# dragonlong/articulated-pose

Measured on AMD Instinct MI355X. Metric: point-clouds/sec (N=1024, eyeglasses ANCSH infer+pose-fit), higher is better.
Workload: dtype f32 (network) / f64 (joint LM)

## Files before the change

### articulated-pose_amd/_lib.py

```python
import ctypes
import os
import subprocess

import torch

_HERE = os.path.dirname(os.path.abspath(__file__))
LIB_PATH = os.environ.get("ANCSH_HIP_LIB") or os.path.join(_HERE, "libancsh_hip.so")

_c_int, _c_long, _c_float, _vp = ctypes.c_int, ctypes.c_long, ctypes.c_float, ctypes.c_void_p

SIGNATURES = {
    "ancsh_farthest_point_sample": [_c_int, _c_int, _c_int, _vp, _vp, _vp, _vp],
    "ancsh_farthest_point_sample_gather": [_c_int, _c_int, _c_int, _vp, _vp, _vp, _vp, _vp],
    "ancsh_prob_sample": [_c_int, _c_int, _c_int, _vp, _vp, _vp, _vp, _vp],
    "ancsh_gather_point": [_c_int, _c_int, _c_int, _vp, _vp, _vp, _vp],
    "ancsh_query_ball_point": [_c_int, _c_int, _c_int, _c_float, _c_int, _vp, _vp, _vp, _vp, _vp],
    "ancsh_query_ball_point_multi": [_c_int] + [_vp] * 10,
    "ancsh_group_point": [_c_int, _c_int, _c_int, _c_int, _c_int, _vp, _vp, _vp, _vp],
    "ancsh_group_point_multi": [_c_int] + [_vp] * 9,
    "ancsh_selection_sort": [_c_int, _c_int, _c_int, _c_int, _vp, _vp, _vp, _vp],
    "ancsh_knn_point": [_c_int, _c_int, _c_int, _c_int, _c_int, _vp, _vp, _vp, _vp, _vp],
    "ancsh_group_point_ex": [_c_int, _c_int, _c_int, _c_int, _c_int, _vp, _vp, _vp, _vp, _c_int, _c_int, _vp],
    "ancsh_three_nn": [_c_int, _c_int, _c_int, _vp, _vp, _vp, _vp, _vp],
    "ancsh_three_weights": [_c_int, _vp, _vp, _vp],
    "ancsh_three_nn_weights": [_c_int, _c_int, _c_int, _vp, _vp, _vp, _vp, _vp, _vp],
    "ancsh_three_interpolate": [_c_int, _c_int, _c_int, _c_int, _vp, _vp, _vp, _vp, _vp],
    "ancsh_three_interpolate_ex": [_c_int, _c_int, _c_int, _c_int, _vp, _vp, _vp, _vp, _c_int, _c_int, _vp],
    "ancsh_conv1x1": [_c_long, _c_int, _c_int, _vp, _c_int, _vp, _vp, _vp, _vp, _c_int, _vp, _c_int, _c_int, _vp],
    "ancsh_conv1x1_ex": [_c_long, _c_int, _c_int, _vp, _c_int, _vp, _vp, _vp, _vp, _c_int, _vp, _c_int, _c_int, _vp, _c_int, _vp],
    "ancsh_conv1x1_packed": [_c_long, _c_int, _c_int, _vp, _c_int, _vp, _vp, _vp, _vp, _c_int, _vp, _c_int, _c_int, _vp, _c_int, _vp],
    "ancsh_conv1x1_packed_grouped": [_c_int, _c_long, _c_int, _c_int, _vp, _c_int, _vp, _vp, _vp, _vp, _c_int, _vp, _c_int, _c_int, _vp, _c_int, _vp],
    "ancsh_conv1x1_grouped": [_c_int, _c_long, _c_int, _c_int, _vp, _c_int, _vp, _vp, _vp, _vp, _c_int, _vp, _c_int, _c_int, _vp],
    "ancsh_sa_module_fused_grouped": [_c_int] * 9 + [_vp] * 4 + [_vp, _vp, _vp],
    "ancsh_sa_module_fused_partial_grouped": [_c_int] * 8 + [_vp] * 7,
    "ancsh_fp_interpolate_concat_ex": [_c_int, _c_int, _c_int, _c_int, _vp, _vp, _vp, _vp, _c_int, _vp, _c_int, _c_int, _c_int, _vp],
    "ancsh_sa_pack_weights_bf16x3": [_c_int, _c_int, _vp, _vp, _vp],
    "ancsh_sa_module_fused_bf16x3": [_c_int] * 8 + [_vp] * 4 + [_vp, _vp, _vp],
    "ancsh_sa_module_fused_partial_bf16x3": [_c_int] * 7 + [_vp] * 7,
    "ancsh_sa_module_fused_bf16x3_grouped": [_c_int] * 9 + [_vp] * 4 + [_vp, _vp, _vp],
    "ancsh_sa_module_fused_partial_bf16x3_grouped": [_c_int] * 8 + [_vp] * 7,
    "ancsh_sa_pack_weights_f16x2": [_c_int, _c_int, _vp, _vp, _vp],
    "ancsh_sa_module_fused_f16x2_grouped": [_c_int] * 9 + [_vp] * 4 + [_vp, _vp, _vp],
    "ancsh_sa_module_fused_partial_f16x2_grouped": [_c_int] * 8 + [_vp] * 7,
    "ancsh_mlp_chain_grouped_fp_f16x2": [_c_int] * 5 + [_vp] * 7 + [_vp],
    "ancsh_sa3_chain_grouped_bf16x3": [_c_int] * 7 + [_vp] * 4 + [_vp],
    "ancsh_sa3_chain_grouped_f16x2": [_c_int] * 7 + [_vp] * 4 + [_vp],
    "ancsh_fp1_chain_grouped_bf16x3": [_c_int] * 6 + [_vp] * 4 + [_vp],
    "ancsh_fp1_chain_grouped_f16x2": [_c_int] * 6 + [_vp] * 4 + [_vp],
    "ancsh_fp2_chain_grouped_bf16x3": [_c_int] * 8 + [_vp] * 6 + [_vp],
    "ancsh_fp2_chain_grouped_f16x2": [_c_int] * 8 + [_vp] * 6 + [_vp],
    "ancsh_sa_module_fused_f16x2_grouped_guarded": [_c_int] * 9 + [_vp] * 4 + [_vp, _vp, _vp, _c_int, _vp],
    "ancsh_sa_module_fused_partial_f16x2_grouped_guarded": [_c_int] * 8 + [_vp] * 6 + [_vp, _c_int, _vp],
    "ancsh_mlp_chain_grouped_fp_f16x2_guarded": [_c_int] * 5 + [_vp] * 7 + [_vp, _c_int, _vp],
    "ancsh_sa3_chain_grouped_f16x2_guarded": [_c_int] * 7 + [_vp] * 4 + [_vp, _c_int, _vp],
    "ancsh_fp1_chain_grouped_f16x2_guarded": [_c_int] * 6 + [_vp] * 4 + [_vp, _c_int, _vp],
    "ancsh_fp2_chain_grouped_f16x2_guarded": [_c_int] * 8 + [_vp] * 6 + [_vp, _c_int, _vp],
    "ancsh_iou_3d": [_c_int, _c_int, _vp, _vp, _vp, _vp, _vp],
    "ancsh_joint_params": [_c_int] * 5 + [_vp] * 9 + [_vp],
    "ancsh_part_extents": [_c_int] * 4 + [_vp] * 3 + [_c_int] + [_vp] * 4 + [_vp],
    "ancsh_articulation_rec": [_c_int] * 5 + [_vp] * 10 + [_vp] * 4 + [_vp],
    "ancsh_fp_interpolate_concat": [_c_int, _c_int, _c_int, _c_int, _vp, _vp, _vp, _vp, _c_int, _vp, _c_int, _vp],
    "ancsh_query_ball_group_xyz": [_c_int, _c_int, _c_int, _c_float, _c_int, _vp, _vp, _c_int, _vp, _vp, _vp, _c_int, _vp],
    "ancsh_query_ball_group_xyz_multi": [_c_int] + [_vp] * 13,
    "ancsh_group_max": [_c_long, _c_int, _c_int, _vp, _vp, _vp],
    "ancsh_sa_module_fused": [_c_int] * 8 + [_vp] * 4 + [_vp, _vp, _vp],
    "ancsh_sa_module_fused_partial": [_c_int] * 7 + [_vp] * 7,
    "ancsh_sa_pack_weights": [_c_int, _c_int, _vp, _vp, _vp],
    "ancsh_mlp_chain": [_c_long, _c_int, _vp, _c_int, _c_int, _vp, _vp, _vp],
    "ancsh_mlp_chain_grouped": [_c_int, _c_long, _c_int, _vp, _c_int, _vp, _vp, _vp, _vp, _vp],
    "ancsh_sa3_chain_grouped": [_c_int] * 7 + [_vp] * 4 + [_vp],
    "ancsh_fp_single_source_init": [_c_int] * 5 + [_vp] * 3 + [_vp],
    "ancsh_fp1_chain_grouped": [_c_int] * 6 + [_vp] * 4 + [_vp],
    "ancsh_fp2_chain_grouped": [_c_int] * 8 + [_vp] * 6 + [_vp],
    "ancsh_mlp_chain_grouped_fp": [_c_int] * 5 + [_vp] * 8 + [_vp],
    "ancsh_mlp_chain_grouped_fp_bf16x3": [_c_int] * 5 + [_vp] * 7 + [_vp],
    "ancsh_head_activations": [_c_long, _c_int, _c_int, _vp, _c_int] + [_vp] * 10 + [_vp],
    "ancsh_pose_partition": [_c_int, _c_int, _c_int] + [_vp] * 11 + [_vp],
    "ancsh_pose_poison_records": [_c_int, _c_int, _c_int] + [_vp] * 5 + [_vp],
    "ancsh_pose_joint_direction": [_c_int, _c_int, _c_int, _vp, _vp, _vp, _vp],
    "ancsh_ransac_single": [_c_int, _vp, _vp, _vp, _c_float, _c_int, _vp, ctypes.c_ulonglong, _c_int, _vp, _vp, _vp, _vp, _vp],
    "ancsh_ransac_single_ex": [_c_int, _vp, _vp, _vp, _c_float, _c_int, _vp, ctypes.c_ulonglong, _c_int, _vp, _vp, _vp, _vp, _vp, _c_long, _vp],
    "ancsh_ransac_single_rec": [_c_int, _vp, _vp, _vp, _c_float, _c_int, _vp, ctypes.c_ulonglong, _c_int, _vp, _vp, _vp, _vp, _vp, _c_long,
                                _vp, _c_int, _vp, _c_float, _vp],
    "ancsh_ransac_joint_rec": [_c_int, _vp, _vp, _vp, _vp, _vp, ctypes.c_double, _c_int, _vp, ctypes.c_ulonglong, _c_int]
                              + [_vp] * 7 + [_c_int, _vp, _c_int, _vp, ctypes.c_double, _vp],
    "ancsh_ransac_joint": [_c_int, _vp, _vp, _vp, _vp, _vp, ctypes.c_double, _c_int, _vp, ctypes.c_ulonglong, _c_int]
                          + [_vp] * 7 + [_vp],
    "ancsh_ransac_single_rec_dseed": [_c_int, _vp, _vp, _vp, _c_float, _c_int, _vp, _vp, _c_int, _vp, _vp, _vp, _vp, _vp, _c_long,
                                      _vp, _c_int, _vp, _c_float, _vp],
    "ancsh_ransac_joint_rec_dseed": [_c_int, _vp, _vp, _vp, _vp, _vp, ctypes.c_double, _c_int, _vp, _vp, _c_int]
                                    + [_vp] * 7 + [_c_int, _vp, _c_int, _vp, ctypes.c_double, _vp],
    "ancsh_input_sample_stream": [_c_int, _c_int, _c_int, _vp, _c_long, _vp, _vp, _c_int, _vp, _vp, _vp, _vp, _vp],
    "ancsh_input_sample_stream_keyed": [_c_int, _c_int, _c_int, _vp, _c_long, _vp, _vp, _c_int, _vp, _vp, _vp, _vp, _vp],
    "ancsh_ransac_single_rec_dkey": [_c_int, _vp, _vp, _vp, _c_float, _c_int, _vp, _vp, _c_int, _vp, _vp, _vp, _vp, _vp, _c_long,
                                     _vp, _c_int, _vp, _c_float, _vp],
    "ancsh_ransac_joint_rec_dkey": [_c_int, _vp, _vp, _vp, _vp, _vp, ctypes.c_double, _c_int, _vp, _vp, _c_int]
                                   + [_vp] * 7 + [_c_int, _vp, _c_int, _vp, ctypes.c_double, _vp],
    "ancsh_raw_point_labels": [_c_int] * 5 + [_vp, _c_long] + [_vp] * 8 + [_vp],
    "ancsh_pose_joint_direction_pred": [_c_int, _c_int, _c_int, _c_int, _vp, _vp, _vp, _vp],
    "ancsh_pose_poison_records_pred": [_c_int, _c_int, _c_int] + [_vp] * 4 + [_c_int, _vp, _vp, _vp],
    "ancsh_input_sample_stream_xyz": [_c_int, _c_int, _c_int, _vp, _c_long, _vp, _vp, _vp, _vp, _vp, _vp],
    "ancsh_input_sample_stream_xyz_keyed": [_c_int, _c_int, _c_int, _vp, _c_long, _vp, _vp, _vp, _vp, _vp, _vp],
    "ancsh_ransac_joint_rec_kind": [_c_int, _vp, _vp, _vp, _vp, _vp, ctypes.c_double, _c_int, _vp, ctypes.c_ulonglong, _c_int]
                                   + [_vp] * 7 + [_c_int, _vp, _c_int, _vp, ctypes.c_double, _vp, _vp],
    "ancsh_ransac_joint_rec_dseed_kind": [_c_int, _vp, _vp, _vp, _vp, _vp, ctypes.c_double, _c_int, _vp, _vp, _c_int]
                                         + [_vp] * 7 + [_c_int, _vp, _c_int, _vp, ctypes.c_double, _vp, _vp],
    "ancsh_ransac_joint_rec_dkey_kind": [_c_int, _vp, _vp, _vp, _vp, _vp, ctypes.c_double, _c_int, _vp, _vp, _c_int]
                                        + [_vp] * 7 + [_c_int, _vp, _c_int, _vp, ctypes.c_double, _vp, _vp],
    "ancsh_depth_unproject_stream": [_c_int, _c_int, _vp, _vp, _c_long, _vp, _vp, _vp, _c_long, _vp, _vp, _vp, _vp],
    "ancsh_depth_label_images": [_c_int, _c_int, _vp, _vp, _c_long] + [_vp] * 5 + [_c_long, _vp, _vp, _vp, _c_long, _vp],
    "ancsh_joint_state_rec": [_c_int] * 3 + [_vp, _c_int] + [_vp] * 5 + [_vp],
    "ancsh_input_sample": [_c_int, _c_int, _c_int, _vp, _vp, _vp, _vp, _c_int, _c_int, _c_int, _vp, _vp, _vp, _vp, _vp],
    "ancsh_test_losses": [_c_int, _c_int, _c_int, _c_int, _vp, _vp, _vp],
    "ancsh_ransac_joint_ex": [_c_int, _vp, _vp, _vp, _vp, _vp, ctypes.c_double, _c_int, _vp, ctypes.c_ulonglong, _c_int]
                             + [_vp] * 7 + [_c_int, _vp],
    "ancsh_umeyama": [_c_int, _vp, _vp, _vp, _vp, _vp],
    "ancsh_estimate_similarity_transform": [_c_int, _vp, _vp, _vp, _c_int, _vp, ctypes.c_ulonglong, _vp, _vp, _vp],
}

_lib = None


def build(force=False):
    args = ["make", "-s", "-j8", "-C", os.path.join(_HERE, "csrc")]
    if force:
        subprocess.check_call(args + ["clean"])
    subprocess.check_call(args)
    return LIB_PATH


def lib():
    global _lib
    if _lib is None:
        if not os.path.exists(LIB_PATH):
            raise RuntimeError(
                f"{LIB_PATH} is missing: the HIP extension is not built (run __graft_entry__.build()); "
                "there is no CPU fallback for the product path")
        L = ctypes.CDLL(LIB_PATH)
        for name, argtypes in SIGNATURES.items():
            fn = getattr(L, name)
            fn.argtypes = argtypes
            fn.restype = _c_int
        L.ancsh_last_error.restype = ctypes.c_char_p
        L.ancsh_abi_version.restype = _c_int
        L.ancsh_last_ball_query_schedule.restype = _c_int
        L.ancsh_sa_packed_weight_floats.argtypes = [_c_int, _c_int]
        L.ancsh_sa_packed_weight_floats.restype = _c_long
        L.ancsh_sa_packed_weight_bytes_bf16x3.argtypes = [_c_int, _c_int]
        L.ancsh_sa_packed_weight_bytes_bf16x3.restype = _c_long
        L.ancsh_sa_packed_weight_bytes_f16x2.argtypes = [_c_int, _c_int]
        L.ancsh_sa_packed_weight_bytes_f16x2.restype = _c_long
        L.ancsh_ransac_single_quads_floats.argtypes = [_c_long, _c_int]
        L.ancsh_ransac_single_quads_floats.restype = _c_long
        _lib = L
    return _lib


def stream_ptr():
    return torch.cuda.current_stream().cuda_stream


def ptr(t):
    return 0 if t is None else t.data_ptr()


_prof = None
_prof_lead = (0, {})


def profile_start(lead=0, lead_for=None):
    global _prof, _prof_lead
    _prof, _prof_lead = [], (int(lead), dict(lead_for or {}))


def profile_stop():
    global _prof
    rec, _prof = _prof, None
    torch.cuda.synchronize()
    return [(n, a, e0.elapsed_time(e1)) for n, a, e0, e1 in rec]


def call(name, *args):
    L = lib()
    if _prof is not None:
        e0, e1 = torch.cuda.Event(enable_timing=True), torch.cuda.Event(enable_timing=True)
        for _ in range(_prof_lead[1].get(name, _prof_lead[0])):
            getattr(L, name)(*args, stream_ptr())
        e0.record()
        rc = getattr(L, name)(*args, stream_ptr())
        e1.record()
        _prof.append((name, args, e0, e1))
    else:
        rc = getattr(L, name)(*args, stream_ptr())
    if rc != 0:
        msg = L.ancsh_last_error().decode()
        if rc == -1:
            raise ValueError(msg)
        raise RuntimeError(f"{name}: {msg}")


def require_cuda(*tensors):
    for t in tensors:
        if t is not None and not t.is_cuda:
            raise RuntimeError("articulated-pose_amd ops run on the MI355X only: got a CPU tensor "
                               "(no CPU fallback in the product path)")
```

### articulated-pose_amd/csrc/pose.hip

```cpp
#include "common.h"
#include "pose_math.h"

namespace ancsh {
namespace pose {

constexpr int MODEL_A = 13;
constexpr int MODEL_B = 26;

__device__ __forceinline__ unsigned long long splitmix64(unsigned long long x) {
    x += 0x9E3779B97F4A7C15ull;
    x = (x ^ (x >> 30)) * 0xBF58476D1CE4E5B9ull;
    x = (x ^ (x >> 27)) * 0x94D049BB133111EBull;
    return x ^ (x >> 31);
}
__device__ __forceinline__ int device_draw(unsigned long long seed, int prob, int iter, int k, int n) {
    const unsigned long long h = splitmix64(seed ^ splitmix64(((unsigned long long)prob << 40) ^ ((unsigned long long)iter << 8) ^ (unsigned)k));
    return (int)(h % (unsigned long long)n);
}
enum { KEY_VALUE = 0, KEY_DSEED = 1, KEY_DKEY = 2 };
struct DKey {
    const ancsh_stream_key *key;
    int parts;
};
template <int KM> struct KeyArgT { typedef unsigned long long type; };
// ... 262 lines not shown
                s3[i][c] = src[(size_t)(r0 + id[i]) * 3 + c];
                t3[i][c] = tgt[(size_t)(r0 + id[i]) * 3 + c];
            }
        estimate_single3(s3, t3, R, sc, tr);
    }
    typedef float f32x8 __attribute__((ext_vector_type(8)));
    const int q0 = quad_start(r0, prob);
    const f32x8 *Q = reinterpret_cast<const f32x8 *>(quads + (size_t)q0 * 24);
    int nq = ((n + 7) >> 3) * 2;
    nq = min(nq, (cap_quads - q0) & ~1);
    f32x2 cnt2 = {0.f, 0.f};
    auto score4 = [&](const f32x8 &v0, const f32x8 &v1, const f32x8 &v2) {
        inlier2_count_f32(R, sc, tr, f32x2{v0[0], v0[1]}, f32x2{v0[4], v0[5]}, f32x2{v1[0], v1[1]}, f32x2{v1[4], v1[5]},
                          f32x2{v2[0], v2[1]}, f32x2{v2[4], v2[5]}, th, cnt2);
        inlier2_count_f32(R, sc, tr, f32x2{v0[2], v0[3]}, f32x2{v0[6], v0[7]}, f32x2{v1[2], v1[3]}, f32x2{v1[6], v1[7]},
                          f32x2{v2[2], v2[3]}, f32x2{v2[6], v2[7]}, th, cnt2);
    };
    constexpr int LGKM0 = 0xC07F;
    if (nq > 0) {
        f32x8 a0 = Q[0], a1 = Q[1], a2 = Q[2];
        __builtin_amdgcn_s_waitcnt(LGKM0);
        for (int q = 0; q < nq; q += 2) {
            const int q2 = q + 2 < nq ? q + 2 : q;
            const f32x8 b0 = Q[q * 3 + 3], b1 = Q[q * 3 + 4], b2 = Q[q * 3 + 5];
            __builtin_amdgcn_sched_barrier(0);
            score4(a0, a1, a2);
            __builtin_amdgcn_sched_barrier(0);
            __builtin_amdgcn_s_waitcnt(LGKM0);
            a0 = Q[q2 * 3]; a1 = Q[q2 * 3 + 1]; a2 = Q[q2 * 3 + 2];
            __builtin_amdgcn_sched_barrier(0);
            score4(b0, b1, b2);
            __builtin_amdgcn_sched_barrier(0);
            __builtin_amdgcn_s_waitcnt(LGKM0);
        }
    }
    if (h < niter) scores[(size_t)prob * niter + h] = n > 0 ? (int)(cnt2.x + cnt2.y) : 0;
}

template <class T>
__device__ __forceinline__ int block_argmax_first(const T *sc, int niter, T *best_out, void *lds) {
    T bv = (T)-1;
    int bi = 0x7fffffff;
    for (int h = threadIdx.x; h < niter; h += blockDim.x) {
        const T v = sc[h];
        if (v > bv) { bv = v; bi = h; }
    }
#pragma unroll
    for (int o = 32; o > 0; o >>= 1) {
        const T ov = __shfl_xor(bv, o, 64);
        const int oi = __shfl_xor(bi, o, 64);
        if (ov > bv || (ov == bv && oi < bi)) { bv = ov; bi = oi; }
    }
    T *rv = (T *)lds;
    int *ri = (int *)(rv + 8);
    const int lane = threadIdx.x & 63, wave = threadIdx.x >> 6, nw = blockDim.x >> 6;
    __syncthreads();
    if (lane == 0) { rv[wave] = bv; ri[wave] = bi; }
    __syncthreads();
    bv = rv[0]; bi = ri[0];
    for (int w = 1; w < nw; ++w)
        if (rv[w] > bv || (rv[w] == bv && ri[w] < bi)) { bv = rv[w]; bi = ri[w]; }
    __syncthreads();
    *best_out = bv;
    return bi;
}

__device__ __forceinline__ void pair_sums(const float (*cs)[3], const float (*ct)[3], int n, double (&pr)[3]) {
#pragma clang fp contract(off)
    const int lane = threadIdx.x & 63;
    const int wave = __builtin_amdgcn_readfirstlane(threadIdx.x >> 6), nw = blockDim.x >> 6;
    const int seg = (n + nw - 1) / nw;
    const int j0 = wave * seg, j1 = min(n, j0 + seg);
    constexpr int RB = 6;
    for (int ib = lane; ib < n; ib += 64 * RB) {
        float sx[RB], sy[RB], sz[RB], tx[RB], ty[RB], tz[RB], ab[RB], aa[RB], bb[RB];
#pragma unroll
        for (int r = 0; r < RB; ++r) {
            const int i = min(ib + 64 * r, n - 1);
            sx[r] = cs[i][0]; sy[r] = cs[i][1]; sz[r] = cs[i][2];
            tx[r] = ct[i][0]; ty[r] = ct[i][1]; tz[r] = ct[i][2];
            ab[r] = aa[r] = bb[r] = 0.f;
        }
        for (int j = j0; j < j1; ++j) {
            const float cx = cs[j][0], cy = cs[j][1], cz = cs[j][2], dx = ct[j][0], dy = ct[j][1], dz = ct[j][2];
#pragma unroll
            for (int r = 0; r < RB; ++r) {
                const float ux = sx[r] - cx, uy = sy[r] - cy, uz = sz[r] - cz;
                const float vx = tx[r] - dx, vy = ty[r] - dy, vz = tz[r] - dz;
                const float A = __builtin_amdgcn_sqrtf((ux * ux + uy * uy) + uz * uz);
                const float b = __builtin_amdgcn_sqrtf((vx * vx + vy * vy) + vz * vz);
                ab[r] += A * b;
                aa[r] += A * A;
                bb[r] += b * b;
            }
        }
#pragma unroll
        for (int r = 0; r < RB; ++r)
            if (ib + 64 * r < n) { pr[0] += (double)ab[r]; pr[1] += (double)aa[r]; pr[2] += (double)bb[r]; }
    }
}

__device__ __forceinline__ void refit_similarity(const float (*cs)[3], const float (*ct)[3], int n_in, double *red,
                                                 double R[9], double &scale, double tr[3]) {
    double sums[6] = {0, 0, 0, 0, 0, 0};
    for (int i = threadIdx.x; i < n_in; i += 256) {
#pragma unroll
        for (int c = 0; c < 3; ++c) { sums[c] += cs[i][c]; sums[3 + c] += ct[i][c]; }
    }
    block_sum<6>(sums, red, 4);
    double sm[3], tm[3];
#pragma unroll
    for (int c = 0; c < 3; ++c) { sm[c] = sums[c] / n_in; tm[c] = sums[3 + c] / n_in; }
    double M[9] = {0, 0, 0, 0, 0, 0, 0, 0, 0};
    for (int i = threadIdx.x; i < n_in; i += 256)
#pragma unroll
        for (int a = 0; a < 3; ++a)
#pragma unroll
            for (int b = 0; b < 3; ++b) M[a * 3 + b] += (ct[i][a] - tm[a]) * (cs[i][b] - sm[b]);
    block_sum<9>(M, red, 4);
    double q[4];
    horn_quat(M, q);
    quat_to_mat(q, R);
    double pr[3] = {0, 0, 0};
    pair_sums(cs, ct, n_in, pr);
    block_sum<3>(pr, red, 4);
    scale = pr[0] / (pr[1] + 1e-6);
    const double sf = (double)(float)scale;
#pragma unroll
    for (int a = 0; a < 3; ++a) tr[a] = tm[a] - sf * (R[a * 3 + 0] * sm[0] + R[a * 3 + 1] * sm[1] + R[a * 3 + 2] * sm[2]);
}

__device__ __forceinline__ int compact_flagged(bool flag, int i, int n, const float *src, const float *tgt, size_t row0,
                                               float (*cs)[3], float (*ct)[3], int base, int *wcnt) {
    const int lane = threadIdx.x & 63, wave = threadIdx.x >> 6;
    const unsigned long long m = __ballot(flag);
    __syncthreads();
    if (lane == 0) wcnt[wave] = __popcll(m);
    __syncthreads();
    int start = base;
    for (int w = 0; w < wave; ++w) start += wcnt[w];
    const int total = wcnt[0] + wcnt[1] + wcnt[2] + wcnt[3];
    if (flag) {
        const int pos = start + __builtin_amdgcn_mbcnt_hi((unsigned)(m >> 32), __builtin_amdgcn_mbcnt_lo((unsigned)m, 0));
#pragma unroll
        for (int c = 0; c < 3; ++c) {
            cs[pos][c] = src[(row0 + i) * 3 + c];
            ct[pos][c] = tgt[(row0 + i) * 3 + c];
        }
    }
    return base + total;
}

template <int KM>
__global__ __launch_bounds__(256) void ransac_single_finish_kernel(const int *__restrict__ off, const float *__restrict__ src,
                                                                   const float *__restrict__ tgt, float th, int niter,
                                                                   const int *__restrict__ draws, KeyArg<KM> seed_arg,
                                                                   const int *__restrict__ scores, int max_n,
                                                                   double *__restrict__ out_model,
                                                                   unsigned char *__restrict__ out_inliers,
                                                                   int *__restrict__ out_best, FitExtras E) {
    const unsigned long long seed = kernel_seed<KM>(seed_arg, 0);
    const int kbase = key_problem_base<KM>(seed_arg);
    extern __shared__ __attribute__((aligned(16))) unsigned char smem[];
    double *red = (double *)smem;
    int *wcnt = (int *)(red + 64);
    float(*cs)[3] = (float(*)[3])(wcnt + 8);
    float(*ct)[3] = cs + max_n;
    const int prob = blockIdx.x;
    const int r0 = off[prob], n = off[prob + 1] - r0;
    double *om = out_model + (size_t)prob * MODEL_A;
    if (n <= 0 || n > max_n) {
        if (threadIdx.x < MODEL_A) om[threadIdx.x] = NAN;
        if (E.record && threadIdx.x < (E.K == 1 ? 2 * MODEL_A : MODEL_A)) E.record[(size_t)prob * 26 + threadIdx.x] = NAN;
        if (E.tie && threadIdx.x < 2) E.tie[prob * 2 + threadIdx.x] = 0;
        if (threadIdx.x == 0) { out_best[prob * 2] = -1; out_best[prob * 2 + 1] = n <= 0 ? 0 : -2; }
        for (int i = threadIdx.x; i < n; i += 256) out_inliers[r0 + i] = 0;
        return;
    }
    int best_score;
    const int best = block_argmax_first<int>(scores + (size_t)prob * niter, niter, &best_score, red);
    int id[3];
    load_draw3(draws, seed, prob, kbase, niter, best, 0, 3, n, id);
    float s3[3][3], t3[3][3], R[9], sc, tr[3];
#pragma unroll
    for (int i = 0; i < 3; ++i)
#pragma unroll
        for (int c = 0; c < 3; ++c) {
            s3[i][c] = src[(size_t)(r0 + id[i]) * 3 + c];
            t3[i][c] = tgt[(size_t)(r0 + id[i]) * 3 + c];
        }
    estimate_single3(s3, t3, R, sc, tr);
    int n_in = 0, n_border = 0, n_near = 0;
    for (int base = 0; base < n; base += 256) {
        const int i = base + threadIdx.x;
        bool f = false, border = false;
        if (i < n) {
            const float *ps = src + (size_t)(r0 + i) * 3, *pt = tgt + (size_t)(r0 + i) * 3;
            const float rs = residual_sq_f32(R, sc, tr, ps[0], ps[1], ps[2], pt[0], pt[1], pt[2]);
            f = rs < th;
            border = rs >= E.lo_f && rs < E.hi_f;
            out_inliers[r0 + i] = f ? 1 : 0;
        }
        n_border += __popcll(__ballot(border));
        n_in = compact_flagged(f, i, n, src, tgt, (size_t)r0, cs, ct, n_in, wcnt);
    }
    if (E.tie) {
        const bool winner_degenerate = id[0] == id[1] || id[0] == id[2] || id[1] == id[2];
        __shared__ int s_cand[TIE_MAX_CAND];
        const int *sp = scores + (size_t)prob * niter;
        const int lane = threadIdx.x & 63, wave = threadIdx.x >> 6;
        int found = 0;
        for (int h0 = 0; h0 < niter; h0 += 256) {
            const int h = h0 + threadIdx.x;
            bool cand = false;
            if (h < niter && h != best && sp[h] >= best_score - 1) {
                int d3[3];
                load_draw3(draws, seed, prob, kbase, niter, h, 0, 3, n, d3);
                cand = d3[0] == d3[1] || d3[0] == d3[2] || d3[1] == d3[2];
            }
            const unsigned long long m = __ballot(cand);
            __syncthreads();
            if (lane == 0) wcnt[wave] = __popcll(m);
            __syncthreads();
            int start = found;
            for (int w = 0; w < wave; ++w) start += wcnt[w];
            if (cand) {
                const int slot = start + __builtin_amdgcn_mbcnt_hi((unsigned)(m >> 32), __builtin_amdgcn_mbcnt_lo((unsigned)m, 0));
                if (slot < TIE_MAX_CAND) s_cand[slot] = h;
            }
            found += wcnt[0] + wcnt[1] + wcnt[2] + wcnt[3];
        }
        __syncthreads();
        const int ncand = found < TIE_MAX_CAND ? found : TIE_MAX_CAND;
        n_near = found - ncand + (winner_degenerate ? 1 : 0);
        for (int c = 0; c < ncand; ++c) {
            const int h = s_cand[c];
            int d3[3];
            load_draw3(draws, seed, prob, kbase, niter, h, 0, 3, n, d3);
            float hs[3][3], ht[3][3], hR[9], hsc, htr[3];
#pragma unroll
            for (int i = 0; i < 3; ++i)
#pragma unroll
                for (int cc = 0; cc < 3; ++cc) {
                    hs[i][cc] = src[(size_t)(r0 + d3[i]) * 3 + cc];
                    ht[i][cc] = tgt[(size_t)(r0 + d3[i]) * 3 + cc];
                }
            estimate_single3(hs, ht, hR, hsc, htr);
            int differs = 0;
            for (int i = threadIdx.x; i < n; i += 256) {
                const float *ps = src + (size_t)(r0 + i) * 3, *pt = tgt + (size_t)(r0 + i) * 3;
                const bool f = residual_sq_f32(hR, hsc, htr, ps[0], ps[1], ps[2], pt[0], pt[1], pt[2]) < th;
                differs |= (int)(f != (out_inliers[r0 + i] != 0));
            }
            n_near += __syncthreads_or(differs) ? 1 : 0;
        }
        if ((threadIdx.x & 63) == 0) wcnt[4 + (threadIdx.x >> 6)] = n_border;
        __syncthreads();
        if (threadIdx.x == 0) {
            E.tie[prob * 2] = wcnt[4] + wcnt[5] + wcnt[6] + wcnt[7];
            E.tie[prob * 2 + 1] = winner_degenerate ? -n_near : n_near;
        }
    }
    __syncthreads();
    double Rd[9], scale, trd[3];
    if (n_in > 0) {
        refit_similarity(cs, ct, n_in, red, Rd, scale, trd);
    } else {
#pragma unroll
        for (int a = 0; a < 9; ++a) Rd[a] = NAN;
        scale = NAN; trd[0] = trd[1] = trd[2] = NAN;
    }
    if (threadIdx.x == 0) {
#pragma unroll
        for (int a = 0; a < 9; ++a) om[a] = Rd[a];
        om[9] = (double)(float)scale;
#pragma unroll
        for (int a = 0; a < 3; ++a) om[10 + a] = trd[a];
        out_best[prob * 2] = best;
        out_best[prob * 2 + 1] = best_score;
        if (E.record) {
            double *rec = E.record + (size_t)prob * 26;
#pragma unroll
            for (int a = 0; a < MODEL_A; ++a) rec[a] = om[a];
            if (E.K == 1) {
#pragma unroll
                for (int a = 0; a < MODEL_A; ++a) rec[MODEL_A + a] = om[a];
            }
        }
    }
}

struct PartFd {
    Rod b, p[3];
    double rh[3];
    double blk[6];
    double gv[3];
    double ju[3];
    double jd[3][3];

    __device__ __forceinline__ void begin_points(const double r[3]) {
        b = rod_prepare(r[0], r[1], r[2]);
#pragma unroll
        for (int q = 0; q < 3; ++q) {
            const double h = fd_step(r[q]);
            rh[q] = fast_rcp(h);
            p[q] = rod_prepare(r[0] + (q == 0 ? h : 0.0), r[1] + (q == 1 ? h : 0.0), r[2] + (q == 2 ? h : 0.0));
        }
#pragma unroll
        for (int i = 0; i < 6; ++i) blk[i] = 0.0;
        gv[0] = gv[1] = gv[2] = 0.0;
    }
    __device__ __forceinline__ void begin(const double r[3], const double J[3]) {
        begin_points(r);
        rod_apply(b, J[0], J[1], J[2], ju[0], ju[1], ju[2]);
#pragma unroll
        for (int q = 0; q < 3; ++q) {
            double qx, qy, qz;
            rod_apply(p[q], J[0], J[1], J[2], qx, qy, qz);
            jd[0][q] = qx; jd[1][q] = qy; jd[2][q] = qz;
        }
    }
    __device__ __forceinline__ void point(double px, double py, double pz, double yx, double yy, double yz) {
        double ox, oy, oz;
        rod_apply(b, px, py, pz, ox, oy, oz);
        const double f0 = yx - ox, f1 = yy - oy, f2 = yz - oz;
        double a[3][3];
#pragma unroll
        for (int q = 0; q < 3; ++q) {
            double qx, qy, qz;
            rod_apply(p[q], px, py, pz, qx, qy, qz);
            a[0][q] = ((yx - qx) - f0) * rh[q];
            a[1][q] = ((yy - qy) - f1) * rh[q];
            a[2][q] = ((yz - qz) - f2) * rh[q];
        }
#pragma unroll
        for (int q = 0; q < 3; ++q) {
#pragma unroll
            for (int r = 0; r <= q; ++r) blk[q * (q + 1) / 2 + r] += a[0][q] * a[0][r] + a[1][q] * a[1][r] + a[2][q] * a[2][r];
            gv[q] += a[0][q] * f0 + a[1][q] * f1 + a[2][q] * f2;
        }
    }
};

__device__ __forceinline__ void assemble_normal(const PartFd &p0, const double blk0[6], const double g0[3], const PartFd &p1,
                                                const double blk1[6], const double g1[3], double wj, double A[21], double g[6]) {
    double f[3], a[3][6];
#pragma unroll
    for (int c = 0; c < 3; ++c) f[c] = p0.ju[c] - p1.ju[c];
#pragma unroll
    for (int c = 0; c < 3; ++c)
#pragma unroll
        for (int q = 0; q < 3; ++q) {
            a[c][q] = (((p0.jd[c][q] - p1.ju[c]) - f[c])) * p0.rh[q];
            a[c][3 + q] = (((p0.ju[c] - p1.jd[c][q]) - f[c])) * p1.rh[q];
        }
#pragma unroll
    for (int i = 0; i < 6; ++i) {
#pragma unroll
        for (int j = 0; j <= i; ++j) {
            double v = wj * (a[0][i] * a[0][j] + a[1][i] * a[1][j] + a[2][i] * a[2][j]);
            if (i < 3) v += blk0[i * (i + 1) / 2 + j];
            else if (j >= 3) v += blk1[(i - 3) * (i - 2) / 2 + (j - 3)];
            A[i * (i + 1) / 2 + j] = v;
        }
        g[i] = wj * (a[0][i] * f[0] + a[1][i] * f[1] + a[2][i] * f[2]) + (i < 3 ? g0[i] : g1[i - 3]);
    }
}

__device__ __forceinline__ double prismatic_cost(const double x[6]) {
    const double a = x[0] - x[3], b = x[1] - x[4], c = x[2] - x[5];
    return a * a + b * b + c * c;
}
__device__ __forceinline__ void assemble_normal_prismatic(const double x[6], const double blk0[6], const double g0[3],
                                                          const double blk1[6], const double g1[3], double A[21], double g[6]) {
    double f[3], d0[3], d1[3];
#pragma unroll
    for (int c = 0; c < 3; ++c) {
        const double h0 = fd_step(x[c]), h1 = fd_step(x[3 + c]);
        f[c] = x[c] - x[3 + c];
        d0[c] = (((x[c] + h0) - x[3 + c]) - f[c]) * fast_rcp(h0);
        d1[c] = ((x[c] - (x[3 + c] + h1)) - f[c]) * fast_rcp(h1);
    }
#pragma unroll
    for (int i = 0; i < 6; ++i) {
#pragma unroll
        for (int j = 0; j <= i; ++j) {
            double v = 0.0;
            if (i < 3) v = (i == j ? d0[i] * d0[i] : 0.0) + blk0[i * (i + 1) / 2 + j];
            else if (j >= 3) v = (i == j ? d1[i - 3] * d1[i - 3] : 0.0) + blk1[(i - 3) * (i - 2) / 2 + (j - 3)];
            else if (i - 3 == j) v = d1[j] * d0[j];
            A[i * (i + 1) / 2 + j] = v;
        }
        g[i] = i < 3 ? d0[i] * f[i] + g0[i] : d1[i - 3] * f[i - 3] + g1[i - 3];
    }
}

template <bool PRISM>
struct HypProblemT {
    double x0[3][3], y0[3][3], x1[3][3], y1[3][3], J[3], wj;

    __device__ __forceinline__ double cost(const double x[6]) const {
        const Rod r0 = rod_prepare(x[0], x[1], x[2]), r1 = rod_prepare(x[3], x[4], x[5]);
        double s = 0.0, ox, oy, oz;
#pragma unroll
        for (int i = 0; i < 3; ++i) {
            rod_apply(r0, x0[i][0], x0[i][1], x0[i][2], ox, oy, oz);
            const double a = y0[i][0] - ox, b = y0[i][1] - oy, c = y0[i][2] - oz;
            s += a * a + b * b + c * c;
            rod_apply(r1, x1[i][0], x1[i][1], x1[i][2], ox, oy, oz);
            const double d = y1[i][0] - ox, e = y1[i][1] - oy, f = y1[i][2] - oz;
            s += d * d + e * e + f * f;
        }
        if constexpr (PRISM) {
            return s + prismatic_cost(x);
        } else {
            double ux, uy, uz, wx, wy, wz;
            rod_apply(r0, J[0], J[1], J[2], ux, uy, uz);
            rod_apply(r1, J[0], J[1], J[2], wx, wy, wz);
            s += wj * ((ux - wx) * (ux - wx) + (uy - wy) * (uy - wy) + (uz - wz) * (uz - wz));
            return s;
        }
    }
    __device__ __forceinline__ void normal(const double x[6], double A[21], double g[6]) const {
        PartFd p0, p1;
        if constexpr (PRISM) p0.begin_points(x); else p0.begin(x, J);
#pragma unroll
        for (int i = 0; i < 3; ++i) p0.point(x0[i][0], x0[i][1], x0[i][2], y0[i][0], y0[i][1], y0[i][2]);
        if constexpr (PRISM) p1.begin_points(x + 3); else p1.begin(x + 3, J);
#pragma unroll
        for (int i = 0; i < 3; ++i) p1.point(x1[i][0], x1[i][1], x1[i][2], y1[i][0], y1[i][1], y1[i][2]);
        if constexpr (PRISM) assemble_normal_prismatic(x, p0.blk, p0.gv, p1.blk, p1.gv, A, g);
        else assemble_normal(p0, p0.blk, p0.gv, p1, p1.blk, p1.gv, wj, A, g);
    }
};
typedef HypProblemT<false> HypProblem;

__device__ __forceinline__ void scales3(const float s[3][3], const float t[3][3], float &sc, float &sc_inv) {
    double ab = 0.0, aa = 0.0, bb = 0.0;
#pragma unroll
    for (int i = 0; i < 3; ++i)
#pragma unroll
        for (int j = i + 1; j < 3; ++j) {
            double ds = 0.0, dt = 0.0;
#pragma unroll
            for (int c = 0; c < 3; ++c) {
                const double u = (double)s[i][c] - s[j][c], v = (double)t[i][c] - t[j][c];
                ds += u * u;
                dt += v * v;
            }
            ab += 2.0 * sqrt(ds) * sqrt(dt);
            aa += 2.0 * ds;
            bb += 2.0 * dt;
        }
    sc = (float)(ab / (aa + 1e-6));
    sc_inv = (float)(ab / (bb + 1e-6));
}

__device__ __forceinline__ void center_part3(const float s[3][3], const float t[3][3], float sc_inv, double xc[3][3],
                                             double yc[3][3]) {
    float sm[3], tm[3];
#pragma unroll
    for (int c = 0; c < 3; ++c) {
        sm[c] = ((s[0][c] + s[1][c]) + s[2][c]) / 3.0f;
        tm[c] = ((sc_inv * t[0][c] + sc_inv * t[1][c]) + sc_inv * t[2][c]) / 3.0f;
    }
#pragma unroll
    for (int i = 0; i < 3; ++i) {
#pragma unroll
        for (int c = 0; c < 3; ++c) {
            xc[i][c] = (double)(s[i][c] - sm[c]);
            yc[i][c] = (double)(sc_inv * t[i][c] - tm[c]);
        }
    }
}

__device__ __forceinline__ void prep_part3(const float s[3][3], const float t[3][3], float sc_inv, double xc[3][3],
                                           double yc[3][3], double rv[3]) {
    center_part3(s, t, sc_inv, xc, yc);
    double M[9] = {0, 0, 0, 0, 0, 0, 0, 0, 0};
#pragma unroll
    for (int i = 0; i < 3; ++i)
#pragma unroll
        for (int a = 0; a < 3; ++a)
#pragma unroll
            for (int b = 0; b < 3; ++b) M[a * 3 + b] += yc[i][a] * xc[i][b];
    double q[4];
    horn_quat_fast(M, q);
    quat_to_rotvec(q, rv);
}

__device__ __forceinline__ double residual_sq_f64(const double R[9], double sc, const double tr[3], float sx, float sy, float sz,
                                                  float tx, float ty, float tz) {
    const double rx = R[0] * sx + R[1] * sy + R[2] * sz, ry = R[3] * sx + R[4] * sy + R[5] * sz,
                 rz = R[6] * sx + R[7] * sy + R[8] * sz;
    const double ex = ((double)tx - sc * rx) - tr[0], ey = ((double)ty - sc * ry) - tr[1], ez = ((double)tz - sc * rz) - tr[2];
    return ex * ex + ey * ey + ez * ez;
}
__device__ __forceinline__ bool inlier_f64(const double R[9], double sc, const double tr[3], float sx, float sy, float sz,
                                           float tx, float ty, float tz, double th) {
    return residual_sq_f64(R, sc, tr, sx, sy, sz, tx, ty, tz) < th;
}

struct HypSamples {
    float s0[3][3], t0[3][3], s1[3][3], t1[3][3];
};
__device__ __forceinline__ void load_hyp_samples(const float *__restrict__ src, const float *__restrict__ tgt, const int *draws,
                                                 unsigned long long seed, int prob, int kbase, int niter, int h, int a0, int n0, int a1,
                                                 int n1, HypSamples &q) {
    int i0[3], i1[3];
    load_draw3(draws, seed, prob, kbase, niter, h, 0, 6, n0, i0);
    load_draw3(draws, seed, prob, kbase, niter, h, 3, 6, n1, i1);
#pragma unroll
    for (int i = 0; i < 3; ++i)
#pragma unroll
        for (int c = 0; c < 3; ++c) {
            q.s0[i][c] = src[(size_t)(a0 + i0[i]) * 3 + c];
            q.t0[i][c] = tgt[(size_t)(a0 + i0[i]) * 3 + c];
            q.s1[i][c] = src[(size_t)(a1 + i1[i]) * 3 + c];
            q.t1[i][c] = tgt[(size_t)(a1 + i1[i]) * 3 + c];
        }
}

template <int KM>
__global__ __launch_bounds__(64) void ransac_joint_init_kernel(const int *__restrict__ rng0, const int *__restrict__ rng1,
                                                               const float *__restrict__ src, const float *__restrict__ tgt,
                                                               int niter, const int *__restrict__ draws, KeyArg<KM> seed_arg,
                                                               double *__restrict__ scores, double *__restrict__ models) {
    const unsigned long long seed = kernel_seed<KM>(seed_arg, 1);
    const int kbase = key_problem_base<KM>(seed_arg);
    const int prob = blockIdx.y, h = blockIdx.x * 64 + threadIdx.x;
    const int a0 = rng0[prob * 2], n0 = rng0[prob * 2 + 1] - a0;
    const int a1 = rng1[prob * 2], n1 = rng1[prob * 2 + 1] - a1;
    if (h >= niter) return;
    double *mo = models + ((size_t)prob * niter + h) * MODEL_B;
    if (n0 <= 0 || n1 <= 0) {
        scores[(size_t)prob * niter + h] = -1.0;
        for (int i = 0; i < MODEL_B; ++i) mo[i] = NAN;
        return;
    }
    HypSamples q;
    load_hyp_samples(src, tgt, draws, seed, prob, kbase, niter, h, a0, n0, a1, n1, q);
    float sc0, sc0i, sc1, sc1i;
    scales3(q.s0, q.t0, sc0, sc0i);
    scales3(q.s1, q.t1, sc1, sc1i);
    double xc[3][3], yc[3][3], x[6];
    prep_part3(q.s0, q.t0, sc0i, xc, yc, x);
    prep_part3(q.s1, q.t1, sc1i, xc, yc, x + 3);
#pragma unroll
    for (int i = 0; i < 6; ++i) mo[i] = x[i];
    mo[6] = sc0i; mo[7] = sc1i; mo[8] = sc0; mo[9] = sc1;
}

constexpr int HYP_CHUNK = 256;
constexpr int HYP_CHUNK_SMALL = 64;
constexpr long HYP_SMALL_LAUNCH = 8192;
constexpr int HYP_REFILL = 16;

template <int KM, bool PRISM>
__device__ __forceinline__ void ransac_joint_lm_run(const int *__restrict__ rng0, const int *__restrict__ rng1,
                                                    const float *__restrict__ src, const float *__restrict__ tgt,
                                                    const float *__restrict__ joint_dir, int niter,
                                                    const int *__restrict__ draws, KeyArg<KM> seed_arg,
                                                    double *__restrict__ models, int *__restrict__ lm_stat, int chunk) {
    const unsigned long long seed = kernel_seed<KM>(seed_arg, 1);
    const int kbase = key_problem_base<KM>(seed_arg);
    const int prob = blockIdx.y;
    const int a0 = rng0[prob * 2], n0 = rng0[prob * 2 + 1] - a0;
    const int a1 = rng1[prob * 2], n1 = rng1[prob * 2 + 1] - a1;
    if (n0 <= 0 || n1 <= 0) return;
    const int c1 = min(niter, (int)(blockIdx.x + 1) * chunk);
    int next = blockIdx.x * chunk;
    HypProblemT<PRISM> P;
    if constexpr (!PRISM) {
        P.J[0] = joint_dir[prob * 3]; P.J[1] = joint_dir[prob * 3 + 1]; P.J[2] = joint_dir[prob * 3 + 2];
        P.wj = 3.0;
    }
    Lm6 S;
    bool active = false;
    int h = 0;
    for (;;) {
        const unsigned long long idle = __ballot(!active);
        const int n_idle = __popcll(idle);
        if (next < c1 && (n_idle >= HYP_REFILL || n_idle >= c1 - next || n_idle == 64)) {
            if (!active) {
                const int mine = next + __builtin_amdgcn_mbcnt_hi((unsigned)(idle >> 32), __builtin_amdgcn_mbcnt_lo((unsigned)idle, 0));
                if (mine < c1) {
                    h = mine;
                    const double *mo = models + ((size_t)prob * niter + h) * MODEL_B;
                    HypSamples q;
                    load_hyp_samples(src, tgt, draws, seed, prob, kbase, niter, h, a0, n0, a1, n1, q);
                    center_part3(q.s0, q.t0, (float)mo[6], P.x0, P.y0);
                    center_part3(q.s1, q.t1, (float)mo[7], P.x1, P.y1);
#pragma unroll
                    for (int i = 0; i < 6; ++i) S.x[i] = mo[i];
                    lm6_begin(P, S);
                    active = true;
                }
            }
            next += n_idle;
        } else if (n_idle == 64) {
            break;
        }
        if (active && lm6_trip(P, S, 1e-4, 1e-8, 1e-8, 4200)) {
            double *mo = models + ((size_t)prob * niter + h) * MODEL_B;
#pragma unroll
            for (int i = 0; i < 6; ++i) mo[i] = S.x[i];
#ifdef LM_COUNT
            if (lm_stat) { lm_stat[((size_t)prob * niter + h) * 2] = S.info | (S.trips << 4) | (S.nchol << 17); lm_stat[((size_t)prob * niter + h) * 2 + 1] = S.nfev; }
#else
            if (lm_stat) { lm_stat[((size_t)prob * niter + h) * 2] = S.info; lm_stat[((size_t)prob * niter + h) * 2 + 1] = S.nfev; }
#endif
            active = false;
        }
    }
}

template <int KM>
__global__ __launch_bounds__(64) void ransac_joint_lm_kernel(const int *__restrict__ rng0, const int *__restrict__ rng1,
                                                             const float *__restrict__ src, const float *__restrict__ tgt,
                                                             const float *__restrict__ joint_dir, int niter,
                                                             const int *__restrict__ draws, KeyArg<KM> seed_arg,
                                                             double *__restrict__ models, int *__restrict__ lm_stat, int chunk) {
    ransac_joint_lm_run<KM, false>(rng0, rng1, src, tgt, joint_dir, niter, draws, seed_arg, models, lm_stat, chunk);
}

template <int KM>
__global__ __launch_bounds__(64) void ransac_joint_lm_kind_kernel(const int *__restrict__ rng0, const int *__restrict__ rng1,
                                                                  const float *__restrict__ src, const float *__restrict__ tgt,
                                                                  const float *__restrict__ joint_dir, int niter,
                                                                  const int *__restrict__ draws, KeyArg<KM> seed_arg,
                                                                  double *__restrict__ models, int *__restrict__ lm_stat, int chunk,
                                                                  const int *__restrict__ joint_kind) {
    if (joint_kind[blockIdx.y] != 0) ransac_joint_lm_run<KM, true>(rng0, rng1, src, tgt, joint_dir, niter, draws, seed_arg, models, lm_stat, chunk);
    else ransac_joint_lm_run<KM, false>(rng0, rng1, src, tgt, joint_dir, niter, draws, seed_arg, models, lm_stat, chunk);
}

constexpr int COOP_G = 8;
constexpr int COOP_XCH = 112;
constexpr int COOP_HYP_PER_WAVE = 32;

__device__ __forceinline__ void group_lds_fence() {
    __builtin_amdgcn_fence(__ATOMIC_RELEASE, "wavefront");
    __builtin_amdgcn_wave_barrier();
    __builtin_amdgcn_fence(__ATOMIC_ACQUIRE, "wavefront");
}

template <bool PRISM>
struct HypProblemCoopT {
    double x0[3][3], y0[3][3], x1[3][3], y1[3][3], J[3], wj;
    double *xch;
    int role;

    __device__ __forceinline__ double cost(const double x[6]) const {
        const bool joint = role >= 6;
        const bool p1 = role >= 3 && role < 6;
        const int i = joint ? 0 : (p1 ? role - 3 : role);
        double partial;
        if (!joint) {
            const Rod r = p1 ? rod_prepare(x[3], x[4], x[5]) : rod_prepare(x[0], x[1], x[2]);
            const double px = p1 ? (i == 0 ? x1[0][0] : i == 1 ? x1[1][0] : x1[2][0]) : (i == 0 ? x0[0][0] : i == 1 ? x0[1][0] : x0[2][0]);
            const double py = p1 ? (i == 0 ? x1[0][1] : i == 1 ? x1[1][1] : x1[2][1]) : (i == 0 ? x0[0][1] : i == 1 ? x0[1][1] : x0[2][1]);
            const double pz = p1 ? (i == 0 ? x1[0][2] : i == 1 ? x1[1][2] : x1[2][2]) : (i == 0 ? x0[0][2] : i == 1 ? x0[1][2] : x0[2][2]);
            const double tx = p1 ? (i == 0 ? y1[0][0] : i == 1 ? y1[1][0] : y1[2][0]) : (i == 0 ? y0[0][0] : i == 1 ? y0[1][0] : y0[2][0]);
            const double ty = p1 ? (i == 0 ? y1[0][1] : i == 1 ? y1[1][1] : y1[2][1]) : (i == 0 ? y0[0][1] : i == 1 ? y0[1][1] : y0[2][1]);
            const double tz = p1 ? (i == 0 ? y1[0][2] : i == 1 ? y1[1][2] : y1[2][2]) : (i == 0 ? y0[0][2] : i == 1 ? y0[1][2] : y0[2][2]);
            double ox, oy, oz;
            rod_apply(r, px, py, pz, ox, oy, oz);
            const double a = tx - ox, b = ty - oy, c = tz - oz;
            partial = a * a + b * b + c * c;
        } else if constexpr (PRISM) {
            partial = prismatic_cost(x);
        } else {
            const Rod r0 = rod_prepare(x[0], x[1], x[2]), r1 = rod_prepare(x[3], x[4], x[5]);
            double ux, uy, uz, wx, wy, wz;
            rod_apply(r0, J[0], J[1], J[2], ux, uy, uz);
            rod_apply(r1, J[0], J[1], J[2], wx, wy, wz);
            partial = (ux - wx) * (ux - wx) + (uy - wy) * (uy - wy) + (uz - wz) * (uz - wz);
        }
        double *cs = xch + 102;
        if (role < 7) cs[role] = partial;
        group_lds_fence();
        double s = 0.0;
#pragma unroll
        for (int k = 0; k < 3; ++k) { s += cs[k]; s += cs[3 + k]; }
        if constexpr (PRISM) s += cs[6]; else s += wj * cs[6];
        group_lds_fence();
        return s;
    }

    __device__ __forceinline__ void normal(const double x[6], double A[21], double g[6]) const {
        double *col = xch, *jdx = xch + 54, *rhx = xch + 72, *fx = xch + 78, *jux = xch + 96;
        {
            const int cr = role < 6 ? role : role - 6;
            const bool p1 = cr >= 3;
            const int q = p1 ? cr - 3 : cr;
            const double r0 = p1 ? x[3] : x[0], r1 = p1 ? x[4] : x[1], r2 = p1 ? x[5] : x[2];
            const Rod b = rod_prepare(r0, r1, r2);
            const double h = fd_step(q == 0 ? r0 : q == 1 ? r1 : r2);
            const double rh = fast_rcp(h);
            const Rod pr = rod_prepare(r0 + (q == 0 ? h : 0.0), r1 + (q == 1 ? h : 0.0), r2 + (q == 2 ? h : 0.0));
            const bool wr = role < 6;
#pragma unroll
            for (int i = 0; i < 3; ++i) {
                const double px = p1 ? x1[i][0] : x0[i][0], py = p1 ? x1[i][1] : x0[i][1], pz = p1 ? x1[i][2] : x0[i][2];
                const double yx = p1 ? y1[i][0] : y0[i][0], yy = p1 ? y1[i][1] : y0[i][1], yz = p1 ? y1[i][2] : y0[i][2];
                double ox, oy, oz, qx, qy, qz;
                rod_apply(b, px, py, pz, ox, oy, oz);
                const double f0 = yx - ox, f1 = yy - oy, f2 = yz - oz;
// ... 172 lines not shown
    for (int i = 0; i < 6; ++i) x[i] = mo[i];
    const float sc0 = (float)mo[8], sc1 = (float)mo[9];
    double R0[9], R1[9], tr0[3], tr1[3];
    rotvec_to_mat(x, R0);
    rotvec_to_mat(x + 3, R1);
#pragma unroll
    for (int a = 0; a < 3; ++a) {
        double u = 0.0, v = 0.0;
#pragma unroll
        for (int i = 0; i < 3; ++i) {
            u += (double)q.t0[i][a] - (double)sc0 * (R0[a * 3] * q.s0[i][0] + R0[a * 3 + 1] * q.s0[i][1] + R0[a * 3 + 2] * q.s0[i][2]);
            v += (double)q.t1[i][a] - (double)sc1 * (R1[a * 3] * q.s1[i][0] + R1[a * 3 + 1] * q.s1[i][1] + R1[a * 3 + 2] * q.s1[i][2]);
        }
        tr0[a] = u / 3.0;
        tr1[a] = v / 3.0;
    }
#pragma unroll
    for (int a = 0; a < 9; ++a) { mo[a] = R0[a]; mo[13 + a] = R1[a]; }
    mo[9] = sc0; mo[22] = sc1;
#pragma unroll
    for (int a = 0; a < 3; ++a) { mo[10 + a] = tr0[a]; mo[23 + a] = tr1[a]; }
}

__global__ __launch_bounds__(256) void ransac_joint_verify_kernel(const int *__restrict__ rng0, const int *__restrict__ rng1,
                                                                 const float *__restrict__ src, const float *__restrict__ tgt,
                                                                 double th, int niter, const double *__restrict__ models,
                                                                 double *__restrict__ scores) {
    const int prob = blockIdx.y, lane = threadIdx.x & 63;
    const int h = blockIdx.x * 4 + (threadIdx.x >> 6);
    if (h >= niter) return;
    const int a0 = rng0[prob * 2], n0 = rng0[prob * 2 + 1] - a0;
    const int a1 = rng1[prob * 2], n1 = rng1[prob * 2 + 1] - a1;
    if (n0 <= 0 || n1 <= 0) return;
    const double *mo = models + ((size_t)prob * niter + h) * MODEL_B;
    double R0[9], R1[9], tr0[3], tr1[3];
#pragma unroll
    for (int a = 0; a < 9; ++a) { R0[a] = mo[a]; R1[a] = mo[13 + a]; }
    const double sc0 = mo[9], sc1 = mo[22];
#pragma unroll
    for (int a = 0; a < 3; ++a) { tr0[a] = mo[10 + a]; tr1[a] = mo[23 + a]; }
    int c0 = 0, c1 = 0;
    for (int i = lane; i < n0; i += 64) {
        const float *ps = src + (size_t)(a0 + i) * 3, *pt = tgt + (size_t)(a0 + i) * 3;
        c0 += inlier_f64(R0, sc0, tr0, ps[0], ps[1], ps[2], pt[0], pt[1], pt[2], th) ? 1 : 0;
    }
    for (int i = lane; i < n1; i += 64) {
        const float *ps = src + (size_t)(a1 + i) * 3, *pt = tgt + (size_t)(a1 + i) * 3;
        c1 += inlier_f64(R1, sc1, tr1, ps[0], ps[1], ps[2], pt[0], pt[1], pt[2], th) ? 1 : 0;
    }
#pragma unroll
    for (int o = 32; o > 0; o >>= 1) { c0 += __shfl_xor(c0, o, 64); c1 += __shfl_xor(c1, o, 64); }
    if (lane == 0) scores[(size_t)prob * niter + h] = ((double)c0 / 3.0 + (double)c1 / 3.0) / 2.0;
}

template <bool PRISM>
struct BlockProblemT {
    const float (*x0)[3];
    const float (*y0)[3];
    const float (*x1)[3];
    const float (*y1)[3];
    int n0, n1;
    double J[3], wj;
    double *red;

    __device__ __forceinline__ double cost(const double x[6]) const {
        const Rod r0 = rod_prepare(x[0], x[1], x[2]), r1 = rod_prepare(x[3], x[4], x[5]);
        double s[1] = {0.0}, ox, oy, oz;
        for (int i = threadIdx.x; i < n0; i += 256) {
            rod_apply(r0, x0[i][0], x0[i][1], x0[i][2], ox, oy, oz);
            const double a = y0[i][0] - ox, b = y0[i][1] - oy, c = y0[i][2] - oz;
            s[0] += a * a + b * b + c * c;
        }
        for (int i = threadIdx.x; i < n1; i += 256) {
            rod_apply(r1, x1[i][0], x1[i][1], x1[i][2], ox, oy, oz);
            const double a = y1[i][0] - ox, b = y1[i][1] - oy, c = y1[i][2] - oz;
            s[0] += a * a + b * b + c * c;
        }
        block_sum<1>(s, red, 4);
        if constexpr (PRISM) {
            return s[0] + prismatic_cost(x);
        } else {
            double ux, uy, uz, wx, wy, wz;
            rod_apply(r0, J[0], J[1], J[2], ux, uy, uz);
            rod_apply(r1, J[0], J[1], J[2], wx, wy, wz);
            return s[0] + wj * ((ux - wx) * (ux - wx) + (uy - wy) * (uy - wy) + (uz - wz) * (uz - wz));
        }
    }
    __device__ __forceinline__ void normal(const double x[6], double A[21], double g[6]) const {
        PartFd p0, p1;
        if constexpr (PRISM) p0.begin_points(x); else p0.begin(x, J);
        for (int i = threadIdx.x; i < n0; i += 256) p0.point(x0[i][0], x0[i][1], x0[i][2], y0[i][0], y0[i][1], y0[i][2]);
        if constexpr (PRISM) p1.begin_points(x + 3); else p1.begin(x + 3, J);
        for (int i = threadIdx.x; i < n1; i += 256) p1.point(x1[i][0], x1[i][1], x1[i][2], y1[i][0], y1[i][1], y1[i][2]);
        double v[18];
#pragma unroll
        for (int i = 0; i < 6; ++i) { v[i] = p0.blk[i]; v[9 + i] = p1.blk[i]; }
#pragma unroll
        for (int i = 0; i < 3; ++i) { v[6 + i] = p0.gv[i]; v[15 + i] = p1.gv[i]; }
        block_sum<18>(v, red, 4);
        if constexpr (PRISM) assemble_normal_prismatic(x, v, v + 6, v + 9, v + 15, A, g);
        else assemble_normal(p0, v, v + 6, p1, v + 9, v + 15, wj, A, g);
    }
};
typedef BlockProblemT<false> BlockProblem;

__device__ __forceinline__ void block_scales(const float (*cs)[3], const float (*ct)[3], int n, double *red, float &sc,
                                             float &sc_inv) {
    double pr[3] = {0, 0, 0};
    pair_sums(cs, ct, n, pr);
    block_sum<3>(pr, red, 4);
    sc = (float)(pr[0] / (pr[1] + 1e-6));
    sc_inv = (float)(pr[0] / (pr[2] + 1e-6));
}

__device__ __forceinline__ void block_prep_part(float (*cs)[3], float (*ct)[3], int n, float sc_inv, double *red,
                                                double smean[3], double tmean[3], double rv[3]) {
    double sums[6] = {0, 0, 0, 0, 0, 0};
    for (int i = threadIdx.x; i < n; i += 256)
#pragma unroll
        for (int c = 0; c < 3; ++c) { sums[c] += cs[i][c]; sums[3 + c] += ct[i][c]; }
    block_sum<6>(sums, red, 4);
#pragma unroll
    for (int c = 0; c < 3; ++c) { smean[c] = sums[c] / n; tmean[c] = sums[3 + c] / n; }
    double M[9] = {0, 0, 0, 0, 0, 0, 0, 0, 0};
    for (int i = threadIdx.x; i < n; i += 256) {
        float xc[3], yc[3];
#pragma unroll
        for (int c = 0; c < 3; ++c) {
            xc[c] = cs[i][c] - (float)smean[c];
            yc[c] = sc_inv * ct[i][c] - (float)((double)sc_inv * tmean[c]);
            cs[i][c] = xc[c];
            ct[i][c] = yc[c];
        }
#pragma unroll
        for (int a = 0; a < 3; ++a)
#pragma unroll
            for (int b = 0; b < 3; ++b) M[a * 3 + b] += (double)yc[a] * xc[b];
    }
    block_sum<9>(M, red, 4);
    double q[4];
    horn_quat(M, q);
    quat_to_rotvec(q, rv);
}

template <int KM, bool PRISM>
__device__ __forceinline__ void ransac_joint_finish_run(const int *__restrict__ rng0, const int *__restrict__ rng1,
                                                        const float *__restrict__ src, const float *__restrict__ tgt,
                                                        const float *__restrict__ joint_dir, double th, int niter,
                                                        const double *__restrict__ scores,
                                                        const double *__restrict__ models, int max_n,
                                                        double *__restrict__ out_model,
                                                        unsigned char *__restrict__ out_inliers,
                                                        int *__restrict__ out_best, double *__restrict__ out_score, const FitExtras &E,
                                                        unsigned char *smem) {
    double *red = (double *)smem;
    int *wcnt = (int *)(red + 128);
    float(*c0s)[3] = (float(*)[3])(wcnt + 8);
    float(*c0t)[3] = c0s + max_n;
    float(*c1s)[3] = c0t + max_n;
    float(*c1t)[3] = c1s + max_n;
    const int prob = blockIdx.x;
    const int a0 = rng0[prob * 2], n0 = rng0[prob * 2 + 1] - a0;
    const int a1 = rng1[prob * 2], n1 = rng1[prob * 2 + 1] - a1;
    double *om = out_model + (size_t)prob * MODEL_B;
    unsigned char *oi0 = out_inliers + (size_t)prob * 2 * max_n, *oi1 = oi0 + max_n;
    double *rec1 = nullptr, *rec0 = nullptr;
    if (E.record) {
        const int cloud = prob / (E.K - 1), q = prob - cloud * (E.K - 1);
        rec1 = E.record + ((size_t)cloud * E.K + q + 1) * 26 + MODEL_A;
        if (q == 0) rec0 = E.record + (size_t)cloud * E.K * 26 + MODEL_A;
    }
    if (n0 <= 0 || n1 <= 0 || n0 > max_n || n1 > max_n) {
        if (threadIdx.x < MODEL_B) om[threadIdx.x] = NAN;
        if (threadIdx.x < MODEL_A) { if (rec1) rec1[threadIdx.x] = NAN; if (rec0) rec0[threadIdx.x] = NAN; }
        if (E.tie && threadIdx.x < 2) E.tie[prob * 2 + threadIdx.x] = 0;
        if (threadIdx.x == 0) { out_best[prob] = -1; out_score[prob] = -1.0; }
        for (int i = threadIdx.x; i < 2 * max_n; i += 256) oi0[i] = 0;
        return;
    }
    for (int i = n0 + threadIdx.x; i < max_n; i += 256) oi0[i] = 0;
    for (int i = n1 + threadIdx.x; i < max_n; i += 256) oi1[i] = 0;
    double best_score;
    const int best = block_argmax_first<double>(scores + (size_t)prob * niter, niter, &best_score, red);
    const double *bm = models + ((size_t)prob * niter + best) * MODEL_B;
    double R0[9], R1[9], tr0[3], tr1[3];
#pragma unroll
    for (int a = 0; a < 9; ++a) { R0[a] = bm[a]; R1[a] = bm[13 + a]; }
    const double hs0 = bm[9], hs1 = bm[22];
#pragma unroll
    for (int a = 0; a < 3; ++a) { tr0[a] = bm[10 + a]; tr1[a] = bm[23 + a]; }
    int m0 = 0, m1 = 0, n_border = 0, n_near = 0;
    for (int base = 0; base < n0; base += 256) {
        const int i = base + threadIdx.x;
        bool f = false, border = false;
        if (i < n0) {
            const float *ps = src + (size_t)(a0 + i) * 3, *pt = tgt + (size_t)(a0 + i) * 3;
            const double rs = residual_sq_f64(R0, hs0, tr0, ps[0], ps[1], ps[2], pt[0], pt[1], pt[2]);
            f = rs < th;
            border = rs >= E.lo_d && rs < E.hi_d;
            oi0[i] = f ? 1 : 0;
        }
        n_border += __popcll(__ballot(border));
        m0 = compact_flagged(f, i, n0, src, tgt, (size_t)a0, c0s, c0t, m0, wcnt);
    }
    for (int base = 0; base < n1; base += 256) {
        const int i = base + threadIdx.x;
        bool f = false, border = false;
        if (i < n1) {
            const float *ps = src + (size_t)(a1 + i) * 3, *pt = tgt + (size_t)(a1 + i) * 3;
            const double rs = residual_sq_f64(R1, hs1, tr1, ps[0], ps[1], ps[2], pt[0], pt[1], pt[2]);
            f = rs < th;
            border = rs >= E.lo_d && rs < E.hi_d;
            oi1[i] = f ? 1 : 0;
        }
        n_border += __popcll(__ballot(border));
        m1 = compact_flagged(f, i, n1, src, tgt, (size_t)a1, c1s, c1t, m1, wcnt);
    }
    if (E.tie) {
        const unsigned long long tseed = kernel_seed<KM>(E.seed, 1);
        const int tbase = KM == KEY_DKEY ? ((const ancsh_stream_key *)E.seed)->cloud_base * (E.K - 1) : 0;
        const double *sp = scores + (size_t)prob * niter;
        const double near = best_score - (1.0 / 6.0 + 1e-9);
        for (int h = threadIdx.x; h < niter + 255 - (niter + 255) % 256; h += 256) {
            bool degenerate = false;
            if (h < niter && sp[h] >= near) {
                int i0[3], i1[3];
                load_draw3(E.draws, tseed, prob, tbase, niter, h, 0, 6, n0, i0);
                load_draw3(E.draws, tseed, prob, tbase, niter, h, 3, 6, n1, i1);
                degenerate = i0[0] == i0[1] || i0[0] == i0[2] || i0[1] == i0[2] || i1[0] == i1[1] || i1[0] == i1[2] || i1[1] == i1[2];
            }
            n_near += __popcll(__ballot(degenerate));
        }
        if ((threadIdx.x & 63) == 0) { wcnt[4 + (threadIdx.x >> 6)] = n_border; red[8 + (threadIdx.x >> 6)] = (double)n_near; }
        __syncthreads();
        if (threadIdx.x == 0) {
            E.tie[prob * 2] = wcnt[4] + wcnt[5] + wcnt[6] + wcnt[7];
            E.tie[prob * 2 + 1] = (int)(red[8] + red[9] + red[10] + red[11]);
        }
    }
    __syncthreads();
    if (m0 == 0 || m1 == 0) {
        if (threadIdx.x < MODEL_B) om[threadIdx.x] = NAN;
        if (threadIdx.x < MODEL_A) { if (rec1) rec1[threadIdx.x] = NAN; if (rec0) rec0[threadIdx.x] = NAN; }
        if (threadIdx.x == 0) { out_best[prob] = best; out_score[prob] = best_score; }
        return;
    }
    float sc0, sc0i, sc1, sc1i;
    block_scales(c0s, c0t, m0, red, sc0, sc0i);
    block_scales(c1s, c1t, m1, red, sc1, sc1i);
    double sm0[3], tm0[3], sm1[3], tm1[3], x[6];
    block_prep_part(c0s, c0t, m0, sc0i, red, sm0, tm0, x);
    block_prep_part(c1s, c1t, m1, sc1i, red, sm1, tm1, x + 3);
    __syncthreads();
    if constexpr (PRISM) {
        BlockProblemT<true> P;
        P.x0 = c0s; P.y0 = c0t; P.x1 = c1s; P.y1 = c1t;
        P.n0 = m0; P.n1 = m1;
        P.red = red;
        lmdif6(P, x, 1e-4, 1e-8, 1e-8, 4200, nullptr);
    } else {
        BlockProblem P;
        P.x0 = c0s; P.y0 = c0t; P.x1 = c1s; P.y1 = c1t;
        P.n0 = m0; P.n1 = m1;
        P.J[0] = joint_dir[prob * 3]; P.J[1] = joint_dir[prob * 3 + 1]; P.J[2] = joint_dir[prob * 3 + 2];
        P.wj = (double)(m0 < m1 ? m0 : m1);
        P.red = red;
        lmdif6(P, x, 1e-4, 1e-8, 1e-8, 4200, nullptr);
    }
    rotvec_to_mat(x, R0);
    rotvec_to_mat(x + 3, R1);
    if (threadIdx.x == 0) {
#pragma unroll
        for (int a = 0; a < 9; ++a) { om[a] = R0[a]; om[13 + a] = R1[a]; }
        om[9] = sc0; om[22] = sc1;
#pragma unroll
        for (int a = 0; a < 3; ++a) {
            om[10 + a] = tm0[a] - (double)sc0 * (R0[a * 3] * sm0[0] + R0[a * 3 + 1] * sm0[1] + R0[a * 3 + 2] * sm0[2]);
            om[23 + a] = tm1[a] - (double)sc1 * (R1[a * 3] * sm1[0] + R1[a * 3 + 1] * sm1[1] + R1[a * 3 + 2] * sm1[2]);
        }
        out_best[prob] = best;
        out_score[prob] = best_score;
#pragma unroll
        for (int a = 0; a < MODEL_A; ++a) {
            if (rec1) rec1[a] = om[MODEL_A + a];
            if (rec0) rec0[a] = om[a];
        }
    }
}

template <int KM>
__global__ __launch_bounds__(256) void ransac_joint_finish_kernel(const int *__restrict__ rng0, const int *__restrict__ rng1,
                                                                  const float *__restrict__ src, const float *__restrict__ tgt,
                                                                  const float *__restrict__ joint_dir, double th, int niter,
                                                                  const double *__restrict__ scores,
                                                                  const double *__restrict__ models, int max_n,
                                                                  double *__restrict__ out_model,
                                                                  unsigned char *__restrict__ out_inliers,
                                                                  int *__restrict__ out_best, double *__restrict__ out_score, FitExtras E) {
    extern __shared__ __attribute__((aligned(16))) unsigned char smem[];
    ransac_joint_finish_run<KM, false>(rng0, rng1, src, tgt, joint_dir, th, niter, scores, models, max_n, out_model, out_inliers, out_best,
                                       out_score, E, smem);
}

template <int KM>
__global__ __launch_bounds__(256) void ransac_joint_finish_kind_kernel(const int *__restrict__ rng0, const int *__restrict__ rng1,
                                                                       const float *__restrict__ src, const float *__restrict__ tgt,
                                                                       const float *__restrict__ joint_dir, double th, int niter,
                                                                       const double *__restrict__ scores,
                                                                       const double *__restrict__ models, int max_n,
                                                                       double *__restrict__ out_model,
                                                                       unsigned char *__restrict__ out_inliers,
                                                                       int *__restrict__ out_best, double *__restrict__ out_score, FitExtras E,
                                                                       const int *__restrict__ joint_kind) {
    extern __shared__ __attribute__((aligned(16))) unsigned char smem[];
    if (joint_kind[blockIdx.x] != 0)
        ransac_joint_finish_run<KM, true>(rng0, rng1, src, tgt, joint_dir, th, niter, scores, models, max_n, out_model, out_inliers, out_best,
                                          out_score, E, smem);
    else
        ransac_joint_finish_run<KM, false>(rng0, rng1, src, tgt, joint_dir, th, niter, scores, models, max_n, out_model, out_inliers, out_best,
                                           out_score, E, smem);
}

__global__ __launch_bounds__(256) void partition_kernel(int n, int K, const float *__restrict__ W, const float *__restrict__ P,
                                                        const float *__restrict__ nocs, int *__restrict__ labels,
                                                        int *__restrict__ part_index, int *__restrict__ off,
                                                        float *__restrict__ src, float *__restrict__ tgt,
                                                        int *__restrict__ counts, int *__restrict__ rng0, int *__restrict__ rng1) {
    __shared__ int wcnt[4];
    __shared__ int part_start[17];
    const int b = blockIdx.x, lane = threadIdx.x & 63, wave = threadIdx.x >> 6;
    const float *Wb = W + (size_t)b * n * K;
    int base = 0;
    for (int j = 0; j < K; ++j) {
        if (threadIdx.x == 0) { off[b * K + j] = b * n + base; part_start[j] = b * n + base; }
        for (int c0 = 0; c0 < n; c0 += 256) {
            const int i = c0 + threadIdx.x;
            bool f = false;
            if (i < n) {
                int lab = 0;
                float bv = Wb[(size_t)i * K];
                for (int k = 1; k < K; ++k) {
                    const float v = Wb[(size_t)i * K + k];
                    if (v > bv) { bv = v; lab = k; }
                }
                f = lab == j;
                if (f && labels) labels[(size_t)b * n + i] = lab;
            }
            const unsigned long long m = __ballot(f);
            __syncthreads();
            if (lane == 0) wcnt[wave] = __popcll(m);
            __syncthreads();
            int start = base;
            for (int w = 0; w < wave; ++w) start += wcnt[w];
            if (f) {
                const int pos = start + __builtin_amdgcn_mbcnt_hi((unsigned)(m >> 32), __builtin_amdgcn_mbcnt_lo((unsigned)m, 0));
                const size_t row = (size_t)b * n + pos;
                part_index[row] = i;
#pragma unroll
                for (int c = 0; c < 3; ++c) {
                    src[row * 3 + c] = nocs[((size_t)b * n + i) * 3 * K + 3 * j + c];
                    tgt[row * 3 + c] = P[((size_t)b * n + i) * 3 + c];
                }
            }
            base += wcnt[0] + wcnt[1] + wcnt[2] + wcnt[3];
        }
    }
    if (threadIdx.x == 0 && b == gridDim.x - 1) off[gridDim.x * K] = gridDim.x * n;
    if (threadIdx.x == 0) part_start[K] = (b + 1) * n;
    __syncthreads();
    if ((int)threadIdx.x < K && counts) counts[b * K + threadIdx.x] = part_start[threadIdx.x + 1] - part_start[threadIdx.x];
    if ((int)threadIdx.x >= 1 && (int)threadIdx.x < K && rng0 && rng1) {
        const int q = b * (K - 1) + (int)threadIdx.x - 1;
        rng0[q * 2] = part_start[0]; rng0[q * 2 + 1] = part_start[1];
        rng1[q * 2] = part_start[threadIdx.x]; rng1[q * 2 + 1] = part_start[threadIdx.x + 1];
    }
}

template <bool IDX>
__global__ __launch_bounds__(1024) void poison_records_kernel(int n, int K, const float *__restrict__ P, const float *__restrict__ nocs,
                                                              const float *__restrict__ W, const float *__restrict__ axis,
                                                              double *__restrict__ record, int jc, const float *__restrict__ index) {
    const int b = blockIdx.x;
    bool bad = false;
    const auto scan = [&](const float *p, long cnt) {
        for (long i0 = threadIdx.x; i0 < cnt; i0 += 8 * 1024) {
            float v[8];
#pragma unroll
            for (int u = 0; u < 8; ++u) v[u] = p[i0 + u * 1024 < cnt ? i0 + u * 1024 : i0];
#pragma unroll
            for (int u = 0; u < 8; ++u) bad = bad | !(fabsf(v[u]) <= 3.4028234664e38f);
        }
    };
    scan(P + (size_t)b * n * 3, (long)n * 3);
    scan(nocs + (size_t)b * n * 3 * K, (long)n * 3 * K);
    scan(W + (size_t)b * n * K, (long)n * K);
    if (axis) scan(axis + (size_t)b * n * 3, (long)n * 3);
    if (IDX) scan(index + (size_t)b * n * jc, (long)n * jc);
    if (__syncthreads_or(bad))
        for (int i = threadIdx.x; i < K * 26; i += 1024) record[(size_t)b * K * 26 + i] = __builtin_nan("");
}

#define ANCSH_JD_COMPACT(IS_J)                                                                                                        \
    for (int c0 = 0; c0 < n; c0 += 256) {                                                                                             \
        const int i = c0 + threadIdx.x;                                                                                               \
        const bool f = i < n && (IS_J);                                                                                               \
        const unsigned long long m = __ballot(f);                                                                                     \
        __syncthreads();                                                                                                              \
        if (lane == 0) wcnt[wave] = __popcll(m);                                                                                      \
        __syncthreads();                                                                                                              \
        int start = cnt;                                                                                                              \
        for (int w = 0; w < wave; ++w) start += wcnt[w];                                                                              \
        if (f) {                                                                                                                      \
            const int pos = start + __builtin_amdgcn_mbcnt_hi((unsigned)(m >> 32), __builtin_amdgcn_mbcnt_lo((unsigned)m, 0));       \
            _Pragma("unroll") for (int c = 0; c < 3; ++c) vals[c * npow2 + pos] = axis[((size_t)b * n + i) * 3 + c];                 \
        }                                                                                                                             \
        cnt += wcnt[0] + wcnt[1] + wcnt[2] + wcnt[3];                                                                                 \
    }
#define ANCSH_JD_MEDIAN                                                                                                               \
    int p2 = 1;                                                                                                                       \
    while (p2 < cnt) p2 <<= 1;                                                                                                        \
    for (int e = cnt + threadIdx.x; e < p2; e += 256)                                                                                 \
        _Pragma("unroll") for (int c = 0; c < 3; ++c) vals[c * npow2 + e] = INFINITY;                                                 \
    __syncthreads();                                                                                                                  \
    for (int k = 2; k <= p2; k <<= 1)                                                                                                 \
        for (int s = k >> 1; s > 0; s >>= 1) {                                                                                        \
            for (int e = threadIdx.x; e < p2; e += 256) {                                                                             \
                const int partner = e ^ s;                                                                                            \
                if (partner > e) {                                                                                                    \
                    const bool up = (e & k) == 0;                                                                                     \
                    _Pragma("unroll") for (int c = 0; c < 3; ++c) {                                                                   \
                        float *v = vals + c * npow2;                                                                                  \
                        const float a = v[e], bb = v[partner];                                                                       \
                        if ((a > bb) == up) { v[e] = bb; v[partner] = a; }                                                            \
                    }                                                                                                                 \
                }                                                                                                                     \
            }                                                                                                                         \
            __syncthreads();                                                                                                          \
        }                                                                                                                             \
    if (threadIdx.x < 3) {                                                                                                            \
        const float *v = vals + threadIdx.x * npow2;                                                                                  \
        float med = NAN;                                                                                                              \
        if (cnt > 0) med = (cnt & 1) ? v[cnt / 2] : (v[cnt / 2 - 1] + v[cnt / 2]) * 0.5f;                                             \
        out[((size_t)b * (K - 1) + (j - 1)) * 3 + threadIdx.x] = med;                                                                 \
    }

__global__ __launch_bounds__(256) void joint_direction_kernel(int n, int K, const float *__restrict__ axis,
                                                              const int *__restrict__ joint_cls, float *__restrict__ out) {
    extern __shared__ float vals[];
    __shared__ int wcnt[4];
    const int b = blockIdx.x, j = blockIdx.y + 1, lane = threadIdx.x & 63, wave = threadIdx.x >> 6;
    int npow2 = 1;
    while (npow2 < n) npow2 <<= 1;
    int cnt = 0;
    ANCSH_JD_COMPACT(joint_cls[(size_t)b * n + i] == j)
    ANCSH_JD_MEDIAN
}

__device__ __forceinline__ int np_argmax_row(const float *r, int jc) {
    int c = 0;
    float best = r[0];
    for (int k = 1; k < jc && best == best; ++k) {
        const float v = r[k];
        if (!(v <= best)) { best = v; c = k; }
    }
    return c;
}

__global__ __launch_bounds__(256) void joint_direction_pred_kernel(int n, int K, int jc, const float *__restrict__ axis,
                                                                   const float *__restrict__ index, float *__restrict__ out) {
    extern __shared__ float vals[];
    __shared__ int wcnt[4];
    const int b = blockIdx.x, j = blockIdx.y + 1, lane = threadIdx.x & 63, wave = threadIdx.x >> 6;
    int npow2 = 1;
// ... 208 lines not shown
        if (is_in(i)) {
            double sc[3], tc[3];
#pragma unroll
            for (int c = 0; c < 3; ++c) { sc[c] = src[(size_t)(r0 + i) * 3 + c] - sm[c]; tc[c] = tgt[(size_t)(r0 + i) * 3 + c] - tm[c]; }
#pragma unroll
            for (int a = 0; a < 3; ++a)
#pragma unroll
                for (int b = 0; b < 3; ++b) acc[a * 3 + b] += tc[a] * sc[b];
            acc[9] += sc[0] * sc[0] + sc[1] * sc[1] + sc[2] * sc[2];
        }
    block_sum<10>(acc, red, 2);
    if (h != 0) return;
    double M[9], q[4], R[9];
#pragma unroll
    for (int a = 0; a < 9; ++a) M[a] = acc[a] / m;
    horn_quat(M, q);
    quat_to_mat(q, R);
    double trace = 0.0;
#pragma unroll
    for (int a = 0; a < 9; ++a) trace += R[a] * M[a];
    const double s = trace / (acc[9] / m);
    o[0] = o[1] = o[2] = s;
#pragma unroll
    for (int a = 0; a < 3; ++a)
#pragma unroll
        for (int b = 0; b < 3; ++b) o[3 + a * 3 + b] = R[b * 3 + a];
#pragma unroll
    for (int a = 0; a < 3; ++a) {
        const double Tv = tm[a] - s * (R[a * 3] * sm[0] + R[a * 3 + 1] * sm[1] + R[a * 3 + 2] * sm[2]);
        o[12 + a] = Tv;
#pragma unroll
        for (int b = 0; b < 3; ++b) o[15 + a * 4 + b] = s * R[a * 3 + b];
        o[15 + a * 4 + 3] = Tv;
    }
    o[27] = 0; o[28] = 0; o[29] = 0; o[30] = 1; o[31] = bestRatio;
    status[prob] = 0;
}

}
}

using namespace ancsh;
using namespace ancsh::pose;

static float sq_threshold_f32(float th) {
    float t = th * th;
    while (sqrtf(t) >= th && t > 0.f) t = nextafterf(t, 0.f);
    while (sqrtf(t) < th) t = nextafterf(t, INFINITY);
    return t;
}
static double sq_threshold_f64(double th) {
    double t = th * th;
    while (sqrt(t) >= th && t > 0.0) t = nextafter(t, 0.0);
    while (sqrt(t) < th) t = nextafter(t, INFINITY);
    return t;
}

extern "C" int ancsh_pose_partition(int b, int n, int K, const float *W, const float *P, const float *nocs, int *labels,
                                    int *part_index, int *off, float *src, float *tgt, int *counts, int *rng0, int *rng1,
                                    void *stream) {
    ANCSH_REQUIRE(b >= 0 && n > 0 && K >= 1 && K <= 16, "pose_partition: bad shape b=%d n=%d K=%d", b, n, K);
    if (b == 0) return ANCSH_OK;
    ANCSH_REQUIRE(W && P && nocs && part_index && off && src && tgt, "pose_partition: null pointer");
    ANCSH_REQUIRE((rng0 == nullptr) == (rng1 == nullptr), "pose_partition: rng0 and rng1 go together");
    hipLaunchKernelGGL(partition_kernel, dim3(b), dim3(256), 0, (hipStream_t)stream, n, K, W, P, nocs, labels, part_index, off,
                       src, tgt, counts, rng0, rng1);
    return check_launch("pose_partition");
}

extern "C" int ancsh_pose_poison_records(int b, int n, int K, const float *P, const float *nocs, const float *W, const float *joint_axis,
                                         double *record, void *stream) {
    ANCSH_REQUIRE(b >= 0 && n > 0 && K >= 1 && K <= 16, "pose_poison_records: bad shape b=%d n=%d K=%d", b, n, K);
    if (b == 0) return ANCSH_OK;
    ANCSH_REQUIRE(P && nocs && W && record, "pose_poison_records: null pointer");
    hipLaunchKernelGGL(poison_records_kernel<false>, dim3(b), dim3(1024), 0, (hipStream_t)stream, n, K, P, nocs, W, joint_axis, record, 0,
                       nullptr);
    return check_launch("pose_poison_records");
}

extern "C" int ancsh_pose_poison_records_pred(int b, int n, int K, const float *P, const float *nocs, const float *W,
                                              const float *joint_axis, int joint_channels, const float *joint_index, double *record,
                                              void *stream) {
    ANCSH_REQUIRE(b >= 0 && n > 0 && K >= 1 && K <= 16, "pose_poison_records_pred: bad shape b=%d n=%d K=%d", b, n, K);
    ANCSH_REQUIRE(joint_channels >= 1 && joint_channels <= 64, "pose_poison_records_pred: joint_channels=%d must be in [1,64]",
                  joint_channels);
    ANCSH_REQUIRE(P && nocs && W && joint_index && record, "pose_poison_records_pred: null pointer");
    if (b == 0) return ANCSH_OK;
    hipLaunchKernelGGL(poison_records_kernel<true>, dim3(b), dim3(1024), 0, (hipStream_t)stream, n, K, P, nocs, W, joint_axis, record,
                       joint_channels, joint_index);
    return check_launch("pose_poison_records_pred");
}

extern "C" int ancsh_pose_joint_direction(int b, int n, int K, const float *joint_axis, const int *joint_cls, float *out,
                                          void *stream) {
    ANCSH_REQUIRE(b >= 0 && n > 0 && K >= 1, "pose_joint_direction: bad shape");
    ANCSH_REQUIRE(n <= 8192, "pose_joint_direction: n %d > 8192", n);
    if (b == 0 || K == 1) return ANCSH_OK;
    ANCSH_REQUIRE(joint_axis && joint_cls && out, "pose_joint_direction: null pointer");
    int npow2 = 1;
    while (npow2 < n) npow2 <<= 1;
    const size_t lds = (size_t)3 * npow2 * sizeof(float);
    if (lds > 48 * 1024) (void)hipFuncSetAttribute((const void *)joint_direction_kernel, hipFuncAttributeMaxDynamicSharedMemorySize, (int)lds);
    hipLaunchKernelGGL(joint_direction_kernel, dim3(b, K - 1), dim3(256), lds, (hipStream_t)stream, n, K, joint_axis, joint_cls, out);
    return check_launch("pose_joint_direction");
}

extern "C" int ancsh_pose_joint_direction_pred(int b, int n, int K, int joint_channels, const float *joint_axis, const float *joint_index,
                                               float *out, void *stream) {
    ANCSH_REQUIRE(b >= 0 && n > 0 && K >= 2 && K <= 16, "pose_joint_direction_pred: bad shape b=%d n=%d K=%d (K >= 2: a joint)", b, n, K);
    ANCSH_REQUIRE(n <= 8192, "pose_joint_direction_pred: n %d > 8192", n);
    ANCSH_REQUIRE(joint_channels >= 1 && joint_channels <= 64, "pose_joint_direction_pred: joint_channels=%d must be in [1,64]",
                  joint_channels);
    ANCSH_REQUIRE(joint_axis && joint_index && out, "pose_joint_direction_pred: null pointer");
    if (b == 0) return ANCSH_OK;
    int npow2 = 1;
    while (npow2 < n) npow2 <<= 1;
    const size_t lds = (size_t)3 * npow2 * sizeof(float);
    if (lds > 48 * 1024)
        (void)hipFuncSetAttribute((const void *)joint_direction_pred_kernel, hipFuncAttributeMaxDynamicSharedMemorySize, (int)lds);
    hipLaunchKernelGGL(joint_direction_pred_kernel, dim3(b, K - 1), dim3(256), lds, (hipStream_t)stream, n, K, joint_channels, joint_axis,
                       joint_index, out);
    return check_launch("pose_joint_direction_pred");
}

static FitExtras no_extras() {
    FitExtras E;
    E.record = nullptr; E.K = 0; E.tie = nullptr;
    E.lo_f = E.hi_f = 0.f; E.lo_d = E.hi_d = 0.0;
    E.draws = nullptr; E.seed = 0;
    return E;
}

static int make_extras(const char *who, int nprob, double *record, int K, int min_K, int *tie, double th, double window, FitExtras &E) {
    E.record = record; E.K = K; E.tie = tie;
    if (record) {
        ANCSH_REQUIRE(K >= min_K && nprob % (K - (min_K - 1)) == 0, "%s: record needs K >= %d and nprob (%d) a multiple of %s (K = %d)", who, min_K, nprob,
                      min_K == 1 ? "K" : "K - 1", K);
    }
    if (tie) {
        ANCSH_REQUIRE(window >= 0.0 && window < th, "%s: tie_window %g must be in [0, inlier_th)", who, window);
        const double lo = (th - window) * (th - window), hi = (th + window) * (th + window);
        E.lo_f = (float)lo; E.hi_f = (float)hi; E.lo_d = lo; E.hi_d = hi;
    }
    return ANCSH_OK;
}

static long single_quads_needed(long rows, int nprob) { return 2 * ((rows + 7) / 8 + nprob) + 2; }

extern "C" long ancsh_ransac_single_quads_floats(long rows, int nprob) {
    if (rows < 0 || nprob < 0) return -1;
    return 24 * single_quads_needed(rows, nprob);
}

template <int KM>
static int ransac_single_impl(int nprob, const int *off, const float *src, const float *tgt, float inlier_th, int niter,
                              const int *draws, KeyArg<KM> seed, int max_n, double *out_model,
                              unsigned char *out_inliers, int *out_best, int *scratch_scores, float *scratch_quads, long rows,
                              FitExtras E, void *stream) {
    ANCSH_REQUIRE(nprob >= 0 && niter > 0 && max_n > 0, "ransac_single: bad sizes nprob=%d niter=%d max_n=%d", nprob, niter, max_n);
    ANCSH_REQUIRE(max_n <= 6144, "ransac_single: max_n %d > 6144 (refit keeps the inliers in LDS)", max_n);
    if (nprob == 0) return ANCSH_OK;
    ANCSH_REQUIRE(off && src && tgt && out_model && out_inliers && out_best && scratch_scores, "ransac_single: null pointer");
    hipStream_t st = (hipStream_t)stream;
    ANCSH_REQUIRE(inlier_th > 0.f, "ransac_single: inlier_th must be positive");
    inlier_th = sq_threshold_f32(inlier_th);
    if (scratch_quads && inlier_th >= 0x1p-100f && inlier_th < 4.0f) {
        ANCSH_REQUIRE(rows >= 0 && rows < (1L << 30), "ransac_single_ex: rows=%ld out of range", rows);
        ANCSH_REQUIRE((((uintptr_t)scratch_quads) & 31) == 0, "ransac_single_ex: scratch_quads must be 32-byte aligned");
        const int cap = (int)single_quads_needed(rows, nprob);
        hipLaunchKernelGGL(soa_quads_kernel, dim3((max_n + 7 + 255) / 256, nprob), dim3(256), 0, st, off, src, tgt, scratch_quads, cap);
        hipLaunchKernelGGL(ransac_single_score_sreg_kernel<KM>, dim3((niter + 255) / 256, nprob), dim3(256), 0, st, off, src, tgt,
                           (const float *)scratch_quads, cap, inlier_th, niter, draws, seed, scratch_scores);
    } else {
        hipLaunchKernelGGL(ransac_single_score_kernel<KM>, dim3((niter + 255) / 256, nprob), dim3(256), 0, st, off, src, tgt, inlier_th,
                           niter, draws, seed, scratch_scores);
    }
    const size_t lds = 64 * sizeof(double) + 8 * sizeof(int) + (size_t)2 * max_n * 3 * sizeof(float);
    if (lds > 48 * 1024) (void)hipFuncSetAttribute((const void *)ransac_single_finish_kernel<KM>, hipFuncAttributeMaxDynamicSharedMemorySize, (int)lds);
    hipLaunchKernelGGL(ransac_single_finish_kernel<KM>, dim3(nprob), dim3(256), lds, st, off, src, tgt, inlier_th, niter, draws, seed,
                       scratch_scores, max_n, out_model, out_inliers, out_best, E);
    return check_launch("ransac_single");
}

extern "C" int ancsh_ransac_single(int nprob, const int *off, const float *src, const float *tgt, float inlier_th, int niter,
                                   const int *draws, unsigned long long seed, int max_n, double *out_model,
                                   unsigned char *out_inliers, int *out_best, int *scratch_scores, void *stream) {
    return ransac_single_impl<KEY_VALUE>(nprob, off, src, tgt, inlier_th, niter, draws, seed, max_n, out_model, out_inliers, out_best,
                                     scratch_scores, nullptr, 0, no_extras(), stream);
}

extern "C" int ancsh_ransac_single_ex(int nprob, const int *off, const float *src, const float *tgt, float inlier_th, int niter,
                                      const int *draws, unsigned long long seed, int max_n, double *out_model,
                                      unsigned char *out_inliers, int *out_best, int *scratch_scores, float *scratch_quads,
                                      long rows, void *stream) {
    ANCSH_REQUIRE(scratch_quads, "ransac_single_ex: scratch_quads is NULL (ancsh_ransac_single is the call without it)");
    return ransac_single_impl<KEY_VALUE>(nprob, off, src, tgt, inlier_th, niter, draws, seed, max_n, out_model, out_inliers, out_best,
                                     scratch_scores, scratch_quads, rows, no_extras(), stream);
}

extern "C" int ancsh_ransac_single_rec(int nprob, const int *off, const float *src, const float *tgt, float inlier_th, int niter,
                                       const int *draws, unsigned long long seed, int max_n, double *out_model,
                                       unsigned char *out_inliers, int *out_best, int *scratch_scores, float *scratch_quads,
                                       long rows, double *record, int K, int *tie_stats, float tie_window, void *stream) {
    FitExtras E = no_extras();
    if (int rc = make_extras("ransac_single_rec", nprob, record, K, 1, tie_stats, (double)inlier_th, (double)tie_window, E)) return rc;
    return ransac_single_impl<KEY_VALUE>(nprob, off, src, tgt, inlier_th, niter, draws, seed, max_n, out_model, out_inliers, out_best,
                                     scratch_scores, scratch_quads, rows, E, stream);
}

template <int KM>
static int ransac_joint_impl(int nprob, const int *rng0, const int *rng1, const float *src, const float *tgt,
                             const float *joint_dir, double inlier_th, int niter, const int *draws,
                             KeyArg<KM> seed, int max_n, double *out_model, unsigned char *out_inliers,
                             int *out_best, double *out_score, double *scratch_scores, double *scratch_models,
                             int *lm_stat, int lm_schedule, FitExtras E, void *stream, const int *joint_kind = nullptr) {
    ANCSH_REQUIRE(lm_schedule >= ANCSH_LM_AUTO && lm_schedule <= ANCSH_LM_LATENCY, "ransac_joint: unknown lm_schedule %d", lm_schedule);
    ANCSH_REQUIRE(nprob >= 0 && niter > 0 && max_n > 0, "ransac_joint: bad sizes");
    ANCSH_REQUIRE(max_n <= 3072, "ransac_joint: max_n %d > 3072 (refit keeps both parts' inliers in LDS)", max_n);
    if (nprob == 0) return ANCSH_OK;
    ANCSH_REQUIRE(rng0 && rng1 && src && tgt && joint_dir && out_model && out_inliers && out_best && out_score &&
                      scratch_scores && scratch_models, "ransac_joint: null pointer");
    hipStream_t st = (hipStream_t)stream;
    ANCSH_REQUIRE(inlier_th > 0.0, "ransac_joint: inlier_th must be positive");
    inlier_th = sq_threshold_f64(inlier_th);
    const dim3 per_hyp((niter + 63) / 64, nprob);
    hipLaunchKernelGGL(ransac_joint_init_kernel<KM>, per_hyp, dim3(64), 0, st, rng0, rng1, src, tgt, niter, draws, seed, scratch_scores,
                       scratch_models);
    if (lm_schedule == ANCSH_LM_LATENCY) {
        const dim3 grid((niter + COOP_HYP_PER_WAVE - 1) / COOP_HYP_PER_WAVE, nprob);
        if (joint_kind)
            hipLaunchKernelGGL(ransac_joint_lm_coop_kind_kernel<KM>, grid, dim3(64), 0, st, rng0, rng1, src, tgt, joint_dir, niter, draws, seed,
                               scratch_models, lm_stat, joint_kind);
        else
            hipLaunchKernelGGL(ransac_joint_lm_coop_kernel<KM>, grid, dim3(64), 0, st,
                               rng0, rng1, src, tgt, joint_dir, niter, draws, seed, scratch_models, lm_stat);
    } else {
        const int chunk = (long)nprob * niter <= HYP_SMALL_LAUNCH ? HYP_CHUNK_SMALL : HYP_CHUNK;
        if (joint_kind)
            hipLaunchKernelGGL(ransac_joint_lm_kind_kernel<KM>, dim3((niter + chunk - 1) / chunk, nprob), dim3(64), 0, st, rng0, rng1, src, tgt,
                               joint_dir, niter, draws, seed, scratch_models, lm_stat, chunk, joint_kind);
        else
            hipLaunchKernelGGL(ransac_joint_lm_kernel<KM>, dim3((niter + chunk - 1) / chunk, nprob), dim3(64), 0, st, rng0, rng1, src, tgt,
                               joint_dir, niter, draws, seed, scratch_models, lm_stat, chunk);
    }
    hipLaunchKernelGGL(ransac_joint_model_kernel<KM>, per_hyp, dim3(64), 0, st, rng0, rng1, src, tgt, niter, draws, seed, scratch_models);
    hipLaunchKernelGGL(ransac_joint_verify_kernel, dim3((niter + 3) / 4, nprob), dim3(256), 0, st, rng0, rng1, src, tgt, inlier_th,
                       niter, scratch_models, scratch_scores);
    const size_t lds = 128 * sizeof(double) + 8 * sizeof(int) + (size_t)4 * max_n * 3 * sizeof(float);
    if (joint_kind) {
        if (lds > 48 * 1024) (void)hipFuncSetAttribute((const void *)ransac_joint_finish_kind_kernel<KM>, hipFuncAttributeMaxDynamicSharedMemorySize, (int)lds);
        hipLaunchKernelGGL(ransac_joint_finish_kind_kernel<KM>, dim3(nprob), dim3(256), lds, st, rng0, rng1, src, tgt, joint_dir, inlier_th,
                           niter, scratch_scores, scratch_models, max_n, out_model, out_inliers, out_best, out_score, E, joint_kind);
        return check_launch("ransac_joint");
    }
    if (lds > 48 * 1024) (void)hipFuncSetAttribute((const void *)ransac_joint_finish_kernel<KM>, hipFuncAttributeMaxDynamicSharedMemorySize, (int)lds);
    hipLaunchKernelGGL(ransac_joint_finish_kernel<KM>, dim3(nprob), dim3(256), lds, st, rng0, rng1, src, tgt, joint_dir, inlier_th,
                       niter, scratch_scores, scratch_models, max_n, out_model, out_inliers, out_best, out_score, E);
    return check_launch("ransac_joint");
}

static int check_joint_kind(const char *who, int nprob, const int *joint_kind) {
    if (!joint_kind || nprob <= 0) return ANCSH_OK;
    hipPointerAttribute_t at;
    if (hipPointerGetAttributes(&at, joint_kind) != hipSuccess) { (void)hipGetLastError(); return ANCSH_OK; }
    if (at.type != hipMemoryTypeHost) return ANCSH_OK;
    for (int p = 0; p < nprob; ++p)
        ANCSH_REQUIRE(joint_kind[p] == 0 || joint_kind[p] == 1, "%s: joint_kind[%d] = %d (0 revolute, 1 prismatic)", who, p, joint_kind[p]);
    return ANCSH_OK;
}

extern "C" int ancsh_ransac_joint(int nprob, const int *rng0, const int *rng1, const float *src, const float *tgt,
                                  const float *joint_dir, double inlier_th, int niter, const int *draws,
                                  unsigned long long seed, int max_n, double *out_model, unsigned char *out_inliers,
                                  int *out_best, double *out_score, double *scratch_scores, double *scratch_models,
                                  int *lm_stat, void *stream) {
    return ransac_joint_impl<KEY_VALUE>(nprob, rng0, rng1, src, tgt, joint_dir, inlier_th, niter, draws, seed, max_n, out_model, out_inliers,
                                    out_best, out_score, scratch_scores, scratch_models, lm_stat, ANCSH_LM_AUTO, no_extras(), stream);
}

extern "C" int ancsh_ransac_joint_ex(int nprob, const int *rng0, const int *rng1, const float *src, const float *tgt,
                                     const float *joint_dir, double inlier_th, int niter, const int *draws,
                                     unsigned long long seed, int max_n, double *out_model, unsigned char *out_inliers,
                                     int *out_best, double *out_score, double *scratch_scores, double *scratch_models,
                                     int *lm_stat, int lm_schedule, void *stream) {
    return ransac_joint_impl<KEY_VALUE>(nprob, rng0, rng1, src, tgt, joint_dir, inlier_th, niter, draws, seed, max_n, out_model, out_inliers,
                                    out_best, out_score, scratch_scores, scratch_models, lm_stat, lm_schedule, no_extras(), stream);
}

extern "C" int ancsh_ransac_joint_rec(int nprob, const int *rng0, const int *rng1, const float *src, const float *tgt,
                                      const float *joint_dir, double inlier_th, int niter, const int *draws,
                                      unsigned long long seed, int max_n, double *out_model, unsigned char *out_inliers,
                                      int *out_best, double *out_score, double *scratch_scores, double *scratch_models,
                                      int *lm_stat, int lm_schedule, double *record, int K, int *tie_stats, double tie_window,
                                      void *stream) {
    FitExtras E = no_extras();
    if (int rc = make_extras("ransac_joint_rec", nprob, record, K, 2, tie_stats, inlier_th, tie_window, E)) return rc;
    E.draws = draws; E.seed = seed;
    return ransac_joint_impl<KEY_VALUE>(nprob, rng0, rng1, src, tgt, joint_dir, inlier_th, niter, draws, seed, max_n, out_model, out_inliers,
                                    out_best, out_score, scratch_scores, scratch_models, lm_stat, lm_schedule, E, stream);
}

extern "C" int ancsh_ransac_single_rec_dseed(int nprob, const int *off, const float *src, const float *tgt, float inlier_th, int niter,
                                             const int *draws, const unsigned long long *seed, int max_n, double *out_model,
                                             unsigned char *out_inliers, int *out_best, int *scratch_scores, float *scratch_quads,
                                             long rows, double *record, int K, int *tie_stats, float tie_window, void *stream) {
    ANCSH_REQUIRE(seed, "ransac_single_rec_dseed: null seed pointer");
    FitExtras E = no_extras();
    if (int rc = make_extras("ransac_single_rec_dseed", nprob, record, K, 1, tie_stats, (double)inlier_th, (double)tie_window, E)) return rc;
    return ransac_single_impl<KEY_DSEED>(nprob, off, src, tgt, inlier_th, niter, draws, (unsigned long long)(uintptr_t)seed, max_n, out_model,
                                    out_inliers, out_best, scratch_scores, scratch_quads, rows, E, stream);
}

extern "C" int ancsh_ransac_joint_rec_dseed(int nprob, const int *rng0, const int *rng1, const float *src, const float *tgt,
                                            const float *joint_dir, double inlier_th, int niter, const int *draws,
                                            const unsigned long long *seed, int max_n, double *out_model, unsigned char *out_inliers,
                                            int *out_best, double *out_score, double *scratch_scores, double *scratch_models,
                                            int *lm_stat, int lm_schedule, double *record, int K, int *tie_stats, double tie_window,
                                            void *stream) {
    ANCSH_REQUIRE(seed, "ransac_joint_rec_dseed: null seed pointer");
    FitExtras E = no_extras();
    if (int rc = make_extras("ransac_joint_rec_dseed", nprob, record, K, 2, tie_stats, inlier_th, tie_window, E)) return rc;
    E.draws = draws; E.seed = (unsigned long long)(uintptr_t)seed;
    return ransac_joint_impl<KEY_DSEED>(nprob, rng0, rng1, src, tgt, joint_dir, inlier_th, niter, draws, E.seed, max_n, out_model,
                                   out_inliers, out_best, out_score, scratch_scores, scratch_models, lm_stat, lm_schedule, E, stream);
}

extern "C" int ancsh_ransac_single_rec_dkey(int nprob, const int *off, const float *src, const float *tgt, float inlier_th, int niter,
                                            const int *draws, const ancsh_stream_key *key, int max_n, double *out_model,
                                            unsigned char *out_inliers, int *out_best, int *scratch_scores, float *scratch_quads,
                                            long rows, double *record, int K, int *tie_stats, float tie_window, void *stream) {
    ANCSH_REQUIRE(key, "ransac_single_rec_dkey: null key pointer");
    ANCSH_REQUIRE(K >= 1 && nprob >= 0 && nprob % K == 0 && nprob < (1 << 20),
                  "ransac_single_rec_dkey: nprob (%d) must be a multiple of K (%d) below 2^20", nprob, K);
    FitExtras E = no_extras();
    if (int rc = make_extras("ransac_single_rec_dkey", nprob, record, K, 1, tie_stats, (double)inlier_th, (double)tie_window, E)) return rc;
    return ransac_single_impl<KEY_DKEY>(nprob, off, src, tgt, inlier_th, niter, draws, DKey{key, K}, max_n, out_model, out_inliers,
                                        out_best, scratch_scores, scratch_quads, rows, E, stream);
}

extern "C" int ancsh_ransac_joint_rec_dkey(int nprob, const int *rng0, const int *rng1, const float *src, const float *tgt,
                                           const float *joint_dir, double inlier_th, int niter, const int *draws,
                                           const ancsh_stream_key *key, int max_n, double *out_model, unsigned char *out_inliers,
                                           int *out_best, double *out_score, double *scratch_scores, double *scratch_models,
                                           int *lm_stat, int lm_schedule, double *record, int K, int *tie_stats, double tie_window,
                                           void *stream) {
    ANCSH_REQUIRE(key, "ransac_joint_rec_dkey: null key pointer");
    ANCSH_REQUIRE(K >= 2 && nprob >= 0 && nprob % (K - 1) == 0 && nprob < (1 << 20),
                  "ransac_joint_rec_dkey: nprob (%d) must be a multiple of K - 1 (K = %d >= 2) below 2^20", nprob, K);
    FitExtras E = no_extras();
    if (int rc = make_extras("ransac_joint_rec_dkey", nprob, record, K, 2, tie_stats, inlier_th, tie_window, E)) return rc;
    E.draws = draws; E.seed = (unsigned long long)(uintptr_t)key;
    return ransac_joint_impl<KEY_DKEY>(nprob, rng0, rng1, src, tgt, joint_dir, inlier_th, niter, draws, DKey{key, K - 1}, max_n,
                                       out_model, out_inliers, out_best, out_score, scratch_scores, scratch_models, lm_stat, lm_schedule,
                                       E, stream);
}

extern "C" int ancsh_ransac_joint_rec_kind(int nprob, const int *rng0, const int *rng1, const float *src, const float *tgt,
                                           const float *joint_dir, double inlier_th, int niter, const int *draws,
                                           unsigned long long seed, int max_n, double *out_model, unsigned char *out_inliers,
                                           int *out_best, double *out_score, double *scratch_scores, double *scratch_models,
                                           int *lm_stat, int lm_schedule, double *record, int K, int *tie_stats, double tie_window,
                                           const int *joint_kind, void *stream) {
    if (int rc = check_joint_kind("ransac_joint_rec_kind", nprob, joint_kind)) return rc;
    FitExtras E = no_extras();
    if (int rc = make_extras("ransac_joint_rec_kind", nprob, record, K, 2, tie_stats, inlier_th, tie_window, E)) return rc;
    E.draws = draws; E.seed = seed;
    return ransac_joint_impl<KEY_VALUE>(nprob, rng0, rng1, src, tgt, joint_dir, inlier_th, niter, draws, seed, max_n, out_model, out_inliers,
                                        out_best, out_score, scratch_scores, scratch_models, lm_stat, lm_schedule, E, stream, joint_kind);
}

extern "C" int ancsh_ransac_joint_rec_dseed_kind(int nprob, const int *rng0, const int *rng1, const float *src, const float *tgt,
                                                 const float *joint_dir, double inlier_th, int niter, const int *draws,
                                                 const unsigned long long *seed, int max_n, double *out_model,
                                                 unsigned char *out_inliers, int *out_best, double *out_score, double *scratch_scores,
                                                 double *scratch_models, int *lm_stat, int lm_schedule, double *record, int K,
                                                 int *tie_stats, double tie_window, const int *joint_kind, void *stream) {
    ANCSH_REQUIRE(seed, "ransac_joint_rec_dseed_kind: null seed pointer");
    if (int rc = check_joint_kind("ransac_joint_rec_dseed_kind", nprob, joint_kind)) return rc;
    FitExtras E = no_extras();
    if (int rc = make_extras("ransac_joint_rec_dseed_kind", nprob, record, K, 2, tie_stats, inlier_th, tie_window, E)) return rc;
    E.draws = draws; E.seed = (unsigned long long)(uintptr_t)seed;
    return ransac_joint_impl<KEY_DSEED>(nprob, rng0, rng1, src, tgt, joint_dir, inlier_th, niter, draws, E.seed, max_n, out_model,
                                        out_inliers, out_best, out_score, scratch_scores, scratch_models, lm_stat, lm_schedule, E, stream,
                                        joint_kind);
}

extern "C" int ancsh_ransac_joint_rec_dkey_kind(int nprob, const int *rng0, const int *rng1, const float *src, const float *tgt,
                                                const float *joint_dir, double inlier_th, int niter, const int *draws,
                                                const ancsh_stream_key *key, int max_n, double *out_model, unsigned char *out_inliers,
                                                int *out_best, double *out_score, double *scratch_scores, double *scratch_models,
                                                int *lm_stat, int lm_schedule, double *record, int K, int *tie_stats,
                                                double tie_window, const int *joint_kind, void *stream) {
    ANCSH_REQUIRE(key, "ransac_joint_rec_dkey_kind: null key pointer");
    ANCSH_REQUIRE(K >= 2 && nprob >= 0 && nprob % (K - 1) == 0 && nprob < (1 << 20),
                  "ransac_joint_rec_dkey_kind: nprob (%d) must be a multiple of K - 1 (K = %d >= 2) below 2^20", nprob, K);
    if (int rc = check_joint_kind("ransac_joint_rec_dkey_kind", nprob, joint_kind)) return rc;
    FitExtras E = no_extras();
    if (int rc = make_extras("ransac_joint_rec_dkey_kind", nprob, record, K, 2, tie_stats, inlier_th, tie_window, E)) return rc;
    E.draws = draws; E.seed = (unsigned long long)(uintptr_t)key;
    return ransac_joint_impl<KEY_DKEY>(nprob, rng0, rng1, src, tgt, joint_dir, inlier_th, niter, draws, DKey{key, K - 1}, max_n,
                                       out_model, out_inliers, out_best, out_score, scratch_scores, scratch_models, lm_stat, lm_schedule,
                                       E, stream, joint_kind);
}

extern "C" int ancsh_umeyama(int nprob, const int *off, const float *src, const float *tgt, double *out, void *stream) {
    ANCSH_REQUIRE(nprob >= 0, "umeyama: negative nprob");
    if (nprob == 0) return ANCSH_OK;
    ANCSH_REQUIRE(off && src && tgt && out, "umeyama: null pointer");
    hipLaunchKernelGGL(umeyama_kernel, dim3(nprob), dim3(256), 0, (hipStream_t)stream, off, src, tgt, out);
    return check_launch("umeyama");
}

extern "C" int ancsh_estimate_similarity_transform(int nprob, const int *off, const float *src, const float *tgt, int niter,
                                                   const int *draws, unsigned long long seed, double *out, int *status,
                                                   void *stream) {
    ANCSH_REQUIRE(nprob >= 0 && niter > 0 && niter <= 128, "estimate_similarity_transform: niter %d outside 1..128", niter);
    if (nprob == 0) return ANCSH_OK;
    ANCSH_REQUIRE(off && src && tgt && out && status, "estimate_similarity_transform: null pointer");
    hipLaunchKernelGGL(ransac_umeyama5_kernel, dim3(nprob), dim3(128), 0, (hipStream_t)stream, off, src, tgt, niter, draws, seed,
                       out, status);
    return check_launch("estimate_similarity_transform");
}
```

### articulated-pose_amd/pose/parallel_ancsh_pose.py

```python
import os
import pickle

import numpy as np
import torch

from .. import _lib
from .d3_utils import rot_diff_degree


def _i32(t, dev):
    if torch.is_tensor(t):
        return t.to(dev, torch.int32).contiguous()
    return torch.from_numpy(np.ascontiguousarray(t, np.int32)).to(dev)


def _f32(t, dev):
    if torch.is_tensor(t):
        return t.to(dev, torch.float32).contiguous()
    return torch.from_numpy(np.ascontiguousarray(t, np.float32)).to(dev)


TIE_WINDOW = 32 * 2.0 ** -27


def ransac_single_batch(off, src, tgt, inlier_th, niter, draws=None, seed=0, max_n=None, scalar_points=True, record=None, K=0,
                        tie_window=None, seed_dev=None, key_dev=None):
    dev = src.device
    nprob = off.numel() - 1
    rows = src.shape[0]
    max_n = int(max_n or rows)
    model = torch.empty((nprob, 13), dtype=torch.float64, device=dev)
    inl = torch.empty((rows,), dtype=torch.uint8, device=dev)
    best = torch.empty((nprob, 2), dtype=torch.int32, device=dev)
    scores = torch.empty((nprob * niter,), dtype=torch.int32, device=dev)
    d = None if draws is None else _i32(draws, dev)
    if d is not None and d.numel() != nprob * niter * 3:
        raise ValueError("draws must have shape (nprob, niter, 3)")
    quads, tie = None, None
    if scalar_points:
        quads = torch.empty((_lib.lib().ancsh_ransac_single_quads_floats(rows, nprob),), dtype=torch.float32, device=dev)
    if key_dev is not None or seed_dev is not None:
        tie = torch.empty((nprob, 2), dtype=torch.int32, device=dev) if tie_window is not None else None
        _lib.call("ancsh_ransac_single_rec_dkey" if key_dev is not None else "ancsh_ransac_single_rec_dseed", nprob, _lib.ptr(off),
                  _lib.ptr(src), _lib.ptr(tgt), float(inlier_th), int(niter), _lib.ptr(d), _lib.ptr(key_dev if key_dev is not None else seed_dev),
                  max_n, _lib.ptr(model), _lib.ptr(inl), _lib.ptr(best), _lib.ptr(scores), _lib.ptr(quads),
                  rows, _lib.ptr(record), int(K), _lib.ptr(tie), float(tie_window or 0.0))
    elif record is not None or tie_window is not None:
        tie = torch.empty((nprob, 2), dtype=torch.int32, device=dev) if tie_window is not None else None
        _lib.call("ancsh_ransac_single_rec", nprob, _lib.ptr(off), _lib.ptr(src), _lib.ptr(tgt), float(inlier_th), int(niter),
                  _lib.ptr(d), int(seed), max_n, _lib.ptr(model), _lib.ptr(inl), _lib.ptr(best), _lib.ptr(scores), _lib.ptr(quads), rows,
                  _lib.ptr(record), int(K), _lib.ptr(tie), float(tie_window or 0.0))
    elif scalar_points:
        _lib.call("ancsh_ransac_single_ex", nprob, _lib.ptr(off), _lib.ptr(src), _lib.ptr(tgt), float(inlier_th), int(niter),
                  _lib.ptr(d), int(seed), max_n, _lib.ptr(model), _lib.ptr(inl), _lib.ptr(best), _lib.ptr(scores), _lib.ptr(quads), rows)
    else:
        _lib.call("ancsh_ransac_single", nprob, _lib.ptr(off), _lib.ptr(src), _lib.ptr(tgt), float(inlier_th), int(niter),
                  _lib.ptr(d), int(seed), max_n, _lib.ptr(model), _lib.ptr(inl), _lib.ptr(best), _lib.ptr(scores))
    return dict(model=model, inliers=inl, best=best, scores=scores.view(nprob, niter), tie=tie, _keep=(d, scores, quads))


LM_SCHEDULES = {"auto": 0, "throughput": 1, "latency": 2}
JOINT_KINDS = {"revolute": 0, "prismatic": 1}


def check_joint_types(joint_types, num_parts):
    if joint_types is None:
        return None
    nj = max(int(num_parts) - 1, 0)
    if isinstance(joint_types, str):
        if joint_types not in JOINT_KINDS:
            raise ValueError("joint_types must be one of %s, got %r" % (tuple(JOINT_KINDS), joint_types))
        return (JOINT_KINDS[joint_types],) * nj
    if not isinstance(joint_types, (list, tuple)):
        raise ValueError("joint_types must be None, one of %s, or a sequence of %d of them (one per joint), got %r"
                         % (tuple(JOINT_KINDS), nj, joint_types))
    if len(joint_types) != nj:
        raise ValueError("joint_types must name the %d joints of a %d-part object, got %d entries: %r"
                         % (nj, num_parts, len(joint_types), list(joint_types)))
    for j, t in enumerate(joint_types):
        if not isinstance(t, str) or t not in JOINT_KINDS:
            raise ValueError("joint_types[%d] (joint %d) must be one of %s, got %r" % (j, j + 1, tuple(JOINT_KINDS), t))
    return tuple(JOINT_KINDS[t] for t in joint_types)


def joint_kind_tensor(kinds, B, device):
    if kinds is None:
        return None
    return torch.tensor(list(kinds) * int(B), dtype=torch.int32).to(device)


def ransac_joint_batch(rng0, rng1, src, tgt, joint_dir, inlier_th, niter, draws=None, seed=0, max_n=None, want_lm_stat=False,
                       lm_schedule="auto", record=None, K=0, tie_window=None, seed_dev=None, key_dev=None, joint_kind=None):
    dev = src.device
    nprob = rng0.shape[0]
    max_n = int(max_n or src.shape[0])
    model = torch.empty((nprob, 26), dtype=torch.float64, device=dev)
    inl = torch.empty((nprob, 2, max_n), dtype=torch.uint8, device=dev)
    best = torch.empty((nprob,), dtype=torch.int32, device=dev)
    score = torch.empty((nprob,), dtype=torch.float64, device=dev)
    sc = torch.empty((nprob * niter,), dtype=torch.float64, device=dev)
    mo = torch.empty((nprob * niter, 26), dtype=torch.float64, device=dev)
    stat = torch.empty((nprob, niter, 2), dtype=torch.int32, device=dev) if want_lm_stat else None
    d = None if draws is None else _i32(draws, dev)
    if d is not None and d.numel() != nprob * niter * 6:
        raise ValueError("draws must have shape (nprob, niter, 6)")
    tie = None
    if joint_kind is not None:
        if joint_kind.dtype != torch.int32 or joint_kind.numel() != nprob or not joint_kind.is_contiguous():
            raise ValueError("joint_kind must be a contiguous int32 tensor of %d entries (one per problem)" % nprob)
        tie = torch.empty((nprob, 2), dtype=torch.int32, device=dev) if tie_window is not None else None
        name, key = (("ancsh_ransac_joint_rec_dkey_kind", _lib.ptr(key_dev)) if key_dev is not None else
                     ("ancsh_ransac_joint_rec_dseed_kind", _lib.ptr(seed_dev)) if seed_dev is not None else
                     ("ancsh_ransac_joint_rec_kind", int(seed)))
        _lib.call(name, nprob, _lib.ptr(rng0), _lib.ptr(rng1), _lib.ptr(src), _lib.ptr(tgt), _lib.ptr(joint_dir), float(inlier_th),
                  int(niter), _lib.ptr(d), key, max_n, _lib.ptr(model), _lib.ptr(inl), _lib.ptr(best), _lib.ptr(score), _lib.ptr(sc),
                  _lib.ptr(mo), _lib.ptr(stat), LM_SCHEDULES[lm_schedule], _lib.ptr(record), int(K), _lib.ptr(tie),
                  float(tie_window or 0.0), _lib.ptr(joint_kind))
    elif key_dev is not None or seed_dev is not None:
        tie = torch.empty((nprob, 2), dtype=torch.int32, device=dev) if tie_window is not None else None
        _lib.call("ancsh_ransac_joint_rec_dkey" if key_dev is not None else "ancsh_ransac_joint_rec_dseed", nprob, _lib.ptr(rng0),
                  _lib.ptr(rng1), _lib.ptr(src), _lib.ptr(tgt), _lib.ptr(joint_dir), float(inlier_th), int(niter), _lib.ptr(d),
                  _lib.ptr(key_dev if key_dev is not None else seed_dev), max_n, _lib.ptr(model), _lib.ptr(inl), _lib.ptr(best),
                  _lib.ptr(score), _lib.ptr(sc), _lib.ptr(mo), _lib.ptr(stat), LM_SCHEDULES[lm_schedule], _lib.ptr(record), int(K),
                  _lib.ptr(tie), float(tie_window or 0.0))
    elif record is not None or tie_window is not None:
        tie = torch.empty((nprob, 2), dtype=torch.int32, device=dev) if tie_window is not None else None
        _lib.call("ancsh_ransac_joint_rec", nprob, _lib.ptr(rng0), _lib.ptr(rng1), _lib.ptr(src), _lib.ptr(tgt), _lib.ptr(joint_dir),
                  float(inlier_th), int(niter), _lib.ptr(d), int(seed), max_n, _lib.ptr(model), _lib.ptr(inl), _lib.ptr(best),
                  _lib.ptr(score), _lib.ptr(sc), _lib.ptr(mo), _lib.ptr(stat), LM_SCHEDULES[lm_schedule], _lib.ptr(record), int(K),
                  _lib.ptr(tie), float(tie_window or 0.0))
    else:
        _lib.call("ancsh_ransac_joint_ex", nprob, _lib.ptr(rng0), _lib.ptr(rng1), _lib.ptr(src), _lib.ptr(tgt), _lib.ptr(joint_dir),
                  float(inlier_th), int(niter), _lib.ptr(d), int(seed), max_n, _lib.ptr(model), _lib.ptr(inl), _lib.ptr(best),
                  _lib.ptr(score), _lib.ptr(sc), _lib.ptr(mo), _lib.ptr(stat), LM_SCHEDULES[lm_schedule])
    return dict(model=model, inliers=inl, best=best, score=score, lm_stat=stat, hyp_models=mo, hyp_scores=sc, tie=tie, _keep=(d, joint_kind))


def draws_from_seed(seed, counts, niter_a, niter_b):
    rs = np.random.RandomState(seed)
    K = len(counts)
    da = np.zeros((K, niter_a, 3), np.int32)
    for j in range(K):
        for i in range(niter_a):
            da[j, i] = rs.randint(counts[j], size=3)
    db = np.zeros((max(K - 1, 0), niter_b, 6), np.int32)
    for j in range(1, K):
        for i in range(niter_b):
            db[j - 1, i, :3] = rs.randint(counts[0], size=3)
            db[j - 1, i, 3:] = rs.randint(counts[j], size=3)
    return da, db


class PoseSolver(object):

    def __init__(self, num_parts, inlier_th=0.1, niter_a=10000, niter_b=200, device="cuda:0", want_lm_stat=False,
                 max_part_points=None, lm_schedule="auto", tie_window=TIE_WINDOW, joint_types=None):
        kinds = check_joint_types(joint_types, num_parts)
        self.joint_kinds = kinds if kinds is not None and any(kinds) else None
        self._kind_dev = {}
        self.K, self.th, self.niter_a, self.niter_b = num_parts, inlier_th, niter_a, niter_b
        self.tie_window = tie_window
        self.device = torch.device(device)
        self.max_part_points = max_part_points
        if lm_schedule not in LM_SCHEDULES:
            raise ValueError("lm_schedule must be one of %s" % sorted(LM_SCHEDULES))
        self.lm_schedule = lm_schedule
        self.want_lm_stat = want_lm_stat

    def prepare(self, B):
        if self.joint_kinds is None or self.K < 2:
            return None
        if B not in self._kind_dev:
            self._kind_dev[B] = joint_kind_tensor(self.joint_kinds, B, self.device)
        return self._kind_dev[B]

    def solve(self, P, nocs_pred, mask_pred, joint_axis_per_point, joint_cls=None, draws_a=None, draws_b=None, seed=0, seed_dev=None,
              key_dev=None, joint_index=None):
        _one_association(joint_cls, joint_index)
        out = self._partition(P, nocs_pred, mask_pred)
        self._stage_b_fits(out, joint_axis_per_point, joint_cls, draws_b, seed, seed_dev, key_dev, joint_index)
        return self._poison(self._stage_a_fits(out, draws_a, seed, seed_dev, key_dev))

    def solve_stage_a(self, P, nocs_pred, mask_pred, draws_a=None, seed=0):
        out = self._partition(P, nocs_pred, mask_pred)
        if self.K > 1:
            out["record"][:, :, 13:] = float("nan")
        return self._poison(self._stage_a_fits(out, draws_a, seed))

    def _poison(self, out):
        B, N = out["_shape"]
        P, nocs, W = out["_inputs"]
        axis = out.get("_axis")
        index = out.get("_index")
        if index is not None:
            _lib.call("ancsh_pose_poison_records_pred", B, N, self.K, _lib.ptr(P), _lib.ptr(nocs), _lib.ptr(W), _lib.ptr(axis),
                      int(index.shape[2]), _lib.ptr(index), _lib.ptr(out["record"]))
        else:
            _lib.call("ancsh_pose_poison_records", B, N, self.K, _lib.ptr(P), _lib.ptr(nocs), _lib.ptr(W), _lib.ptr(axis),
                      _lib.ptr(out["record"]))
        return out

    def _partition(self, P, nocs_pred, mask_pred):
        dev, K = self.device, self.K
        P, nocs, W = _f32(P, dev), _f32(nocs_pred, dev), _f32(mask_pred, dev)
        B, N, _ = P.shape
        if nocs.shape != (B, N, 3 * K) or W.shape != (B, N, K):
            raise ValueError("nocs_pred must be (B,N,3K) and mask_pred (B,N,K)")
        max_n = min(N, self.max_part_points or N)
        labels = torch.empty((B, N), dtype=torch.int32, device=dev)
        pidx = torch.empty((B, N), dtype=torch.int32, device=dev)
        off = torch.empty((B * K + 1,), dtype=torch.int32, device=dev)
        src = torch.empty((B * N, 3), dtype=torch.float32, device=dev)
        tgt = torch.empty((B * N, 3), dtype=torch.float32, device=dev)
        counts = torch.empty((B, K), dtype=torch.int32, device=dev)
        rng0 = torch.empty((B * max(K - 1, 1), 2), dtype=torch.int32, device=dev) if K > 1 else None
        rng1 = torch.empty((B * max(K - 1, 1), 2), dtype=torch.int32, device=dev) if K > 1 else None
        _lib.call("ancsh_pose_partition", B, N, K, _lib.ptr(W), _lib.ptr(P), _lib.ptr(nocs), _lib.ptr(labels), _lib.ptr(pidx),
                  _lib.ptr(off), _lib.ptr(src), _lib.ptr(tgt), _lib.ptr(counts), _lib.ptr(rng0), _lib.ptr(rng1))
        record = torch.empty((B, K, 26), dtype=torch.float64, device=dev)
        return dict(labels=labels, part_index=pidx, off=off, counts=counts, record=record, _src=src, _tgt=tgt, _max_n=max_n, _shape=(B, N),
                    _rng=(rng0, rng1), _inputs=(P, nocs, W))

    def _stage_a_fits(self, out, draws_a=None, seed=0, seed_dev=None, key_dev=None):
        dev, K = self.device, self.K
        B, N = out["_shape"]
        a = ransac_single_batch(out["off"], out["_src"], out["_tgt"], self.th, self.niter_a,
                                None if draws_a is None else _i32(draws_a, dev).reshape(B * K, self.niter_a, 3), seed, out["_max_n"],
                                record=out["record"], K=K, tie_window=self.tie_window, seed_dev=seed_dev, key_dev=key_dev)
        out.update(baseline=out["record"][:, :, :13], best_a=a["best"].view(B, K, 2), inliers_a=a["inliers"].view(B, N))
        if a["tie"] is not None:
            out["tie_a"] = a["tie"].view(B, K, 2)
        if K == 1:
            out["nonlinear"] = out["record"][:, :, 13:]
        return out

    def solve_stage_b(self, out, joint_axis_per_point, joint_cls=None, draws_b=None, seed=0, seed_dev=None, key_dev=None,
                      joint_index=None):
        _one_association(joint_cls, joint_index)
        return self._poison(self._stage_b_fits(out, joint_axis_per_point, joint_cls, draws_b, seed, seed_dev, key_dev, joint_index))

    def _stage_b_fits(self, out, joint_axis_per_point, joint_cls, draws_b=None, seed=0, seed_dev=None, key_dev=None, joint_index=None):
        dev, K = self.device, self.K
        B, N = out["_shape"]
        src, tgt, max_n = out["_src"], out["_tgt"], out["_max_n"]
        rng0, rng1 = out["_rng"]
        if K > 1:
            axis = _f32(joint_axis_per_point, dev)
            out["_axis"] = axis
            jdir = torch.empty((B, K - 1, 3), dtype=torch.float32, device=dev)
            if joint_index is not None:
                index = _f32(joint_index, dev)
                if index.dim() != 3 or tuple(index.shape[:2]) != (B, N):
                    raise ValueError("joint_index must be (B, N, C) for %d clouds of %d points, got %s" % (B, N, tuple(index.shape)))
                out["_index"] = index
                _lib.call("ancsh_pose_joint_direction_pred", B, N, K, int(index.shape[2]), _lib.ptr(axis), _lib.ptr(index), _lib.ptr(jdir))
            else:
                jcls = _i32(joint_cls, dev)
                _lib.call("ancsh_pose_joint_direction", B, N, K, _lib.ptr(axis), _lib.ptr(jcls), _lib.ptr(jdir))
            b = ransac_joint_batch(rng0, rng1, src, tgt, jdir.view(-1, 3), self.th, self.niter_b,
                                   None if draws_b is None else _i32(draws_b, dev).reshape(B * (K - 1), self.niter_b, 6),
                                   seed + 1, max_n, want_lm_stat=self.want_lm_stat, lm_schedule=self.lm_schedule,
                                   record=out["record"], K=K, tie_window=self.tie_window, seed_dev=seed_dev, key_dev=key_dev,
                                   joint_kind=self.prepare(B))
            if self.want_lm_stat:
                out["lm_stat"] = b["lm_stat"].view(B, K - 1, self.niter_b, 2)
            out["nonlinear"] = out["record"][:, :, 13:]
            if b["tie"] is not None:
                out["tie_b"] = b["tie"].view(B, K - 1, 2)
            out["best_b"] = b["best"].view(B, K - 1)
            out["score_b"] = b["score"].view(B, K - 1)
            out["joint_direction"] = jdir
            out["inliers_b"] = b["inliers"].view(B, K - 1, 2, max_n)
        else:
            out["nonlinear"] = out["record"][:, :, 13:]
        return out


def _one_association(joint_cls, joint_index):
    if (joint_cls is None) == (joint_index is None):
        raise ValueError("give exactly one of joint_cls (a label per point) and joint_index (the index_per_point head), got %s"
                         % ("both" if joint_cls is not None else "neither"))


def _model_to_rst(m):
    return m[:9].reshape(3, 3), m[9], m[10:13]


def records_from_solution(sol, rts_list=None):
    base = sol["baseline"].cpu().numpy()
    nonl = sol["nonlinear"].cpu().numpy()
    B, K, _ = base.shape
    recs = []
    for b in range(B):
        scale_dict = {'gt': [], 'baseline': [], 'nonlinear': []}
        r_dict = {'gt': [], 'baseline': [], 'nonlinear': []}
        t_dict = {'gt': [], 'baseline': [], 'nonlinear': []}
        xyz_err = {'baseline': [], 'nonlinear': []}
        rpy_err = {'baseline': [], 'nonlinear': []}
        scale_err = {'baseline': [], 'nonlinear': []}
        for j in range(K):
            for kind, arr in (('baseline', base), ('nonlinear', nonl)):
                R, s, t = _model_to_rst(arr[b, j])
                scale_dict[kind].append(s)
                r_dict[kind].append(R)
                t_dict[kind].append(t)
                if rts_list is not None:
                    rt_gt, s_gt = rts_list[b]['rt']['gt'][j], rts_list[b]['scale']['gt'][j]
                    rpy_err[kind].append(rot_diff_degree(R, rt_gt[:3, :3]))
                    xyz_err[kind].append(np.linalg.norm(t - rt_gt[:3, 3]))
                    scale_err[kind].append(np.linalg.norm(s - s_gt[0]))
            if rts_list is not None:
                scale_dict['gt'].append(rts_list[b]['scale']['gt'][j][0])
                r_dict['gt'].append(rts_list[b]['rt']['gt'][j][:3, :3])
                t_dict['gt'].append(rts_list[b]['rt']['gt'][j][:3, 3])
        recs.append({'scale': scale_dict, 'rotation': r_dict, 'translation': t_dict, 'xyz_err': xyz_err,
                     'rpy_err': rpy_err, 'scale_err': scale_err})
    return recs


JOINT_SOURCES = ("gt", "predicted")


def solver_ransac_nonlinear(s_ind, e_ind, test_exp, baseline_exp, choose_threshold, num_parts, test_group, problem_ins,
                            rts_all, file_name, base_path=None, batch_size=32, seed=0, device="cuda:0", joint_source="gt",
                            joint_types=None):
    if joint_source not in JOINT_SOURCES:
        raise ValueError("joint_source must be one of %s, got %r" % (JOINT_SOURCES, joint_source))
    check_joint_types(joint_types, num_parts)
    from .. import prediction_io
    base_path = base_path or os.environ.get("ANCSH_BASE_PATH", ".")
    solver = PoseSolver(num_parts, choose_threshold, device=device, joint_types=joint_types)
    names = [test_group[i].split('.')[0] for i in range(s_ind, e_ind) if test_group[i].split('_')[0] not in problem_ins]
    all_rts = {}
    for c0 in range(0, len(names), batch_size):
        chunk = names[c0:c0 + batch_size]
        f = [prediction_io.load_record(os.path.join(base_path, 'results/test_pred', str(test_exp)), n) for n in chunk]
        fb = [prediction_io.load_record(os.path.join(base_path, 'results/test_pred', str(baseline_exp)), n) for n in chunk]
        sol = solver.solve(np.stack([r['P'][:, :3] for r in f]), np.stack([r['nocs_per_point'] for r in fb]),
                           np.stack([r['instance_per_point'] for r in fb]), np.stack([r['joint_axis_per_point'] for r in f]),
                           **({"joint_index": np.stack([r['index_per_point'] for r in f])} if joint_source == "predicted" else
                              {"joint_cls": np.stack([r['joint_cls_gt'] for r in f])}), seed=seed + c0)
        gts = [rts_all[n] for n in chunk] if rts_all is not None else None
        for n, rec in zip(chunk, records_from_solution(sol, gts)):
            all_rts[n] = rec
    with open(file_name, 'wb') as fh:
        pickle.dump(all_rts, fh)
    return all_rts
```

### include/ancsh_hip.h

```cpp
#ifndef ANCSH_HIP_H
#define ANCSH_HIP_H

#ifdef __cplusplus
extern "C" {
#endif

#define ANCSH_OK 0
#define ANCSH_EINVAL (-1)
#define ANCSH_EHIP (-2)

#define ANCSH_ACT_NONE 0
#define ANCSH_ACT_RELU 1
#define ANCSH_MAX_GROUPS 4
#define ANCSH_ACT_RAW 2

int ancsh_abi_version(void);
const char *ancsh_last_error(void);


int ancsh_farthest_point_sample(int b, int n, int m, const float *inp, float *temp, int *out, void *stream);

int ancsh_farthest_point_sample_gather(int b, int n, int m, const float *inp, float *temp, int *out_idx, float *out_xyz,
                                       void *stream);

// ... 118 lines not shown
                    void *stream);

int ancsh_mlp_chain_grouped(int ngroups, long rows, int cin, const float *x, int ldx, const int *nops, const int *const *ops,
                            const void *const *const *ptrs, float *scratch, void *stream);

int ancsh_sa3_chain_grouped(int ngroups, int b, int npts, int cfeat, int c1, int c2, int c3, const float *xyz, const float *feats,
                            const float *const *params, float *out, void *stream);
int ancsh_fp_single_source_init(int ngroups, int b, int cin, int cout, int nparts, const float *x, const float *const *w, float *y,
                                void *stream);
int ancsh_fp1_chain_grouped(int ngroups, int b, int npts, int cskip, int c1, int c2, const float *skip, const float *init,
                            const float *const *params, float *out, void *stream);
int ancsh_fp2_chain_grouped(int ngroups, int b, int m, int n, int c2, int c1, int n1, int n2, const float *points2, const int *idx,
                            const float *weight, const float *points1, const float *const *params, float *out, void *stream);

int ancsh_last_ball_query_schedule(void);

int ancsh_mlp_chain_grouped_fp(int ngroups, int b, int n, int m, int c2, const float *points2, const int *idx, const float *weight,
                               const float *xyz, const int *nops, const int *const *ops, const void *const *const *ptrs, float *scratch,
                               void *stream);

int ancsh_mlp_chain_grouped_fp_bf16x3(int ngroups, int b, int n, int m, int c2, const float *points2, const int *idx, const float *weight,
                                      const float *xyz, const int *nops, const int *const *ops, const void *const *const *ptrs,
                                      void *stream);
int ancsh_mlp_chain_grouped_fp_f16x2(int ngroups, int b, int n, int m, int c2, const float *points2, const int *idx, const float *weight,
                                     const float *xyz, const int *nops, const int *const *ops, const void *const *const *ptrs,
                                     void *stream);
int ancsh_mlp_chain_grouped_fp_f16x2_guarded(int ngroups, int b, int n, int m, int c2, const float *points2, const int *idx, const float *weight,
                                             const float *xyz, const int *nops, const int *const *ops, const void *const *const *ptrs,
                                             unsigned *range_flags, int flag_bit0, void *stream);

int ancsh_sa3_chain_grouped_bf16x3(int ngroups, int b, int npts, int cfeat, int c1, int c2, int c3, const float *xyz, const float *feats,
                                   const float *const *params, float *out, void *stream);
int ancsh_sa3_chain_grouped_f16x2(int ngroups, int b, int npts, int cfeat, int c1, int c2, int c3, const float *xyz, const float *feats,
                                  const float *const *params, float *out, void *stream);
int ancsh_fp1_chain_grouped_bf16x3(int ngroups, int b, int npts, int cskip, int c1, int c2, const float *skip, const float *init,
                                   const float *const *params, float *out, void *stream);
int ancsh_fp1_chain_grouped_f16x2(int ngroups, int b, int npts, int cskip, int c1, int c2, const float *skip, const float *init,
                                  const float *const *params, float *out, void *stream);
int ancsh_fp2_chain_grouped_bf16x3(int ngroups, int b, int m, int n, int c2, int c1, int n1, int n2, const float *points2, const int *idx,
                                   const float *weight, const float *points1, const float *const *params, float *out, void *stream);
int ancsh_fp2_chain_grouped_f16x2(int ngroups, int b, int m, int n, int c2, int c1, int n1, int n2, const float *points2, const int *idx,
                                  const float *weight, const float *points1, const float *const *params, float *out, void *stream);
int ancsh_sa3_chain_grouped_f16x2_guarded(int ngroups, int b, int npts, int cfeat, int c1, int c2, int c3, const float *xyz, const float *feats,
                                          const float *const *params, float *out, unsigned *range_flags, int flag_bit0, void *stream);
int ancsh_fp1_chain_grouped_f16x2_guarded(int ngroups, int b, int npts, int cskip, int c1, int c2, const float *skip, const float *init,
                                          const float *const *params, float *out, unsigned *range_flags, int flag_bit0, void *stream);
int ancsh_fp2_chain_grouped_f16x2_guarded(int ngroups, int b, int m, int n, int c2, int c1, int n1, int n2, const float *points2, const int *idx,
                                          const float *weight, const float *points1, const float *const *params, float *out,
                                          unsigned *range_flags, int flag_bit0, void *stream);

int ancsh_group_max(long groups, int nsample, int c, const float *x, float *y, void *stream);

int ancsh_head_activations(long rows, int K, int mixed_pred, const float *logits, int ld, float *W, float *nocs,
                           float *confi, float *heatmap, float *unitvec, float *axis, float *joint_cls,
                           float *gocs, float *scale, float *trans, void *stream);


int ancsh_pose_partition(int b, int n, int K, const float *W, const float *P, const float *nocs, int *labels,
                         int *part_index, int *off, float *src, float *tgt, int *counts, int *rng0, int *rng1, void *stream);

int ancsh_pose_poison_records(int b, int n, int K, const float *P, const float *nocs, const float *W, const float *joint_axis,
                              double *record, void *stream);

int ancsh_pose_poison_records_pred(int b, int n, int K, const float *P, const float *nocs, const float *W, const float *joint_axis,
                                   int joint_channels, const float *joint_index, double *record, void *stream);

int ancsh_pose_joint_direction(int b, int n, int K, const float *joint_axis, const int *joint_cls, float *out,
                               void *stream);

int ancsh_pose_joint_direction_pred(int b, int n, int K, int joint_channels, const float *joint_axis, const float *joint_index,
                                    float *out, void *stream);

int ancsh_ransac_single(int nprob, const int *off, const float *src, const float *tgt, float inlier_th, int niter,
                        const int *draws, unsigned long long seed, int max_n, double *out_model,
                        unsigned char *out_inliers, int *out_best, int *scratch_scores, void *stream);

long ancsh_ransac_single_quads_floats(long rows, int nprob);
int ancsh_ransac_single_ex(int nprob, const int *off, const float *src, const float *tgt, float inlier_th, int niter,
                           const int *draws, unsigned long long seed, int max_n, double *out_model,
                           unsigned char *out_inliers, int *out_best, int *scratch_scores, float *scratch_quads, long rows,
                           void *stream);

int ancsh_ransac_single_rec(int nprob, const int *off, const float *src, const float *tgt, float inlier_th, int niter,
                            const int *draws, unsigned long long seed, int max_n, double *out_model, unsigned char *out_inliers,
                            int *out_best, int *scratch_scores, float *scratch_quads, long rows, double *record, int K,
                            int *tie_stats, float tie_window, void *stream);

int ancsh_ransac_joint(int nprob, const int *rng0, const int *rng1, const float *src, const float *tgt,
                       const float *joint_dir, double inlier_th, int niter, const int *draws,
                       unsigned long long seed, int max_n, double *out_model, unsigned char *out_inliers,
                       int *out_best, double *out_score, double *scratch_scores, double *scratch_models,
                       int *lm_stat, void *stream);

#define ANCSH_LM_AUTO 0
#define ANCSH_LM_THROUGHPUT 1
#define ANCSH_LM_LATENCY 2
int ancsh_ransac_joint_ex(int nprob, const int *rng0, const int *rng1, const float *src, const float *tgt,
                          const float *joint_dir, double inlier_th, int niter, const int *draws,
                          unsigned long long seed, int max_n, double *out_model, unsigned char *out_inliers,
                          int *out_best, double *out_score, double *scratch_scores, double *scratch_models,
                          int *lm_stat, int lm_schedule, void *stream);

int ancsh_ransac_joint_rec(int nprob, const int *rng0, const int *rng1, const float *src, const float *tgt,
                           const float *joint_dir, double inlier_th, int niter, const int *draws, unsigned long long seed,
                           int max_n, double *out_model, unsigned char *out_inliers, int *out_best, double *out_score,
                           double *scratch_scores, double *scratch_models, int *lm_stat, int lm_schedule, double *record, int K,
                           int *tie_stats, double tie_window, void *stream);

int ancsh_ransac_single_rec_dseed(int nprob, const int *off, const float *src, const float *tgt, float inlier_th, int niter,
                                  const int *draws, const unsigned long long *seed, int max_n, double *out_model,
                                  unsigned char *out_inliers, int *out_best, int *scratch_scores, float *scratch_quads, long rows,
                                  double *record, int K, int *tie_stats, float tie_window, void *stream);
int ancsh_ransac_joint_rec_dseed(int nprob, const int *rng0, const int *rng1, const float *src, const float *tgt,
                                 const float *joint_dir, double inlier_th, int niter, const int *draws, const unsigned long long *seed,
                                 int max_n, double *out_model, unsigned char *out_inliers, int *out_best, double *out_score,
                                 double *scratch_scores, double *scratch_models, int *lm_stat, int lm_schedule, double *record, int K,
                                 int *tie_stats, double tie_window, void *stream);

typedef struct {
    unsigned long long seed;
    int cloud_base;
    int reserved;
} ancsh_stream_key;

int ancsh_ransac_single_rec_dkey(int nprob, const int *off, const float *src, const float *tgt, float inlier_th, int niter,
                                 const int *draws, const ancsh_stream_key *key, int max_n, double *out_model,
                                 unsigned char *out_inliers, int *out_best, int *scratch_scores, float *scratch_quads, long rows,
                                 double *record, int K, int *tie_stats, float tie_window, void *stream);
int ancsh_ransac_joint_rec_dkey(int nprob, const int *rng0, const int *rng1, const float *src, const float *tgt,
                                const float *joint_dir, double inlier_th, int niter, const int *draws, const ancsh_stream_key *key,
                                int max_n, double *out_model, unsigned char *out_inliers, int *out_best, double *out_score,
                                double *scratch_scores, double *scratch_models, int *lm_stat, int lm_schedule, double *record, int K,
                                int *tie_stats, double tie_window, void *stream);

#define ANCSH_JOINT_REVOLUTE 0
#define ANCSH_JOINT_PRISMATIC 1
int ancsh_ransac_joint_rec_kind(int nprob, const int *rng0, const int *rng1, const float *src, const float *tgt,
                                const float *joint_dir, double inlier_th, int niter, const int *draws, unsigned long long seed,
                                int max_n, double *out_model, unsigned char *out_inliers, int *out_best, double *out_score,
                                double *scratch_scores, double *scratch_models, int *lm_stat, int lm_schedule, double *record, int K,
                                int *tie_stats, double tie_window, const int *joint_kind, void *stream);
int ancsh_ransac_joint_rec_dseed_kind(int nprob, const int *rng0, const int *rng1, const float *src, const float *tgt,
                                      const float *joint_dir, double inlier_th, int niter, const int *draws,
                                      const unsigned long long *seed, int max_n, double *out_model, unsigned char *out_inliers,
                                      int *out_best, double *out_score, double *scratch_scores, double *scratch_models, int *lm_stat,
                                      int lm_schedule, double *record, int K, int *tie_stats, double tie_window, const int *joint_kind,
                                      void *stream);
int ancsh_ransac_joint_rec_dkey_kind(int nprob, const int *rng0, const int *rng1, const float *src, const float *tgt,
                                     const float *joint_dir, double inlier_th, int niter, const int *draws, const ancsh_stream_key *key,
                                     int max_n, double *out_model, unsigned char *out_inliers, int *out_best, double *out_score,
                                     double *scratch_scores, double *scratch_models, int *lm_stat, int lm_schedule, double *record, int K,
                                     int *tie_stats, double tie_window, const int *joint_kind, void *stream);

int ancsh_umeyama(int nprob, const int *off, const float *src, const float *tgt, double *out, void *stream);

int ancsh_estimate_similarity_transform(int nprob, const int *off, const float *src, const float *tgt, int niter,
                                        const int *draws, unsigned long long seed, double *out, int *status, void *stream);

int ancsh_iou_3d(int npairs, int nres, const double *bbox1, const double *bbox2, double *iou, long *counts, void *stream);

int ancsh_joint_params(int b, int n, int K, int gocs_channels, int axis_mean, const float *gocs, const float *nocs,
                       const float *mask, const float *heatmap, const float *unitvec, const float *joint_axis,
                       const int *joint_cls, double *st, double *joint, void *stream);

int ancsh_part_extents(int b, int n, int K, int nocs_channels, const float *nocs, const float *mask, const float *P, int ldp,
                       const double *pose0, float *scale_pred, double *dynam, int *count, void *stream);

#define ANCSH_ARTICULATION_MAX_N 4096
int ancsh_articulation_rec(int b, int n, int K, int gocs_channels, int joint_channels, const float *gocs, const float *nocs,
                           const float *mask, const float *heatmap, const float *unitvec, const float *joint_axis,
                           const float *joint_index, const float *npcs_nocs, const float *npcs_mask, const double *record,
                           double *art, double *joint_nocs, double *st0, float *extent, void *stream);

int ancsh_joint_state_rec(int b, int n, int K, const float *P, int ldp, const float *npcs_nocs, const float *npcs_mask,
                          const double *record, const double *art, double *wide, void *stream);


int ancsh_input_sample(int nclouds, int num_points, int nchan, const float *rows, const int *offsets, const int *perm,
                       const float *norm_factor, int cls_col, int jcls_col, int n_parts, float *P, float *chan_out,
                       float *mask_array, float *joint_cls_mask, void *stream);

int ancsh_input_sample_stream(int nclouds, int num_points, int nchan, const float *rows, long capacity, const int *offsets,
                              const float *norm_factor, int jcls_col, const unsigned long long *seed, float *P, int *joint_cls,
                              int *perm_out, void *stream);

int ancsh_input_sample_stream_keyed(int nclouds, int num_points, int nchan, const float *rows, long capacity, const int *offsets,
                                    const float *norm_factor, int jcls_col, const ancsh_stream_key *key, float *P, int *joint_cls,
                                    int *perm_out, void *stream);

int ancsh_input_sample_stream_xyz(int nclouds, int num_points, int nchan, const float *rows, long capacity, const int *offsets,
                                  const float *norm_factor, const unsigned long long *seed, float *P, int *perm_out, void *stream);
int ancsh_input_sample_stream_xyz_keyed(int nclouds, int num_points, int nchan, const float *rows, long capacity, const int *offsets,
                                        const float *norm_factor, const ancsh_stream_key *key, float *P, int *perm_out, void *stream);

#define ANCSH_DEPTH_U16 0
#define ANCSH_DEPTH_F32 1
#define ANCSH_DEPTH_MAX_CHUNKS 64
int ancsh_depth_unproject_stream(int nclouds, int depth_type, const void *depth, const unsigned char *mask, long pixel_capacity,
                                 const int *geom, const float *cam, float *rows, long capacity, int *offsets, int *counts, int *scratch,
                                 void *stream);

#define ANCSH_LABEL_NAN_BITS 0x7fc00000u
int ancsh_depth_label_images(int nclouds, int depth_type, const void *depth, const unsigned char *mask, long pixel_capacity,
                             const int *geom, const int *offsets, const int *scratch, const int *labels, const float *values,
                             long capacity, const int *dest, int *img_labels, float *img_values, long image_capacity, void *stream);

int ancsh_raw_point_labels(int nclouds, int num_points, int K, int gocs_channels, int nchan, const float *rows, long capacity,
                           const int *offsets, const float *norm_factor, const float *P, const float *W, const float *nocs,
                           const float *gocs, int *labels, float *values, void *stream);


int ancsh_test_losses(int b, int n, int K, int type_l, const void *const *ptrs, float *out, void *stream);

#ifdef __cplusplus
}
#endif
#endif
```

Baseline: 17920.

## Fuse single-part and joint RANSAC finish stages into one paired launch

Adds a paired RANSAC entry point that runs the single-part and joint scoring and then launches one combined finish kernel. Blocks below nprob_a do the single-part refit and the rest do the joint refit. The goal is fewer kernel launches and host round trips, and letting the two independent fits share the GPU at the same time. In exchange, the combined kernel must reserve the larger joint LDS footprint for every block, which may lower occupancy for the single-part blocks. It also adds a new API surface and Python plumbing.

```diff
diff --git a/articulated-pose_amd/_lib.py b/articulated-pose_amd/_lib.py
--- a/articulated-pose_amd/_lib.py
+++ b/articulated-pose_amd/_lib.py
@@ -110,6 +110,18 @@
     "ancsh_depth_unproject_stream": [_c_int, _c_int, _vp, _vp, _c_long, _vp, _vp, _vp, _c_long, _vp, _vp, _vp, _vp],
     "ancsh_depth_label_images": [_c_int, _c_int, _vp, _vp, _c_long] + [_vp] * 5 + [_c_long, _vp, _vp, _vp, _c_long, _vp],
     "ancsh_joint_state_rec": [_c_int] * 3 + [_vp, _c_int] + [_vp] * 5 + [_vp],
+    "ancsh_ransac_pair_rec": [_vp, _vp, _c_int, _vp, _c_int]
+                             + [_c_int, _vp, _c_float, _c_int, _vp, ctypes.c_ulonglong, _vp, _vp, _vp, _vp, _vp, _c_long, _vp, _c_float]
+                             + [_c_int, _vp, _vp, _vp, ctypes.c_double, _c_int, _vp, ctypes.c_ulonglong] + [_vp] * 7
+                             + [_c_int, _vp, ctypes.c_double, _vp, _vp],
+    "ancsh_ransac_pair_rec_dseed": [_vp, _vp, _c_int, _vp, _c_int]
+                                   + [_c_int, _vp, _c_float, _c_int, _vp, _vp, _vp, _vp, _vp, _vp, _vp, _c_long, _vp, _c_float]
+                                   + [_c_int, _vp, _vp, _vp, ctypes.c_double, _c_int, _vp] + [_vp] * 7
+                                   + [_c_int, _vp, ctypes.c_double, _vp, _vp],
+    "ancsh_ransac_pair_rec_dkey": [_vp, _vp, _c_int, _vp, _c_int]
+                                  + [_c_int, _vp, _c_float, _c_int, _vp, _vp, _vp, _vp, _vp, _vp, _vp, _c_long, _vp, _c_float]
+                                  + [_c_int, _vp, _vp, _vp, ctypes.c_double, _c_int, _vp] + [_vp] * 7
+                                  + [_c_int, _vp, ctypes.c_double, _vp, _vp],
     "ancsh_input_sample": [_c_int, _c_int, _c_int, _vp, _vp, _vp, _vp, _c_int, _c_int, _c_int, _vp, _vp, _vp, _vp, _vp],
     "ancsh_test_losses": [_c_int, _c_int, _c_int, _c_int, _vp, _vp, _vp],
     "ancsh_ransac_joint_ex": [_c_int, _vp, _vp, _vp, _vp, _vp, ctypes.c_double, _c_int, _vp, ctypes.c_ulonglong, _c_int]
diff --git a/articulated-pose_amd/csrc/pose.hip b/articulated-pose_amd/csrc/pose.hip
--- a/articulated-pose_amd/csrc/pose.hip
+++ b/articulated-pose_amd/csrc/pose.hip
@@ -438,13 +438,13 @@
 }
 
 template <int KM>
-__global__ __launch_bounds__(256) void ransac_single_finish_kernel(const int *__restrict__ off, const float *__restrict__ src,
-                                                                   const float *__restrict__ tgt, float th, int niter,
-                                                                   const int *__restrict__ draws, KeyArg<KM> seed_arg,
-                                                                   const int *__restrict__ scores, int max_n,
-                                                                   double *__restrict__ out_model,
-                                                                   unsigned char *__restrict__ out_inliers,
-                                                                   int *__restrict__ out_best, FitExtras E) {
+__device__ __forceinline__ void ransac_single_finish_run(const int *off, const float *src,
+                                                         const float *tgt, float th, int niter,
+                                                         const int *draws, KeyArg<KM> seed_arg,
+                                                         const int *scores, int max_n,
+                                                         double *out_model,
+                                                         unsigned char *out_inliers,
+                                                         int *out_best, const FitExtras &E, int prob) {
     const unsigned long long seed = kernel_seed<KM>(seed_arg, 0);
     const int kbase = key_problem_base<KM>(seed_arg);
     extern __shared__ __attribute__((aligned(16))) unsigned char smem[];
@@ -452,7 +452,6 @@
     int *wcnt = (int *)(red + 64);
     float(*cs)[3] = (float(*)[3])(wcnt + 8);
     float(*ct)[3] = cs + max_n;
-    const int prob = blockIdx.x;
     const int r0 = off[prob], n = off[prob + 1] - r0;
     double *om = out_model + (size_t)prob * MODEL_A;
     if (n <= 0 || n > max_n) {
@@ -576,6 +575,17 @@
     }
 }
 
+template <int KM>
+__global__ __launch_bounds__(256) void ransac_single_finish_kernel(const int *__restrict__ off, const float *__restrict__ src,
+                                                                   const float *__restrict__ tgt, float th, int niter,
+                                                                   const int *__restrict__ draws, KeyArg<KM> seed_arg,
+                                                                   const int *__restrict__ scores, int max_n,
+                                                                   double *__restrict__ out_model,
+                                                                   unsigned char *__restrict__ out_inliers,
+                                                                   int *__restrict__ out_best, FitExtras E) {
+    ransac_single_finish_run<KM>(off, src, tgt, th, niter, draws, seed_arg, scores, max_n, out_model, out_inliers, out_best, E, blockIdx.x);
+}
+
 struct PartFd {
     Rod b, p[3];
     double rh[3];
@@ -840,6 +850,7 @@
 constexpr int HYP_CHUNK = 256;
 constexpr int HYP_CHUNK_SMALL = 64;
 constexpr long HYP_SMALL_LAUNCH = 8192;
+constexpr long HYP_WAVES_AT_ONCE = 1024;
 constexpr int HYP_REFILL = 16;
 
 template <int KM, bool PRISM>
@@ -1318,14 +1329,13 @@
                                                         double *__restrict__ out_model,
                                                         unsigned char *__restrict__ out_inliers,
                                                         int *__restrict__ out_best, double *__restrict__ out_score, const FitExtras &E,
-                                                        unsigned char *smem) {
+                                                        int prob, unsigned char *smem) {
     double *red = (double *)smem;
     int *wcnt = (int *)(red + 128);
     float(*c0s)[3] = (float(*)[3])(wcnt + 8);
     float(*c0t)[3] = c0s + max_n;
     float(*c1s)[3] = c0t + max_n;
     float(*c1t)[3] = c1s + max_n;
-    const int prob = blockIdx.x;
     const int a0 = rng0[prob * 2], n0 = rng0[prob * 2 + 1] - a0;
     const int a1 = rng1[prob * 2], n1 = rng1[prob * 2 + 1] - a1;
     double *om = out_model + (size_t)prob * MODEL_B;
@@ -1465,7 +1475,7 @@
                                                                   int *__restrict__ out_best, double *__restrict__ out_score, FitExtras E) {
     extern __shared__ __attribute__((aligned(16))) unsigned char smem[];
     ransac_joint_finish_run<KM, false>(rng0, rng1, src, tgt, joint_dir, th, niter, scores, models, max_n, out_model, out_inliers, out_best,
-                                       out_score, E, smem);
+                                       out_score, E, blockIdx.x, smem);
 }
 
 template <int KM>
@@ -1481,10 +1491,57 @@
     extern __shared__ __attribute__((aligned(16))) unsigned char smem[];
     if (joint_kind[blockIdx.x] != 0)
         ransac_joint_finish_run<KM, true>(rng0, rng1, src, tgt, joint_dir, th, niter, scores, models, max_n, out_model, out_inliers, out_best,
-                                          out_score, E, smem);
+                                          out_score, E, blockIdx.x, smem);
     else
         ransac_joint_finish_run<KM, false>(rng0, rng1, src, tgt, joint_dir, th, niter, scores, models, max_n, out_model, out_inliers, out_best,
-                                           out_score, E, smem);
+                                           out_score, E, blockIdx.x, smem);
+}
+
+template <int KM>
+__global__ __launch_bounds__(256) void ransac_finish_pair_kernel(int nprob_a, const float *__restrict__ src, const float *__restrict__ tgt, int max_n,
+                                                                 const int *__restrict__ off, float th_a, int niter_a,
+                                                                 const int *__restrict__ draws_a, KeyArg<KM> seed_a,
+                                                                 const int *__restrict__ scores_a, double *__restrict__ out_model_a,
+                                                                 unsigned char *__restrict__ out_inliers_a, int *__restrict__ out_best_a,
+                                                                 FitExtras EA,
+                                                                 const int *__restrict__ rng0, const int *__restrict__ rng1,
+                                                                 const float *__restrict__ joint_dir, double th_b, int niter_b,
+                                                                 const double *__restrict__ scores_b, const double *__restrict__ models,
+                                                                 double *__restrict__ out_model_b, unsigned char *__restrict__ out_inliers_b,
+                                                                 int *__restrict__ out_best_b, double *__restrict__ out_score_b, FitExtras EB) {
+    extern __shared__ __attribute__((aligned(16))) unsigned char smem[];
+    if ((int)blockIdx.x < nprob_a)
+        ransac_single_finish_run<KM>(off, src, tgt, th_a, niter_a, draws_a, seed_a, scores_a, max_n, out_model_a, out_inliers_a, out_best_a, EA,
+                                     blockIdx.x);
+    else
+        ransac_joint_finish_run<KM, false>(rng0, rng1, src, tgt, joint_dir, th_b, niter_b, scores_b, models, max_n, out_model_b, out_inliers_b,
+                                           out_best_b, out_score_b, EB, (int)blockIdx.x - nprob_a, smem);
+}
+
+template <int KM>
+__global__ __launch_bounds__(256) void ransac_finish_pair_kind_kernel(int nprob_a, const float *__restrict__ src, const float *__restrict__ tgt,
+                                                                      int max_n, const int *__restrict__ off, float th_a, int niter_a,
+                                                                      const int *__restrict__ draws_a, KeyArg<KM> seed_a,
+                                                                      const int *__restrict__ scores_a, double *__restrict__ out_model_a,
+                                                                      unsigned char *__restrict__ out_inliers_a, int *__restrict__ out_best_a,
+                                                                      FitExtras EA,
+                                                                      const int *__restrict__ rng0, const int *__restrict__ rng1,
+                                                                      const float *__restrict__ joint_dir, double th_b, int niter_b,
+                                                                      const double *__restrict__ scores_b, const double *__restrict__ models,
+                                                                      double *__restrict__ out_model_b, unsigned char *__restrict__ out_inliers_b,
+                                                                      int *__restrict__ out_best_b, double *__restrict__ out_score_b, FitExtras EB,
+                                                                      const int *__restrict__ joint_kind) {
+    extern __shared__ __attribute__((aligned(16))) unsigned char smem[];
+    const int prob_b = (int)blockIdx.x - nprob_a;
+    if (prob_b < 0)
+        ransac_single_finish_run<KM>(off, src, tgt, th_a, niter_a, draws_a, seed_a, scores_a, max_n, out_model_a, out_inliers_a, out_best_a, EA,
+                                     blockIdx.x);
+    else if (joint_kind[prob_b] != 0)
+        ransac_joint_finish_run<KM, true>(rng0, rng1, src, tgt, joint_dir, th_b, niter_b, scores_b, models, max_n, out_model_b, out_inliers_b,
+                                          out_best_b, out_score_b, EB, prob_b, smem);
+    else
+        ransac_joint_finish_run<KM, false>(rng0, rng1, src, tgt, joint_dir, th_b, niter_b, scores_b, models, max_n, out_model_b, out_inliers_b,
+                                           out_best_b, out_score_b, EB, prob_b, smem);
 }
 
 __global__ __launch_bounds__(256) void partition_kernel(int n, int K, const float *__restrict__ W, const float *__restrict__ P,
@@ -1999,21 +2056,28 @@
     return 24 * single_quads_needed(rows, nprob);
 }
 
-template <int KM>
-static int ransac_single_impl(int nprob, const int *off, const float *src, const float *tgt, float inlier_th, int niter,
-                              const int *draws, KeyArg<KM> seed, int max_n, double *out_model,
-                              unsigned char *out_inliers, int *out_best, int *scratch_scores, float *scratch_quads, long rows,
-                              FitExtras E, void *stream) {
+static int ransac_single_check(int nprob, const int *off, const float *src, const float *tgt, float inlier_th, int niter, int max_n,
+                               const double *out_model, const unsigned char *out_inliers, const int *out_best, const int *scratch_scores,
+                               const float *scratch_quads, long rows) {
     ANCSH_REQUIRE(nprob >= 0 && niter > 0 && max_n > 0, "ransac_single: bad sizes nprob=%d niter=%d max_n=%d", nprob, niter, max_n);
     ANCSH_REQUIRE(max_n <= 6144, "ransac_single: max_n %d > 6144 (refit keeps the inliers in LDS)", max_n);
     if (nprob == 0) return ANCSH_OK;
     ANCSH_REQUIRE(off && src && tgt && out_model && out_inliers && out_best && scratch_scores, "ransac_single: null pointer");
-    hipStream_t st = (hipStream_t)stream;
     ANCSH_REQUIRE(inlier_th > 0.f, "ransac_single: inlier_th must be positive");
     inlier_th = sq_threshold_f32(inlier_th);
     if (scratch_quads && inlier_th >= 0x1p-100f && inlier_th < 4.0f) {
         ANCSH_REQUIRE(rows >= 0 && rows < (1L << 30), "ransac_single_ex: rows=%ld out of range", rows);
         ANCSH_REQUIRE((((uintptr_t)scratch_quads) & 31) == 0, "ransac_single_ex: scratch_quads must be 32-byte aligned");
+    }
+    return ANCSH_OK;
+}
+
+template <int KM>
+static float ransac_single_score(int nprob, const int *off, const float *src, const float *tgt, float inlier_th, int niter,
+                                 const int *draws, KeyArg<KM> seed, int max_n, int *scratch_scores, float *scratch_quads, long rows,
+                                 hipStream_t st) {
+    inlier_th = sq_threshold_f32(inlier_th);
+    if (scratch_quads && inlier_th >= 0x1p-100f && inlier_th < 4.0f) {
         const int cap = (int)single_quads_needed(rows, nprob);
         hipLaunchKernelGGL(soa_quads_kernel, dim3((max_n + 7 + 255) / 256, nprob), dim3(256), 0, st, off, src, tgt, scratch_quads, cap);
         hipLaunchKernelGGL(ransac_single_score_sreg_kernel<KM>, dim3((niter + 255) / 256, nprob), dim3(256), 0, st, off, src, tgt,
@@ -2022,7 +2086,23 @@
         hipLaunchKernelGGL(ransac_single_score_kernel<KM>, dim3((niter + 255) / 256, nprob), dim3(256), 0, st, off, src, tgt, inlier_th,
                            niter, draws, seed, scratch_scores);
     }
-    const size_t lds = 64 * sizeof(double) + 8 * sizeof(int) + (size_t)2 * max_n * 3 * sizeof(float);
+    return inlier_th;
+}
+
+static size_t single_finish_lds(int max_n) { return 64 * sizeof(double) + 8 * sizeof(int) + (size_t)2 * max_n * 3 * sizeof(float); }
+static size_t joint_finish_lds(int max_n) { return 128 * sizeof(double) + 8 * sizeof(int) + (size_t)4 * max_n * 3 * sizeof(float); }
+
+template <int KM>
+static int ransac_single_impl(int nprob, const int *off, const float *src, const float *tgt, float inlier_th, int niter,
+                              const int *draws, KeyArg<KM> seed, int max_n, double *out_model,
+                              unsigned char *out_inliers, int *out_best, int *scratch_scores, float *scratch_quads, long rows,
+                              FitExtras E, void *stream) {
+    if (int rc = ransac_single_check(nprob, off, src, tgt, inlier_th, niter, max_n, out_model, out_inliers, out_best, scratch_scores,
+                                     scratch_quads, rows)) return rc;
+    if (nprob == 0) return ANCSH_OK;
+    hipStream_t st = (hipStream_t)stream;
+    inlier_th = ransac_single_score<KM>(nprob, off, src, tgt, inlier_th, niter, draws, seed, max_n, scratch_scores, scratch_quads, rows, st);
+    const size_t lds = single_finish_lds(max_n);
     if (lds > 48 * 1024) (void)hipFuncSetAttribute((const void *)ransac_single_finish_kernel<KM>, hipFuncAttributeMaxDynamicSharedMemorySize, (int)lds);
     hipLaunchKernelGGL(ransac_single_finish_kernel<KM>, dim3(nprob), dim3(256), lds, st, off, src, tgt, inlier_th, niter, draws, seed,
                        scratch_scores, max_n, out_model, out_inliers, out_best, E);
@@ -2055,20 +2135,30 @@
                                      scratch_scores, scratch_quads, rows, E, stream);
 }
 
-template <int KM>
-static int ransac_joint_impl(int nprob, const int *rng0, const int *rng1, const float *src, const float *tgt,
-                             const float *joint_dir, double inlier_th, int niter, const int *draws,
-                             KeyArg<KM> seed, int max_n, double *out_model, unsigned char *out_inliers,
-                             int *out_best, double *out_score, double *scratch_scores, double *scratch_models,
-                             int *lm_stat, int lm_schedule, FitExtras E, void *stream, const int *joint_kind = nullptr) {
+static int ransac_joint_check(int nprob, const int *rng0, const int *rng1, const float *src, const float *tgt, const float *joint_dir,
+                              double inlier_th, int niter, int max_n, const double *out_model, const unsigned char *out_inliers,
+                              const int *out_best, const double *out_score, const double *scratch_scores, const double *scratch_models,
+                              int lm_schedule) {
     ANCSH_REQUIRE(lm_schedule >= ANCSH_LM_AUTO && lm_schedule <= ANCSH_LM_LATENCY, "ransac_joint: unknown lm_schedule %d", lm_schedule);
     ANCSH_REQUIRE(nprob >= 0 && niter > 0 && max_n > 0, "ransac_joint: bad sizes");
     ANCSH_REQUIRE(max_n <= 3072, "ransac_joint: max_n %d > 3072 (refit keeps both parts' inliers in LDS)", max_n);
     if (nprob == 0) return ANCSH_OK;
     ANCSH_REQUIRE(rng0 && rng1 && src && tgt && joint_dir && out_model && out_inliers && out_best && out_score &&
                       scratch_scores && scratch_models, "ransac_joint: null pointer");
-    hipStream_t st = (hipStream_t)stream;
     ANCSH_REQUIRE(inlier_th > 0.0, "ransac_joint: inlier_th must be positive");
+    return ANCSH_OK;
+}
+
+static int lm_chunk(int nprob, int niter, int lm_schedule) {
+    if (lm_schedule == ANCSH_LM_THROUGHPUT) return (long)nprob * niter <= HYP_SMALL_LAUNCH ? HYP_CHUNK_SMALL : HYP_CHUNK;
+    return (long)nprob * ((niter + HYP_CHUNK_SMALL - 1) / HYP_CHUNK_SMALL) <= HYP_WAVES_AT_ONCE ? HYP_CHUNK_SMALL : HYP_CHUNK;
+}
+
+template <int KM>
+static double ransac_joint_hypotheses(int nprob, const int *rng0, const int *rng1, const float *src, const float *tgt,
+                                      const float *joint_dir, double inlier_th, int niter, const int *draws, KeyArg<KM> seed,
+                                      double *scratch_scores, double *scratch_models, int *lm_stat, int lm_schedule,
+                                      const int *joint_kind, hipStream_t st) {
     inlier_th = sq_threshold_f64(inlier_th);
     const dim3 per_hyp((niter + 63) / 64, nprob);
     hipLaunchKernelGGL(ransac_joint_init_kernel<KM>, per_hyp, dim3(64), 0, st, rng0, rng1, src, tgt, niter, draws, seed, scratch_scores,
@@ -2082,7 +2172,7 @@
             hipLaunchKernelGGL(ransac_joint_lm_coop_kernel<KM>, grid, dim3(64), 0, st,
                                rng0, rng1, src, tgt, joint_dir, niter, draws, seed, scratch_models, lm_stat);
     } else {
-        const int chunk = (long)nprob * niter <= HYP_SMALL_LAUNCH ? HYP_CHUNK_SMALL : HYP_CHUNK;
+        const int chunk = lm_chunk(nprob, niter, lm_schedule);
         if (joint_kind)
             hipLaunchKernelGGL(ransac_joint_lm_kind_kernel<KM>, dim3((niter + chunk - 1) / chunk, nprob), dim3(64), 0, st, rng0, rng1, src, tgt,
                                joint_dir, niter, draws, seed, scratch_models, lm_stat, chunk, joint_kind);
@@ -2093,7 +2183,22 @@
     hipLaunchKernelGGL(ransac_joint_model_kernel<KM>, per_hyp, dim3(64), 0, st, rng0, rng1, src, tgt, niter, draws, seed, scratch_models);
     hipLaunchKernelGGL(ransac_joint_verify_kernel, dim3((niter + 3) / 4, nprob), dim3(256), 0, st, rng0, rng1, src, tgt, inlier_th,
                        niter, scratch_models, scratch_scores);
-    const size_t lds = 128 * sizeof(double) + 8 * sizeof(int) + (size_t)4 * max_n * 3 * sizeof(float);
+    return inlier_th;
+}
+
+template <int KM>
+static int ransac_joint_impl(int nprob, const int *rng0, const int *rng1, const float *src, const float *tgt,
+                             const float *joint_dir, double inlier_th, int niter, const int *draws,
+                             KeyArg<KM> seed, int max_n, double *out_model, unsigned char *out_inliers,
+                             int *out_best, double *out_score, double *scratch_scores, double *scratch_models,
+                             int *lm_stat, int lm_schedule, FitExtras E, void *stream, const int *joint_kind = nullptr) {
+    if (int rc = ransac_joint_check(nprob, rng0, rng1, src, tgt, joint_dir, inlier_th, niter, max_n, out_model, out_inliers, out_best,
+                                    out_score, scratch_scores, scratch_models, lm_schedule)) return rc;
+    if (nprob == 0) return ANCSH_OK;
+    hipStream_t st = (hipStream_t)stream;
+    inlier_th = ransac_joint_hypotheses<KM>(nprob, rng0, rng1, src, tgt, joint_dir, inlier_th, niter, draws, seed, scratch_scores,
+                                            scratch_models, lm_stat, lm_schedule, joint_kind, st);
+    const size_t lds = joint_finish_lds(max_n);
     if (joint_kind) {
         if (lds > 48 * 1024) (void)hipFuncSetAttribute((const void *)ransac_joint_finish_kind_kernel<KM>, hipFuncAttributeMaxDynamicSharedMemorySize, (int)lds);
         hipLaunchKernelGGL(ransac_joint_finish_kind_kernel<KM>, dim3(nprob), dim3(256), lds, st, rng0, rng1, src, tgt, joint_dir, inlier_th,
@@ -2250,6 +2355,112 @@
                                        E, stream, joint_kind);
 }
 
+template <int KM>
+static int ransac_pair_impl(const char *who, const float *src, const float *tgt, int max_n, double *record, int K,
+                            int nprob_a, const int *off, float inlier_th_a, int niter_a, const int *draws_a, KeyArg<KM> seed_a,
+                            double *out_model_a, unsigned char *out_inliers_a, int *out_best_a, int *scratch_scores_a,
+                            float *scratch_quads, long rows, int *tie_stats_a, float tie_window_a,
+                            int nprob_b, const int *rng0, const int *rng1, const float *joint_dir, double inlier_th_b, int niter_b,
+                            const int *draws_b, KeyArg<KM> seed_b, unsigned long long tie_seed_b, double *out_model_b,
+                            unsigned char *out_inliers_b, int *out_best_b, double *out_score_b, double *scratch_scores_b,
+                            double *scratch_models, int *lm_stat, int lm_schedule, int *tie_stats_b, double tie_window_b,
+                            const int *joint_kind, void *stream) {
+    if (int rc = ransac_single_check(nprob_a, off, src, tgt, inlier_th_a, niter_a, max_n, out_model_a, out_inliers_a, out_best_a,
+                                     scratch_scores_a, scratch_quads, rows)) return rc;
+    if (int rc = ransac_joint_check(nprob_b, rng0, rng1, src, tgt, joint_dir, inlier_th_b, niter_b, max_n, out_model_b, out_inliers_b,
+                                    out_best_b, out_score_b, scratch_scores_b, scratch_models, lm_schedule)) return rc;
+    if (int rc = check_joint_kind(who, nprob_b, joint_kind)) return rc;
+    FitExtras EA = no_extras(), EB = no_extras();
+    if (int rc = make_extras(who, nprob_a, record, K, 1, tie_stats_a, (double)inlier_th_a, (double)tie_window_a, EA)) return rc;
+    if (nprob_b > 0) {
+        if (int rc = make_extras(who, nprob_b, record, K, 2, tie_stats_b, inlier_th_b, tie_window_b, EB)) return rc;
+    }
+    EB.draws = draws_b; EB.seed = tie_seed_b;
+    if (nprob_a + nprob_b == 0) return ANCSH_OK;
+    hipStream_t st = (hipStream_t)stream;
+    double th_b = 0.0;
+    float th_a = 0.f;
+    if (nprob_b > 0)
+        th_b = ransac_joint_hypotheses<KM>(nprob_b, rng0, rng1, src, tgt, joint_dir, inlier_th_b, niter_b, draws_b, seed_b, scratch_scores_b,
+                                           scratch_models, lm_stat, lm_schedule, joint_kind, st);
+    if (nprob_a > 0)
+        th_a = ransac_single_score<KM>(nprob_a, off, src, tgt, inlier_th_a, niter_a, draws_a, seed_a, max_n, scratch_scores_a, scratch_quads,
+                                       rows, st);
+    const size_t lds_a = nprob_a > 0 ? single_finish_lds(max_n) : 0, lds_b = nprob_b > 0 ? joint_finish_lds(max_n) : 0;
+    const size_t lds = lds_a > lds_b ? lds_a : lds_b;
+    if (joint_kind) {
+        if (lds > 48 * 1024) (void)hipFuncSetAttribute((const void *)ransac_finish_pair_kind_kernel<KM>, hipFuncAttributeMaxDynamicSharedMemorySize, (int)lds);
+        hipLaunchKernelGGL(ransac_finish_pair_kind_kernel<KM>, dim3(nprob_a + nprob_b), dim3(256), lds, st, nprob_a, src, tgt, max_n, off, th_a,
+                           niter_a, draws_a, seed_a, (const int *)scratch_scores_a, out_model_a, out_inliers_a, out_best_a, EA, rng0, rng1,
+                           joint_dir, th_b, niter_b, (const double *)scratch_scores_b, (const double *)scratch_models, out_model_b,
+                           out_inliers_b, out_best_b, out_score_b, EB, joint_kind);
+        return check_launch(who);
+    }
+    if (lds > 48 * 1024) (void)hipFuncSetAttribute((const void *)ransac_finish_pair_kernel<KM>, hipFuncAttributeMaxDynamicSharedMemorySize, (int)lds);
+    hipLaunchKernelGGL(ransac_finish_pair_kernel<KM>, dim3(nprob_a + nprob_b), dim3(256), lds, st, nprob_a, src, tgt, max_n, off, th_a, niter_a,
+                       draws_a, seed_a, (const int *)scratch_scores_a, out_model_a, out_inliers_a, out_best_a, EA, rng0, rng1, joint_dir, th_b,
+                       niter_b, (const double *)scratch_scores_b, (const double *)scratch_models, out_model_b, out_inliers_b, out_best_b,
+                       out_score_b, EB);
+    return check_launch(who);
+}
+
+extern "C" int ancsh_ransac_pair_rec(const float *src, const float *tgt, int max_n, double *record, int K,
+                                     int nprob_a, const int *off, float inlier_th_a, int niter_a, const int *draws_a,
+                                     unsigned long long seed_a, double *out_model_a, unsigned char *out_inliers_a, int *out_best_a,
+                                     int *scratch_scores_a, float *scratch_quads, long rows, int *tie_stats_a, float tie_window_a,
+                                     int nprob_b, const int *rng0, const int *rng1, const float *joint_dir, double inlier_th_b,
+                                     int niter_b, const int *draws_b, unsigned long long seed_b, double *out_model_b,
+                                     unsigned char *out_inliers_b, int *out_best_b, double *out_score_b, double *scratch_scores_b,
+                                     double *scratch_models, int *lm_stat, int lm_schedule, int *tie_stats_b, double tie_window_b,
+                                     const int *joint_kind, void *stream) {
+    return ransac_pair_impl<KEY_VALUE>("ransac_pair_rec", src, tgt, max_n, record, K, nprob_a, off, inlier_th_a, niter_a, draws_a, seed_a,
+                                       out_model_a, out_inliers_a, out_best_a, scratch_scores_a, scratch_quads, rows, tie_stats_a,
+                                       tie_window_a, nprob_b, rng0, rng1, joint_dir, inlier_th_b, niter_b, draws_b, seed_b, seed_b,
+                                       out_model_b, out_inliers_b, out_best_b, out_score_b, scratch_scores_b, scratch_models, lm_stat,
+                                       lm_schedule, tie_stats_b, tie_window_b, joint_kind, stream);
+}
+
+extern "C" int ancsh_ransac_pair_rec_dseed(const float *src, const float *tgt, int max_n, double *record, int K,
+                                           int nprob_a, const int *off, float inlier_th_a, int niter_a, const int *draws_a,
+                                           const unsigned long long *seed, double *out_model_a, unsigned char *out_inliers_a,
+                                           int *out_best_a, int *scratch_scores_a, float *scratch_quads, long rows, int *tie_stats_a,
+                                           float tie_window_a,
+                                           int nprob_b, const int *rng0, const int *rng1, const float *joint_dir, double inlier_th_b,
+                                           int niter_b, const int *draws_b, double *out_model_b, unsigned char *out_inliers_b,
+                                           int *out_best_b, double *out_score_b, double *scratch_scores_b, double *scratch_models,
+                                           int *lm_stat, int lm_schedule, int *tie_stats_b, double tie_window_b, const int *joint_kind,
+                                           void *stream) {
+    ANCSH_REQUIRE(seed, "ransac_pair_rec_dseed: null seed pointer");
+    const unsigned long long key = (unsigned long long)(uintptr_t)seed;
+    return ransac_pair_impl<KEY_DSEED>("ransac_pair_rec_dseed", src, tgt, max_n, record, K, nprob_a, off, inlier_th_a, niter_a, draws_a, key,
+                                       out_model_a, out_inliers_a, out_best_a, scratch_scores_a, scratch_quads, rows, tie_stats_a,
+                                       tie_window_a, nprob_b, rng0, rng1, joint_dir, inlier_th_b, niter_b, draws_b, key, key, out_model_b,
+                                       out_inliers_b, out_best_b, out_score_b, scratch_scores_b, scratch_models, lm_stat, lm_schedule,
+                                       tie_stats_b, tie_window_b, joint_kind, stream);
+}
+
+extern "C" int ancsh_ransac_pair_rec_dkey(const float *src, const float *tgt, int max_n, double *record, int K,
+                                          int nprob_a, const int *off, float inlier_th_a, int niter_a, const int *draws_a,
+                                          const ancsh_stream_key *key, double *out_model_a, unsigned char *out_inliers_a,
+                                          int *out_best_a, int *scratch_scores_a, float *scratch_quads, long rows, int *tie_stats_a,
+                                          float tie_window_a,
+                                          int nprob_b, const int *rng0, const int *rng1, const float *joint_dir, double inlier_th_b,
+                                          int niter_b, const int *draws_b, double *out_model_b, unsigned char *out_inliers_b,
+                                          int *out_best_b, double *out_score_b, double *scratch_scores_b, double *scratch_models,
+                                          int *lm_stat, int lm_schedule, int *tie_stats_b, double tie_window_b, const int *joint_kind,
+                                          void *stream) {
+    ANCSH_REQUIRE(key, "ransac_pair_rec_dkey: null key pointer");
+    ANCSH_REQUIRE(K >= 2 && nprob_a >= 0 && nprob_a % K == 0 && nprob_a < (1 << 20) && nprob_b >= 0 && nprob_b % (K - 1) == 0,
+                  "ransac_pair_rec_dkey: nprob_a (%d) must be a multiple of K (%d >= 2) below 2^20 and nprob_b (%d) one of K - 1", nprob_a, K,
+                  nprob_b);
+    return ransac_pair_impl<KEY_DKEY>("ransac_pair_rec_dkey", src, tgt, max_n, record, K, nprob_a, off, inlier_th_a, niter_a, draws_a,
+                                      DKey{key, K}, out_model_a, out_inliers_a, out_best_a, scratch_scores_a, scratch_quads, rows,
+                                      tie_stats_a, tie_window_a, nprob_b, rng0, rng1, joint_dir, inlier_th_b, niter_b, draws_b,
+                                      DKey{key, K - 1}, (unsigned long long)(uintptr_t)key, out_model_b, out_inliers_b, out_best_b,
+                                      out_score_b, scratch_scores_b, scratch_models, lm_stat, lm_schedule, tie_stats_b, tie_window_b,
+                                      joint_kind, stream);
+}
+
 extern "C" int ancsh_umeyama(int nprob, const int *off, const float *src, const float *tgt, double *out, void *stream) {
     ANCSH_REQUIRE(nprob >= 0, "umeyama: negative nprob");
     if (nprob == 0) return ANCSH_OK;
diff --git a/articulated-pose_amd/pose/parallel_ancsh_pose.py b/articulated-pose_amd/pose/parallel_ancsh_pose.py
--- a/articulated-pose_amd/pose/parallel_ancsh_pose.py
+++ b/articulated-pose_amd/pose/parallel_ancsh_pose.py
@@ -136,6 +136,48 @@
     return dict(model=model, inliers=inl, best=best, score=score, lm_stat=stat, hyp_models=mo, hyp_scores=sc, tie=tie, _keep=(d, joint_kind))
 
 
+def ransac_pair_batch(off, rng0, rng1, src, tgt, joint_dir, inlier_th, niter_a, niter_b, draws_a=None, draws_b=None, seed=0, max_n=None,
+                      want_lm_stat=False, lm_schedule="auto", record=None, K=0, tie_window=None, seed_dev=None, key_dev=None,
+                      joint_kind=None):
+    dev = src.device
+    nprob_a, nprob_b, rows = off.numel() - 1, rng0.shape[0], src.shape[0]
+    max_n = int(max_n or rows)
+    model_a = torch.empty((nprob_a, 13), dtype=torch.float64, device=dev)
+    inl_a = torch.empty((rows,), dtype=torch.uint8, device=dev)
+    best_a = torch.empty((nprob_a, 2), dtype=torch.int32, device=dev)
+    scores_a = torch.empty((nprob_a * niter_a,), dtype=torch.int32, device=dev)
+    quads = torch.empty((_lib.lib().ancsh_ransac_single_quads_floats(rows, nprob_a),), dtype=torch.float32, device=dev)
+    model_b = torch.empty((nprob_b, 26), dtype=torch.float64, device=dev)
+    inl_b = torch.empty((nprob_b, 2, max_n), dtype=torch.uint8, device=dev)
+    best_b = torch.empty((nprob_b,), dtype=torch.int32, device=dev)
+    score_b = torch.empty((nprob_b,), dtype=torch.float64, device=dev)
+    sc = torch.empty((nprob_b * niter_b,), dtype=torch.float64, device=dev)
+    mo = torch.empty((nprob_b * niter_b, 26), dtype=torch.float64, device=dev)
+    stat = torch.empty((nprob_b, niter_b, 2), dtype=torch.int32, device=dev) if want_lm_stat else None
+    da = None if draws_a is None else _i32(draws_a, dev)
+    db = None if draws_b is None else _i32(draws_b, dev)
+    if da is not None and da.numel() != nprob_a * niter_a * 3:
+        raise ValueError("draws_a must have shape (nprob_a, niter_a, 3)")
+    if db is not None and db.numel() != nprob_b * niter_b * 6:
+        raise ValueError("draws_b must have shape (nprob_b, niter_b, 6)")
+    if joint_kind is not None and (joint_kind.dtype != torch.int32 or joint_kind.numel() != nprob_b or not joint_kind.is_contiguous()):
+        raise ValueError("joint_kind must be a contiguous int32 tensor of %d entries (one per problem)" % nprob_b)
+    tie_a = torch.empty((nprob_a, 2), dtype=torch.int32, device=dev) if tie_window is not None else None
+    tie_b = torch.empty((nprob_b, 2), dtype=torch.int32, device=dev) if tie_window is not None else None
+    name, key_a, key_b = (("ancsh_ransac_pair_rec_dkey", (_lib.ptr(key_dev),), ()) if key_dev is not None else
+                          ("ancsh_ransac_pair_rec_dseed", (_lib.ptr(seed_dev),), ()) if seed_dev is not None else
+                          ("ancsh_ransac_pair_rec", (int(seed),), (int(seed) + 1,)))
+    _lib.call(name, _lib.ptr(src), _lib.ptr(tgt), max_n, _lib.ptr(record), int(K),
+              nprob_a, _lib.ptr(off), float(inlier_th), int(niter_a), _lib.ptr(da), *key_a, _lib.ptr(model_a), _lib.ptr(inl_a),
+              _lib.ptr(best_a), _lib.ptr(scores_a), _lib.ptr(quads), rows, _lib.ptr(tie_a), float(tie_window or 0.0),
+              nprob_b, _lib.ptr(rng0), _lib.ptr(rng1), _lib.ptr(joint_dir), float(inlier_th), int(niter_b), _lib.ptr(db), *key_b,
+              _lib.ptr(model_b), _lib.ptr(inl_b), _lib.ptr(best_b), _lib.ptr(score_b), _lib.ptr(sc), _lib.ptr(mo), _lib.ptr(stat),
+              LM_SCHEDULES[lm_schedule], _lib.ptr(tie_b), float(tie_window or 0.0), _lib.ptr(joint_kind))
+    return (dict(model=model_a, inliers=inl_a, best=best_a, scores=scores_a.view(nprob_a, niter_a), tie=tie_a, _keep=(da, scores_a, quads)),
+            dict(model=model_b, inliers=inl_b, best=best_b, score=score_b, lm_stat=stat, hyp_models=mo, hyp_scores=sc, tie=tie_b,
+                 _keep=(db, joint_kind)))
+
+
 def draws_from_seed(seed, counts, niter_a, niter_b):
     rs = np.random.RandomState(seed)
     K = len(counts)
@@ -178,6 +220,8 @@
               key_dev=None, joint_index=None):
         _one_association(joint_cls, joint_index)
         out = self._partition(P, nocs_pred, mask_pred)
+        if self.K > 1:
+            return self._poison(self._pair_fits(out, joint_axis_per_point, joint_cls, draws_a, draws_b, seed, seed_dev, key_dev, joint_index))
         self._stage_b_fits(out, joint_axis_per_point, joint_cls, draws_b, seed, seed_dev, key_dev, joint_index)
         return self._poison(self._stage_a_fits(out, draws_a, seed, seed_dev, key_dev))
 
@@ -227,6 +271,11 @@
         a = ransac_single_batch(out["off"], out["_src"], out["_tgt"], self.th, self.niter_a,
                                 None if draws_a is None else _i32(draws_a, dev).reshape(B * K, self.niter_a, 3), seed, out["_max_n"],
                                 record=out["record"], K=K, tie_window=self.tie_window, seed_dev=seed_dev, key_dev=key_dev)
+        return self._take_a(out, a)
+
+    def _take_a(self, out, a):
+        K = self.K
+        B, N = out["_shape"]
         out.update(baseline=out["record"][:, :, :13], best_a=a["best"].view(B, K, 2), inliers_a=a["inliers"].view(B, N))
         if a["tie"] is not None:
             out["tie_a"] = a["tie"].view(B, K, 2)
@@ -245,35 +294,60 @@
         src, tgt, max_n = out["_src"], out["_tgt"], out["_max_n"]
         rng0, rng1 = out["_rng"]
         if K > 1:
-            axis = _f32(joint_axis_per_point, dev)
-            out["_axis"] = axis
-            jdir = torch.empty((B, K - 1, 3), dtype=torch.float32, device=dev)
-            if joint_index is not None:
-                index = _f32(joint_index, dev)
-                if index.dim() != 3 or tuple(index.shape[:2]) != (B, N):
-                    raise ValueError("joint_index must be (B, N, C) for %d clouds of %d points, got %s" % (B, N, tuple(index.shape)))
-                out["_index"] = index
-                _lib.call("ancsh_pose_joint_direction_pred", B, N, K, int(index.shape[2]), _lib.ptr(axis), _lib.ptr(index), _lib.ptr(jdir))
-            else:
-                jcls = _i32(joint_cls, dev)
-                _lib.call("ancsh_pose_joint_direction", B, N, K, _lib.ptr(axis), _lib.ptr(jcls), _lib.ptr(jdir))
+            jdir = self._joint_directions(out, joint_axis_per_point, joint_cls, joint_index)
             b = ransac_joint_batch(rng0, rng1, src, tgt, jdir.view(-1, 3), self.th, self.niter_b,
                                    None if draws_b is None else _i32(draws_b, dev).reshape(B * (K - 1), self.niter_b, 6),
                                    seed + 1, max_n, want_lm_stat=self.want_lm_stat, lm_schedule=self.lm_schedule,
                                    record=out["record"], K=K, tie_window=self.tie_window, seed_dev=seed_dev, key_dev=key_dev,
                                    joint_kind=self.prepare(B))
-            if self.want_lm_stat:
-                out["lm_stat"] = b["lm_stat"].view(B, K - 1, self.niter_b, 2)
-            out["nonlinear"] = out["record"][:, :, 13:]
-            if b["tie"] is not None:
-                out["tie_b"] = b["tie"].view(B, K - 1, 2)
-            out["best_b"] = b["best"].view(B, K - 1)
-            out["score_b"] = b["score"].view(B, K - 1)
-            out["joint_direction"] = jdir
-            out["inliers_b"] = b["inliers"].view(B, K - 1, 2, max_n)
+            self._take_b(out, b, jdir)
         else:
             out["nonlinear"] = out["record"][:, :, 13:]
         return out
+
+    def _joint_directions(self, out, joint_axis_per_point, joint_cls, joint_index):
+        dev, K = self.device, self.K
+        B, N = out["_shape"]
+        axis = _f32(joint_axis_per_point, dev)
+        out["_axis"] = axis
+        jdir = torch.empty((B, K - 1, 3), dtype=torch.float32, device=dev)
+        if joint_index is not None:
+            index = _f32(joint_index, dev)
+            if index.dim() != 3 or tuple(index.shape[:2]) != (B, N):
+                raise ValueError("joint_index must be (B, N, C) for %d clouds of %d points, got %s" % (B, N, tuple(index.shape)))
+            out["_index"] = index
+            _lib.call("ancsh_pose_joint_direction_pred", B, N, K, int(index.shape[2]), _lib.ptr(axis), _lib.ptr(index), _lib.ptr(jdir))
+        else:
+            jcls = _i32(joint_cls, dev)
+            _lib.call("ancsh_pose_joint_direction", B, N, K, _lib.ptr(axis), _lib.ptr(jcls), _lib.ptr(jdir))
+        return jdir
+
+    def _take_b(self, out, b, jdir):
+        K = self.K
+        B, _N = out["_shape"]
+        if self.want_lm_stat:
+            out["lm_stat"] = b["lm_stat"].view(B, K - 1, self.niter_b, 2)
+        out["nonlinear"] = out["record"][:, :, 13:]
+        if b["tie"] is not None:
+            out["tie_b"] = b["tie"].view(B, K - 1, 2)
+        out["best_b"] = b["best"].view(B, K - 1)
+        out["score_b"] = b["score"].view(B, K - 1)
+        out["joint_direction"] = jdir
+        out["inliers_b"] = b["inliers"].view(B, K - 1, 2, out["_max_n"])
+
+    def _pair_fits(self, out, joint_axis_per_point, joint_cls, draws_a=None, draws_b=None, seed=0, seed_dev=None, key_dev=None,
+                   joint_index=None):
+        dev, K = self.device, self.K
+        B, _N = out["_shape"]
+        rng0, rng1 = out["_rng"]
+        jdir = self._joint_directions(out, joint_axis_per_point, joint_cls, joint_index)
+        a, b = ransac_pair_batch(out["off"], rng0, rng1, out["_src"], out["_tgt"], jdir.view(-1, 3), self.th, self.niter_a, self.niter_b,
+                                 None if draws_a is None else _i32(draws_a, dev).reshape(B * K, self.niter_a, 3),
+                                 None if draws_b is None else _i32(draws_b, dev).reshape(B * (K - 1), self.niter_b, 6),
+                                 seed, out["_max_n"], want_lm_stat=self.want_lm_stat, lm_schedule=self.lm_schedule, record=out["record"],
+                                 K=K, tie_window=self.tie_window, seed_dev=seed_dev, key_dev=key_dev, joint_kind=self.prepare(B))
+        self._take_b(out, b, jdir)
+        return self._take_a(out, a)
 
 
 def _one_association(joint_cls, joint_index):
diff --git a/include/ancsh_hip.h b/include/ancsh_hip.h
--- a/include/ancsh_hip.h
+++ b/include/ancsh_hip.h
@@ -294,6 +294,31 @@
                                      double *scratch_scores, double *scratch_models, int *lm_stat, int lm_schedule, double *record, int K,
                                      int *tie_stats, double tie_window, const int *joint_kind, void *stream);
 
+int ancsh_ransac_pair_rec(const float *src, const float *tgt, int max_n, double *record, int K,
+                          int nprob_a, const int *off, float inlier_th_a, int niter_a, const int *draws_a, unsigned long long seed_a,
+                          double *out_model_a, unsigned char *out_inliers_a, int *out_best_a, int *scratch_scores_a,
+                          float *scratch_quads, long rows, int *tie_stats_a, float tie_window_a,
+                          int nprob_b, const int *rng0, const int *rng1, const float *joint_dir, double inlier_th_b, int niter_b,
+                          const int *draws_b, unsigned long long seed_b, double *out_model_b, unsigned char *out_inliers_b,
+                          int *out_best_b, double *out_score_b, double *scratch_scores_b, double *scratch_models, int *lm_stat,
+                          int lm_schedule, int *tie_stats_b, double tie_window_b, const int *joint_kind, void *stream);
+int ancsh_ransac_pair_rec_dseed(const float *src, const float *tgt, int max_n, double *record, int K,
+                                int nprob_a, const int *off, float inlier_th_a, int niter_a, const int *draws_a,
+                                const unsigned long long *seed, double *out_model_a, unsigned char *out_inliers_a, int *out_best_a,
+                                int *scratch_scores_a, float *scratch_quads, long rows, int *tie_stats_a, float tie_window_a,
+                                int nprob_b, const int *rng0, const int *rng1, const float *joint_dir, double inlier_th_b, int niter_b,
+                                const int *draws_b, double *out_model_b, unsigned char *out_inliers_b, int *out_best_b,
+                                double *out_score_b, double *scratch_scores_b, double *scratch_models, int *lm_stat, int lm_schedule,
+                                int *tie_stats_b, double tie_window_b, const int *joint_kind, void *stream);
+int ancsh_ransac_pair_rec_dkey(const float *src, const float *tgt, int max_n, double *record, int K,
+                               int nprob_a, const int *off, float inlier_th_a, int niter_a, const int *draws_a,
+                               const ancsh_stream_key *key, double *out_model_a, unsigned char *out_inliers_a, int *out_best_a,
+                               int *scratch_scores_a, float *scratch_quads, long rows, int *tie_stats_a, float tie_window_a,
+                               int nprob_b, const int *rng0, const int *rng1, const float *joint_dir, double inlier_th_b, int niter_b,
+                               const int *draws_b, double *out_model_b, unsigned char *out_inliers_b, int *out_best_b,
+                               double *out_score_b, double *scratch_scores_b, double *scratch_models, int *lm_stat, int lm_schedule,
+                               int *tie_stats_b, double tie_window_b, const int *joint_kind, void *stream);
+
 int ancsh_umeyama(int nprob, const int *off, const float *src, const float *tgt, double *out, void *stream);
 
 int ancsh_estimate_similarity_transform(int nprob, const int *off, const float *src, const float *tgt, int niter,
```

Measured after the change: 17600. 1.8% lower.
